# SciML/NeuralPDE.jl

Hardware: AMD Instinct MI355X
Metric: collocation-point residual+grad evals/sec, 2D Poisson 4x64 MLP (higher is better)
Workload: dtype f32, hidden-layer forward / dA / dW GEMMs as 3-piece bf16 split products (6 bf16 MFMAs per product block, fp32 accumulation; 24 mantissa bits rebuilt; the five small piece products on an accumulator of their own: zero-mean, a third of the rms error of an fp32-MFMA fmaf chain per GEMM output, tools/m

## Files before the change

### neuralpde.jl_amd/csrc/aux_kernels.hpp

```cpp
#pragma once
#include <cstdlib>
#include "aux_limits.hpp"
#include "int_limits.hpp"
#include "plat.hpp"
#include "rprog.hpp"
#include "update_rules.hpp"
#include "sample_rules.hpp"

namespace aux {

#ifdef PINN_EMU
#define AUX_DEV inline
#else
#define AUX_DEV __device__ __forceinline__
#endif

struct alignas(16) F4 { float x, y, z, w; };

struct Reduce1Args {
    double* tmp[MAX_GROUPS];
    const float* slabs[MAX_GROUPS];
    const double* losspart[MAX_GROUPS];
    int slab[MAX_GROUPS], nblocks[MAX_GROUPS], nsplit[MAX_GROUPS], nent[MAX_GROUPS], active[MAX_GROUPS];
    int nwpb[MAX_GROUPS];
    int K;
};
struct Reduce2Args {
    float* out;
    float* sums;
    double* lossraw;
    const int* row_ptr;
    const int* row_grp;
    const int* row_ent;
    const double* tmp[MAX_GROUPS];
    int stride[MAX_GROUPS], nsplit[MAX_GROUPS], nent[MAX_GROUPS], active[MAX_GROUPS];
    int ent_active[MAX_GROUPS];
    int ngroups, P, K;
    int skip_grad;
    const int* perm;
};
struct ReduceOneArgs {
    const float* slabs;
    int slab, nblocks, nent;
    const int* ent_theta;
    float* out;
    float* sums;
    double* lossraw;
    int P, K;
    int nloss;
    const double* losspart[MAX_GROUPS];
    int nrows[MAX_GROUPS];
};
constexpr int RONE_CHUNKS = 32, RONE_ENT = 32;

struct ExprArgs {
    const float* pts;
    int N, d, nparams, nparams_estim;
    const float* params;
    int nslots;
    const float* jets[EXPR_MAX_SLOTS];
    float* ubar[EXPR_MAX_SLOTS];
    int nzero;
    float* zero[EXPR_MAX_SLOTS];
    const rp::Instr* prog;
    int nops, out_row;
    float scale;
    double* losspart;
    float* pslab;
    int K, term_id;
    float* resid;
    int loss_only;
    const float* data;
    const float* pw;
};
AUX_DEV float expr_point(int p, const ExprArgs& a, float (&pb)[4]) {
    float v[EXPR_MAX_ROWS], g[EXPR_MAX_ROWS];
    const int R0 = a.d + a.nparams + a.nslots;
    for (int i = 0; i < a.d; ++i) v[i] = a.pts[(size_t)p * a.d + i];
    for (int j = 0; j < a.nparams; ++j) v[a.d + j] = a.params[j];
    for (int s = 0; s < a.nslots; ++s) v[a.d + a.nparams + s] = a.jets[s][p];
    for (int q = 0; q < a.nops; ++q) {
        const rp::Instr ins = a.prog[q];
        const float va = rp::is_nullary(ins.code) ? 0.f : v[ins.a];
        const float vb = rp::is_binary(ins.code) ? v[ins.b] : 0.f;
        v[R0 + q] = (ins.code == rp::OP_DATA) ? a.data[(size_t)(int)ins.imm * a.N + p] : rp::apply<float>(ins.code, va, vb, ins.imm);
    }
    const float r = v[a.out_row];
    for (int j = 0; j < 4; ++j) pb[j] = 0.f;
    if (a.resid) { a.resid[p] = r; return r; }
    if (a.loss_only) return r * (a.pw ? a.pw[p] : 1.0f);
    for (int q = 0; q < R0 + a.nops; ++q) g[q] = 0.f;
    g[a.out_row] = 1.0f;
    for (int q = a.nops - 1; q >= 0; --q) {
        const rp::Instr ins = a.prog[q];
        if (rp::is_nullary(ins.code)) continue;
        const float vb = rp::is_binary(ins.code) ? v[ins.b] : 0.f;
        float da, db;
        rp::adjoint<float>(ins.code, v[ins.a], vb, v[R0 + q], ins.imm, g[R0 + q], da, db);
        g[ins.a] += da;
        if (rp::is_binary(ins.code)) g[ins.b] += db;
    }
    const float sw = a.pw ? a.pw[p] : 1.0f;
    const float rs = r * sw;
    const float rbar = rs * a.scale * sw;
    for (int s = 0; s < a.nslots; ++s) a.ubar[s][p] = rbar * g[a.d + a.nparams + s];
    for (int z = 0; z < a.nzero; ++z) a.zero[z][p] = 0.f;
    for (int j = 0; j < a.nparams_estim; ++j) pb[j] = rbar * g[a.d + j];
    return rs;
}

struct IntNodeDev {
    int var, lo_row, hi_row;
    float lo, hi;
    double lo64, hi64;
    int slot0, nslots;
    int prog_off, nops, out_row;
};
struct IntSitesArgs {
    float* sites;
    int N, d, nnodes, Q;
    const double* xi;
    IntNodeDev node[INT_MAX_NODES];
};
AUX_DEV void int_site_body(int e, const IntSitesArgs& a) {
    const int per = a.nnodes * a.Q;
    if (e >= a.N * per) return;
    const int p = e % a.N, j = e / a.N;
    const int k = j / a.Q, q = j % a.Q;
    const IntNodeDev nd = a.node[k];
    const float* x = a.sites + (size_t)p * a.d;
    const double lo = nd.lo_row >= 0 ? (double)x[nd.lo_row] : nd.lo64;
    const double hi = nd.hi_row >= 0 ? (double)x[nd.hi_row] : nd.hi64;
    const float s = (float)(lo + (hi - lo) * (0.5 * (a.xi[q] + 1.0)));
    float* y = a.sites + ((size_t)(1 + j) * a.N + p) * a.d;
    for (int i = 0; i < a.d; ++i) y[i] = (i == nd.var) ? s : x[i];
}

// ... 142 lines not shown
    for (int q = a.inv_ptr[i]; q < a.inv_ptr[i + 1]; ++q) {
        const int pos = a.inv_pos[q];
        a.packed[pos >> 24][pos & 0xFFFFFF] = t;
    }
}
AUX_DEV void total_loss_body(double* hist, int step, const float* out, int P, int K, const float* w_over_n) {
    double s = 0.0;
    for (int k = 0; k < K; ++k) s += (double)out[P + k] * (double)w_over_n[k];
    hist[step] = s;
}
AUX_DEV void sums_from_double_body(int k, float* out_sums, const double* raw) { out_sums[k] = (float)raw[k]; }
constexpr int PACK_BF_MAX_LAYERS = 16;
struct PackBfArgs {
    const float* theta;
    unsigned* out_fwd;
    unsigned* out_tr;
    int nhh, hp;
    float* packed;
    const int* idx;
    int n_gather;
    int woff[PACK_BF_MAX_LAYERS], nout[PACK_BF_MAX_LAYERS], nin[PACK_BF_MAX_LAYERS];
};
AUX_DEV unsigned bf16_rne(float x) {
    unsigned u;
    __builtin_memcpy(&u, &x, 4);
    if ((u & 0x7FFFFFFFu) > 0x7F800000u) return (u >> 16) | 0x40u;
    u += 0x7FFFu + ((u >> 16) & 1u);
    return u >> 16;
}
AUX_DEV float bf16_val(unsigned h) { const unsigned u = h << 16; float x; __builtin_memcpy(&x, &u, 4); return x; }
AUX_DEV unsigned bf16_piece(float v, int piece) {
    const unsigned h = bf16_rne(v);
    if (piece == 0) return h;
    const float r = v - bf16_val(h);
    const unsigned m = bf16_rne(r);
    if (piece == 1) return m;
    return bf16_rne(r - bf16_val(m));
}
AUX_DEV void pack_bf16_body(int e, const PackBfArgs& a) {
    const int mt = a.hp / 16, kbn = a.hp / 32;
    const int total = a.nhh * mt * kbn * 3 * 256;
    if (e >= 2 * total) return;
    const bool tr = e >= total;
    int r = tr ? e - total : e;
    const int j2 = r & 3; r >>= 2;
    const int lane = r & 63; r >>= 6;
    const int piece = r % 3; r /= 3;
    const int kb = r % kbn; r /= kbn;
    const int ta = r % mt; r /= mt;
    const int hl = r;
    const int g = lane >> 4, c = lane & 15;
    unsigned word = 0;
    for (int half = 0; half < 2; ++half) {
        const int j = 2 * j2 + half;
        const int other = 16 * (2 * kb + (j >> 2)) + 4 * g + (j & 3), mine = 16 * ta + c;
        const int out = tr ? other : mine, in = tr ? mine : other;
        const float v = (out < a.nout[hl] && in < a.nin[hl]) ? a.theta[a.woff[hl] + out + in * a.nout[hl]] : 0.f;
        word |= bf16_piece(v, piece) << (16 * half);
    }
    (tr ? a.out_tr : a.out_fwd)[tr ? e - total : e] = word;
}
struct EmbedArgs {
    const float* upts;
    float* pts;
    int n, du, dx;
    int src[4], is_cos[4];
    double omega[4];
};
AUX_DEV void embed_body(int p, const EmbedArgs& a) {
    if (p >= a.n) return;
    for (int i = 0; i < a.du; ++i) a.pts[(size_t)p * a.dx + i] = a.upts[(size_t)p * a.du + i];
    for (int k = 0; k < a.dx - a.du; ++k) {
        const double ph = a.omega[k] * (double)a.upts[(size_t)p * a.du + a.src[k]];
        a.pts[(size_t)p * a.dx + a.du + k] = (float)(a.is_cos[k] ? cos(ph) : sin(ph));
    }
}
AUX_DEV void pack_body(int i, float* packed, const int* idx, const float* theta) {
    const int j = idx[i];
    packed[i] = (j >= 0) ? theta[j] : 0.f;
}
AUX_DEV void params_body(int j, float* params, const float* theta, const float* defaults, int ne, int p_off) {
    params[j] = (j < ne) ? theta[p_off + j] : defaults[j];
}
#ifdef PINN_EMU
#define AUX_UNROLL8
#else
#define AUX_UNROLL8 _Pragma("unroll 8")
#endif
AUX_DEV void reduce1_body(int e4, int chunk, int g, const Reduce1Args& a) {
    if (!a.active[g] || chunk >= a.nsplit[g]) return;
    const int nb = a.nblocks[g], ns = a.nsplit[g];
    const int per = (nb + ns - 1) / ns;
    const int b0 = chunk * per, b1 = (b0 + per < nb) ? b0 + per : nb;
    double* out = a.tmp[g] + chunk;
    const int nq = a.nent[g] / 4;
    if (e4 < nq) {
        double s0 = 0.0, s1 = 0.0, s2 = 0.0, s3 = 0.0;
        const float* p = a.slabs[g] + 4 * e4;
        AUX_UNROLL8
        for (int b = b0; b < b1; ++b) {
            const F4 q = *reinterpret_cast<const F4*>(p + (size_t)b * a.slab[g]);
            s0 += (double)q.x; s1 += (double)q.y; s2 += (double)q.z; s3 += (double)q.w;
        }
        out[(size_t)(4 * e4) * ns] = s0; out[(size_t)(4 * e4 + 1) * ns] = s1;
        out[(size_t)(4 * e4 + 2) * ns] = s2; out[(size_t)(4 * e4 + 3) * ns] = s3;
    } else if (e4 < nq + a.K) {
        const int k = e4 - nq;
        const double* p = a.losspart[g] + k;
        double s = 0.0;
        AUX_UNROLL8
        for (int wv = b0 * a.nwpb[g]; wv < b1 * a.nwpb[g]; ++wv) s += p[(size_t)wv * a.K];
        out[(size_t)(a.nent[g] + k) * ns] = s;
    }
}
AUX_DEV void reduce_one_chunk(int e4, int ch, const ReduceOneArgs& a, double (&s)[4]) {
    const int per = (a.nblocks + RONE_CHUNKS - 1) / RONE_CHUNKS;
    const int b0 = ch * per, b1 = (b0 + per < a.nblocks) ? b0 + per : a.nblocks;
    s[0] = s[1] = s[2] = s[3] = 0.0;
    const float* p = a.slabs + 4 * e4;
    AUX_UNROLL8
    for (int b = b0; b < b1; ++b) {
        const F4 q = *reinterpret_cast<const F4*>(p + (size_t)b * a.slab);
        s[0] += (double)q.x; s[1] += (double)q.y; s[2] += (double)q.z; s[3] += (double)q.w;
    }
}
AUX_DEV double reduce_one_loss_part(int k, int t, int nthreads, const ReduceOneArgs& a) {
    double s = 0.0;
    for (int i = 0; i < a.nloss; ++i)
        for (int r = t; r < a.nrows[i]; r += nthreads) s += a.losspart[i][(size_t)r * a.K + k];
    return s;
}
AUX_DEV void reduce2_body(int r, const Reduce2Args& a) {
    if (r < a.P) {
        if (a.skip_grad) return;
        double s = 0.0;
        const int i0 = a.row_ptr[r], i1 = a.row_ptr[r + 1];
        for (int i = i0; i < i1; i += 4) {
            const double* t[4];
            int ns[4];
            for (int j = 0; j < 4; ++j) {
                const int ii = (i + j < i1) ? i + j : i;
                const int g = a.row_grp[ii];
                ns[j] = (i + j < i1 && a.ent_active[g]) ? a.nsplit[g] : 0;
                t[j] = a.tmp[g] + (size_t)a.row_ent[ii] * a.nsplit[g];
            }
            for (int j = 0; j < 4; ++j) {
                AUX_UNROLL8
                for (int ch = 0; ch < ns[j]; ++ch) s += t[j][ch];
            }
        }
        a.out[r] = (float)s;
    } else if (r < a.P + a.K) {
        const int k = r - a.P;
        double s = 0.0;
        for (int g = 0; g < a.ngroups; ++g) {
            if (!a.active[g]) continue;
            const double* t = a.tmp[g] + (size_t)(a.nent[g] + k) * a.nsplit[g];
            AUX_UNROLL8
            for (int ch = 0; ch < a.nsplit[g]; ++ch) s += t[ch];
        }
        a.sums[k] = (float)s;
        if (a.lossraw) a.lossraw[k] = s;
    }
}

constexpr int REDUCE_DIRECT_MAX = 32;
AUX_DEV void reduce_direct_body(int t, const Reduce1Args& a1, const Reduce2Args& a) {
    if (t >= a.P + a.K) return;
    const int r = a.perm ? a.perm[t] : t;
    if (r < a.P) {
        if (a.skip_grad) return;
        double s = 0.0;
        for (int i = a.row_ptr[r]; i < a.row_ptr[r + 1]; ++i) {
            const int g = a.row_grp[i];
            if (!a.ent_active[g]) continue;
            const float* p = a1.slabs[g] + a.row_ent[i];
            const int nb = a1.nblocks[g], st = a1.slab[g];
            AUX_UNROLL8
            for (int b = 0; b < nb; ++b) s += (double)p[(size_t)b * st];
        }
        a.out[r] = (float)s;
    } else if (r < a.P + a.K) {
        const int k = r - a.P;
        double s = 0.0;
        for (int g = 0; g < a.ngroups; ++g) {
            if (!a.active[g]) continue;
            const double* p = a1.losspart[g] + k;
            const int nw = a1.nblocks[g] * a1.nwpb[g];
            AUX_UNROLL8
            for (int wv = 0; wv < nw; ++wv) s += p[(size_t)wv * a.K];
        }
        a.sums[k] = (float)s;
        if (a.lossraw) a.lossraw[k] = s;
    }
}

inline bool reduce_is_small(const Reduce1Args& a1, const Reduce2Args& a2) {
    const char* e = std::getenv("PINN_REDUCE_DIRECT_MAX");
    const int lim = e ? std::atoi(e) : REDUCE_DIRECT_MAX;
    for (int g = 0; g < a2.ngroups; ++g)
        if (a1.active[g] && a1.nblocks[g] > lim) return false;
    return true;
}
#ifdef PINN_EMU
inline void launch_pack(float* packed, const int* idx, const float* theta, int n, plat_stream) {
    for (int i = 0; i < n; ++i) pack_body(i, packed, idx, theta);
}
inline void launch_embed(const EmbedArgs& a, plat_stream) {
    for (int p = 0; p < a.n; ++p) embed_body(p, a);
}
inline void launch_params(float* params, const float* theta, const float* defaults, int np, int ne, int p_off, plat_stream) {
    for (int j = 0; j < np; ++j) params_body(j, params, theta, defaults, ne, p_off);
}
// ... 2 lines not shown
    for (int i = 0; i < a.n_gather; ++i) pack_body(i, a.packed, a.idx, a.theta);
    for (int e = 0; e < 2 * total; ++e) pack_bf16_body(e, a);
}
inline void launch_sums_from_double(float* out_sums, const double* raw, int K, plat_stream) {
    for (int k = 0; k < K; ++k) sums_from_double_body(k, out_sums, raw);
}
inline void launch_adam(float* theta, float* m, float* v, const float* grad, int P, float lr, float b1, float b2, float eps, float c1, float c2, plat_stream) {
    for (int i = 0; i < P; ++i) adam_body(i, theta, m, v, grad, lr, b1, b2, eps, c1, c2);
}
inline void launch_total_loss(double* hist, int step, const float* out, int P, int K, const float* w_over_n, plat_stream) {
    total_loss_body(hist, step, out, P, K, w_over_n);
}
inline void launch_sample(int kind, float* pts, int n_elems, int d, const float* lb, const float* ub, unsigned seed, unsigned draw, plat_stream) {
    for (int e = 0; e < n_elems; ++e) {
        if (kind == 3) sample_sobol_body(e, pts, d, lb, ub, seed, draw);
        else if (kind == 2) sample_lhs_body(e, pts, d, n_elems / d, lb, ub, seed, draw);
        else sample_body(e, pts, d, lb, ub, seed, draw);
    }
}
inline void launch_adam_fused(const AdamFusedArgs& a, plat_stream) {
    for (int i = 0; i < (a.P > 1 ? a.P : 1); ++i) adam_fused_body(i, a);
}
inline void launch_resample(const ResampleTerm* samp, int nsamp, int max_n, int step, plat_stream) {
    for (int p = 0; p < max_n; ++p) resample_point_sets(samp, nsamp, p, max_n, step);
}
inline void launch_adam_dev(float* theta, float* m, float* v, const float* grad, int P, float lr, float b1, float b2, float eps, const float* c12, const int* step, plat_stream st) {
    launch_adam(theta, m, v, grad, P, lr, b1, b2, eps, c12[2 * step[0]], c12[2 * step[0] + 1], st);
}
inline void launch_total_loss_dev(double* hist, const int* step, const float* out, int P, int K, const float* w_over_n, plat_stream st) {
    launch_total_loss(hist, step[0], out, P, K, w_over_n, st);
}
inline void launch_sample_dev(int kind, float* pts, int n_elems, int d, const float* lb, const float* ub, unsigned seed, const unsigned* draw, plat_stream st) {
    launch_sample(kind, pts, n_elems, d, lb, ub, seed, draw[0], st);
}
inline void launch_advance(int* step, unsigned* draws, const int* sampled, int K, plat_stream) {
    for (int t = 0; t < K; ++t) if (sampled[t]) ++draws[t];
    ++step[0];
}
inline void launch_src(const SrcArgs& a, plat_stream) {
    for (int p = 0; p < a.N; ++p) src_point(p, a);
}
inline void launch_expr(const ExprArgs& a, int nblocks, plat_stream) {
    for (int b = 0; b < nblocks; ++b)
        for (int w = 0; w < 4; ++w) {
            double ls = 0.0;
            double ps[4] = {0, 0, 0, 0};
            for (int l = 0; l < 64; ++l) {
                const int p = (b * 4 + w) * 64 + l;
                if (p >= a.N) continue;
                float pb[4];
                const float r = expr_point(p, a, pb);
                ls += (double)r * (double)r;
                for (int j = 0; j < 4; ++j) ps[j] += (double)pb[j];
            }
            if (!a.resid) {
                a.losspart[(size_t)(b * 4 + w) * a.K + a.term_id] = ls;
                for (int j = 0; j < 4; ++j) a.pslab[(size_t)(b * 4 + w) * 4 + j] = (float)ps[j];
            }
        }
}
inline void launch_int_sites(const IntSitesArgs& a, plat_stream) {
    for (int e = 0; e < a.N * a.nnodes * a.Q; ++e) int_site_body(e, a);
}
inline void launch_int_expr(const IntExprArgs& a, int nblocks, plat_stream) {
    for (int b = 0; b < nblocks; ++b)
        for (int w = 0; w < 4; ++w) {
            double ls = 0.0;
            double ps[4] = {0, 0, 0, 0};
            for (int l = 0; l < 64; ++l) {
                const int p = (b * 4 + w) * 64 + l;
                if (p >= a.N) continue;
                float pb[4];
                const float r = int_expr_point(p, a, pb);
                ls += (double)r * (double)r;
                for (int j = 0; j < 4; ++j) ps[j] += (double)pb[j];
            }
            if (!a.resid) {
                a.losspart[(size_t)(b * 4 + w) * a.K + a.term_id] = ls;
                for (int j = 0; j < 4; ++j) a.pslab[(size_t)(b * 4 + w) * 4 + j] = (float)ps[j];
            }
        }
}
inline void launch_reduce_one(const ReduceOneArgs& a, plat_stream) {
    for (int e4 = 0; e4 < a.nent / 4; ++e4) {
        double tot[4] = {0, 0, 0, 0}, s[4];
        for (int ch = 0; ch < RONE_CHUNKS; ++ch) {
            reduce_one_chunk(e4, ch, a, s);
            for (int e = 0; e < 4; ++e) tot[e] += s[e];
        }
        for (int e = 0; e < 4; ++e)
            if (a.ent_theta[4 * e4 + e] >= 0) a.out[a.ent_theta[4 * e4 + e]] = (float)tot[e];
    }
    for (int k = 0; k < a.K; ++k) {
        double part[256], s = 0.0;
        for (int t = 0; t < 256; ++t) part[t] = reduce_one_loss_part(k, t, 256, a);
        for (int st = 128; st >= 1; st >>= 1)
            for (int t = 0; t < st; ++t) part[t] += part[t + st];
        s = part[0];
        a.sums[k] = (float)s;
        if (a.lossraw) a.lossraw[k] = s;
    }
}
inline void launch_reduce(const Reduce1Args& a1, const Reduce2Args& a2, int max_n1, int max_split, plat_stream) {
    if (reduce_is_small(a1, a2)) {
        for (int r = 0; r < a2.P + a2.K; ++r) reduce_direct_body(r, a1, a2);
        return;
    }
    for (int g = 0; g < a2.ngroups; ++g)
        for (int ch = 0; ch < max_split; ++ch)
            for (int e = 0; e < max_n1; ++e) reduce1_body(e, ch, g, a1);
    for (int r = 0; r < a2.P + a2.K; ++r) reduce2_body(r, a2);
}
#else
__global__ void k_pack(float* packed, const int* idx, const float* theta, int n) {
    const int i = blockIdx.x * blockDim.x + threadIdx.x;
    if (i < n) pack_body(i, packed, idx, theta);
}
__global__ void k_params(float* params, const float* theta, const float* defaults, int np, int ne, int p_off) {
    const int j = threadIdx.x;
    if (j < np) params_body(j, params, theta, defaults, ne, p_off);
}
__global__ void k_adam(float* theta, float* m, float* v, const float* grad, int P, float lr, float b1, float b2, float eps, float c1, float c2) {
    const int i = blockIdx.x * blockDim.x + threadIdx.x;
    if (i < P) adam_body(i, theta, m, v, grad, lr, b1, b2, eps, c1, c2);
}
__global__ void k_total_loss(double* hist, int step, const float* out, int P, int K, const float* w_over_n) {
    if (threadIdx.x == 0 && blockIdx.x == 0) total_loss_body(hist, step, out, P, K, w_over_n);
}
__global__ void k_sample(float* pts, int n_elems, int d, const float* lb, const float* ub, unsigned seed, unsigned draw) {
    const int e = blockIdx.x * blockDim.x + threadIdx.x;
    if (e < n_elems) sample_body(e, pts, d, lb, ub, seed, draw);
}
__global__ void k_sample_lhs(float* pts, int n_elems, int d, const float* lb, const float* ub, unsigned seed, unsigned draw) {
    const int e = blockIdx.x * blockDim.x + threadIdx.x;
    if (e < n_elems) sample_lhs_body(e, pts, d, n_elems / d, lb, ub, seed, draw);
}
__global__ void k_sample_sobol(float* pts, int n_elems, int d, const float* lb, const float* ub, unsigned seed, unsigned draw) {
    const int e = blockIdx.x * blockDim.x + threadIdx.x;
    if (e < n_elems) sample_sobol_body(e, pts, d, lb, ub, seed, draw);
}
inline void launch_adam(float* theta, float* m, float* v, const float* grad, int P, float lr, float b1, float b2, float eps, float c1, float c2, plat_stream st) {
    hipLaunchKernelGGL(k_adam, dim3((P + 255) / 256), dim3(256), 0, st, theta, m, v, grad, P, lr, b1, b2, eps, c1, c2);
}
inline void launch_total_loss(double* hist, int step, const float* out, int P, int K, const float* w_over_n, plat_stream st) {
    hipLaunchKernelGGL(k_total_loss, dim3(1), dim3(64), 0, st, hist, step, out, P, K, w_over_n);
}
inline void launch_sample(int kind, float* pts, int n_elems, int d, const float* lb, const float* ub, unsigned seed, unsigned draw, plat_stream st) {
    if (kind == 3) hipLaunchKernelGGL(k_sample_sobol, dim3((n_elems + 255) / 256), dim3(256), 0, st, pts, n_elems, d, lb, ub, seed, draw);
    else if (kind == 2) hipLaunchKernelGGL(k_sample_lhs, dim3((n_elems + 255) / 256), dim3(256), 0, st, pts, n_elems, d, lb, ub, seed, draw);
    else hipLaunchKernelGGL(k_sample, dim3((n_elems + 255) / 256), dim3(256), 0, st, pts, n_elems, d, lb, ub, seed, draw);
}
__global__ void __launch_bounds__(256) k_resample(const ResampleTerm* samp, int nsamp, int step) {
    resample_point_sets(samp, nsamp, (int)(blockIdx.x * blockDim.x + threadIdx.x), (int)(gridDim.x * blockDim.x), step);
}
inline void launch_resample(const ResampleTerm* samp, int nsamp, int max_n, int step, plat_stream st) {
    hipLaunchKernelGGL(k_resample, dim3((max_n + 255) / 256), dim3(256), 0, st, samp, nsamp, step);
}
__global__ void k_adam_fused(const AdamFusedArgs a) { adam_fused_body((int)(blockIdx.x * blockDim.x + threadIdx.x), a); }
inline void launch_adam_fused(const AdamFusedArgs& a, plat_stream st) {
    hipLaunchKernelGGL(k_adam_fused, dim3((a.P + 255) / 256), dim3(256), 0, st, a);
}
__global__ void k_adam_dev(float* theta, float* m, float* v, const float* grad, int P, float lr, float b1, float b2, float eps, const float* c12, const int* step) {
    const int i = blockIdx.x * blockDim.x + threadIdx.x;
    const int s = step[0];
    if (i < P) adam_body(i, theta, m, v, grad, lr, b1, b2, eps, c12[2 * s], c12[2 * s + 1]);
}
__global__ void k_total_loss_dev(double* hist, const int* step, const float* out, int P, int K, const float* w_over_n) {
    if (threadIdx.x == 0 && blockIdx.x == 0) total_loss_body(hist, step[0], out, P, K, w_over_n);
}
__global__ void k_sample_dev(int kind, float* pts, int n_elems, int d, const float* lb, const float* ub, unsigned seed, const unsigned* draw) {
    const int e = blockIdx.x * blockDim.x + threadIdx.x;
    if (e >= n_elems) return;
    const unsigned dr = draw[0];
    if (kind == 3) sample_sobol_body(e, pts, d, lb, ub, seed, dr);
    else if (kind == 2) sample_lhs_body(e, pts, d, n_elems / d, lb, ub, seed, dr);
    else sample_body(e, pts, d, lb, ub, seed, dr);
}
__global__ void k_advance(int* step, unsigned* draws, const int* sampled, int K) {
    const int t = threadIdx.x;
    if (t < K && sampled[t]) ++draws[t];
    if (t == 0) ++step[0];
}
inline void launch_adam_dev(float* theta, float* m, float* v, const float* grad, int P, float lr, float b1, float b2, float eps, const float* c12, const int* step, plat_stream st) {
    hipLaunchKernelGGL(k_adam_dev, dim3((P + 255) / 256), dim3(256), 0, st, theta, m, v, grad, P, lr, b1, b2, eps, c12, step);
// ... 13 lines not shown
    float pb[4] = {0.f, 0.f, 0.f, 0.f};
    float r = 0.f;
    if (p < a.N) r = expr_point(p, a, pb);
    if (a.resid) return;
    sh[0][threadIdx.x] = (double)r * (double)r;
    for (int j = 0; j < 4; ++j) sh[1 + j][threadIdx.x] = (double)pb[j];
    __syncthreads();
    if (threadIdx.x < 20) {
        const int w = threadIdx.x & 3, q = threadIdx.x >> 2;
        double s = 0.0;
        for (int l = 0; l < 64; ++l) s += sh[q][w * 64 + l];
        if (q == 0) a.losspart[(size_t)(blockIdx.x * 4 + w) * a.K + a.term_id] = s;
        else a.pslab[(size_t)(blockIdx.x * 4 + w) * 4 + (q - 1)] = (float)s;
    }
}
__global__ void k_reduce1(const Reduce1Args a) {
    reduce1_body((int)(blockIdx.x * blockDim.x + threadIdx.x), (int)blockIdx.y, (int)blockIdx.z, a);
}
__global__ void k_reduce2(const Reduce2Args a) {
    reduce2_body((int)(blockIdx.x * blockDim.x + threadIdx.x), a);
}
inline void launch_pack(float* packed, const int* idx, const float* theta, int n, plat_stream st) {
    hipLaunchKernelGGL(k_pack, dim3((n + 255) / 256), dim3(256), 0, st, packed, idx, theta, n);
}
__global__ void k_embed(const EmbedArgs a) { embed_body((int)(blockIdx.x * blockDim.x + threadIdx.x), a); }
inline void launch_embed(const EmbedArgs& a, plat_stream st) {
    hipLaunchKernelGGL(k_embed, dim3((a.n + 255) / 256), dim3(256), 0, st, a);
}
inline void launch_params(float* params, const float* theta, const float* defaults, int np, int ne, int p_off, plat_stream st) {
    if (np > 0) hipLaunchKernelGGL(k_params, dim3(1), dim3(64), 0, st, params, theta, defaults, np, ne, p_off);
}
__global__ void k_pack_bf16(const PackBfArgs a) {
    const int e = (int)(blockIdx.x * blockDim.x + threadIdx.x);
    if (e < a.n_gather) pack_body(e, a.packed, a.idx, a.theta);
    else pack_bf16_body(e - a.n_gather, a);
}
inline void launch_pack_bf16(const PackBfArgs& a, plat_stream st) {
    const int total = a.nhh * (a.hp / 16) * (a.hp / 32) * 3 * 256;
    hipLaunchKernelGGL(k_pack_bf16, dim3((a.n_gather + 2 * total + 255) / 256), dim3(256), 0, st, a);
}
__global__ void k_sums_from_double(float* out_sums, const double* raw, int K) {
    const int k = (int)(blockIdx.x * blockDim.x + threadIdx.x);
    if (k < K) sums_from_double_body(k, out_sums, raw);
}
inline void launch_sums_from_double(float* out_sums, const double* raw, int K, plat_stream st) {
    hipLaunchKernelGGL(k_sums_from_double, dim3((K + 63) / 64), dim3(64), 0, st, out_sums, raw, K);
}
__global__ void __launch_bounds__(256) k_src(const SrcArgs a) {
    const int p = blockIdx.x * 256 + threadIdx.x;
    if (p < a.N) src_point(p, a);
}
inline void launch_src(const SrcArgs& a, plat_stream st) {
    hipLaunchKernelGGL(k_src, dim3((a.N + 255) / 256), dim3(256), 0, st, a);
}
inline void launch_expr(const ExprArgs& a, int nblocks, plat_stream st) {
    hipLaunchKernelGGL(k_expr, dim3(nblocks), dim3(256), 0, st, a);
}
__global__ void __launch_bounds__(256) k_int_sites(const IntSitesArgs a) { int_site_body((int)(blockIdx.x * 256 + threadIdx.x), a); }
inline void launch_int_sites(const IntSitesArgs& a, plat_stream st) {
    hipLaunchKernelGGL(k_int_sites, dim3((a.N * a.nnodes * a.Q + 255) / 256), dim3(256), 0, st, a);
}
__global__ void __launch_bounds__(256) k_int_expr(const IntExprArgs a) {
    __shared__ double sh[5][256];
    const int p = blockIdx.x * 256 + threadIdx.x;
    float pb[4] = {0.f, 0.f, 0.f, 0.f};
    float r = 0.f;
    if (p < a.N) r = int_expr_point(p, a, pb);
    if (a.resid) return;
    sh[0][threadIdx.x] = (double)r * (double)r;
    for (int j = 0; j < 4; ++j) sh[1 + j][threadIdx.x] = (double)pb[j];
    __syncthreads();
    if (threadIdx.x < 20) {
        const int w = threadIdx.x & 3, q = threadIdx.x >> 2;
        double s = 0.0;
        for (int l = 0; l < 64; ++l) s += sh[q][w * 64 + l];
        if (q == 0) a.losspart[(size_t)(blockIdx.x * 4 + w) * a.K + a.term_id] = s;
        else a.pslab[(size_t)(blockIdx.x * 4 + w) * 4 + (q - 1)] = (float)s;
    }
}
inline void launch_int_expr(const IntExprArgs& a, int nblocks, plat_stream st) {
    hipLaunchKernelGGL(k_int_expr, dim3(nblocks), dim3(256), 0, st, a);
}
__global__ void __launch_bounds__(256) k_reduce_one(const ReduceOneArgs a) {
    __shared__ double sh[RONE_CHUNKS][RONE_ENT + 1];
    const int tid = (int)threadIdx.x;
    const int nentblocks = (a.nent + RONE_ENT - 1) / RONE_ENT;
    if ((int)blockIdx.x < nentblocks) {
        const int j = tid & 7, ch = tid >> 3;
        const int e4 = (int)blockIdx.x * (RONE_ENT / 4) + j;
        double s[4] = {0.0, 0.0, 0.0, 0.0};
        if (4 * e4 < a.nent) reduce_one_chunk(e4, ch, a, s);
        for (int e = 0; e < 4; ++e) sh[ch][4 * j + e] = s[e];
        __syncthreads();
        if (tid < RONE_ENT) {
            const int ent = (int)blockIdx.x * RONE_ENT + tid;
            if (ent < a.nent) {
                double tot = 0.0;
                for (int c2 = 0; c2 < RONE_CHUNKS; ++c2) tot += sh[c2][tid];
                const int th = a.ent_theta[ent];
                if (th >= 0) a.out[th] = (float)tot;
            }
        }
    } else {
        const int k = (int)blockIdx.x - nentblocks;
        double* part = &sh[0][0];
        part[tid] = reduce_one_loss_part(k, tid, 256, a);
        __syncthreads();
        for (int st = 128; st >= 1; st >>= 1) {
            if (tid < st) part[tid] += part[tid + st];
            __syncthreads();
        }
        if (tid == 0) {
            a.sums[k] = (float)part[0];
            if (a.lossraw) a.lossraw[k] = part[0];
        }
    }
}
inline void launch_reduce_one(const ReduceOneArgs& a, plat_stream st) {
    hipLaunchKernelGGL(k_reduce_one, dim3((a.nent + RONE_ENT - 1) / RONE_ENT + a.K), dim3(256), 0, st, a);
}
__global__ void k_reduce_direct(const Reduce1Args a1, const Reduce2Args a2) {
    reduce_direct_body((int)(blockIdx.x * blockDim.x + threadIdx.x), a1, a2);
}
inline void launch_reduce(const Reduce1Args& a1, const Reduce2Args& a2, int max_n1, int max_split, plat_stream st) {
    if (reduce_is_small(a1, a2)) {
        hipLaunchKernelGGL(k_reduce_direct, dim3((a2.P + a2.K + 63) / 64), dim3(64), 0, st, a1, a2);
        return;
    }
    hipLaunchKernelGGL(k_reduce1, dim3((max_n1 + 255) / 256, max_split, a2.ngroups), dim3(256), 0, st, a1);
    hipLaunchKernelGGL(k_reduce2, dim3((a2.P + a2.K + 255) / 256), dim3(256), 0, st, a2);
}
#endif

}
```

### neuralpde.jl_amd/csrc/comm.cpp

```cpp
#include "engine_types.hpp"

using namespace pe;

#ifndef PINN_EMU
#include <dlfcn.h>
#include <rccl/rccl.h>

namespace {
struct Rccl {
    void* lib = nullptr;
    ncclResult_t (*GetUniqueId)(ncclUniqueId*) = nullptr;
    ncclResult_t (*CommInitRank)(ncclComm_t*, int, ncclUniqueId, int) = nullptr;
    ncclResult_t (*CommInitAll)(ncclComm_t*, int, const int*) = nullptr;
    ncclResult_t (*CommDestroy)(ncclComm_t) = nullptr;
    ncclResult_t (*AllReduce)(const void*, void*, size_t, ncclDataType_t, ncclRedOp_t, ncclComm_t, hipStream_t) = nullptr;
    ncclResult_t (*GroupStart)() = nullptr;
    ncclResult_t (*GroupEnd)() = nullptr;
    const char* (*GetErrorString)(ncclResult_t) = nullptr;
    std::string err;
};
Rccl& rccl() {
    static Rccl R = [] {
        Rccl r;
        for (const char* name : {"librccl.so.1", "librccl.so", "/opt/rocm/lib/librccl.so.1"}) {
// ... 216 lines not shown
    for (int i = 0; i < ndev; ++i) {
        pinn_engine& E = *es[i];
        DeviceScope scope(E.device);
        const ncclResult_t rc = rccl().AllReduce(vec[i], vec[i], (size_t)count, ncclDouble, ncclSum, (ncclComm_t)E.comm, E.stream);
        if (rc != ncclSuccess) { (void)rccl().GroupEnd(); return nccl_fail("ncclAllReduce", rc); }
    }
    NCCL_TRY(rccl().GroupEnd(), "ncclGroupEnd");
#else
    {
        std::vector<double> sum((size_t)count, 0.0);
        for (int i = 0; i < ndev; ++i)
            for (int64_t j = 0; j < count; ++j) sum[(size_t)j] += vec[i][j];
        for (int i = 0; i < ndev; ++i) std::memcpy(vec[i], sum.data(), sizeof(double) * (size_t)count);
    }
#endif
    return 0;
}

extern "C" {

int pinn_loss_grad_sharded_device_f64(pinn_handle h, const double* d_theta, const float* term_w, double* d_out, void* stream) {
    if (!h || !d_theta || !d_out) return fail("pinn_loss_grad_sharded_device_f64: null argument");
    pinn_engine& E = *h;
    if (!E.f64) return fail("pinn_loss_grad_sharded_device_f64: the handle is not in the float64 evaluation mode (pinn_set_option(h, \"precision\", \"f64\"))");
    if (!E.comm) return fail("pinn_loss_grad_sharded_device_f64: the handle has no communicator (pinn_comm_init_rank / pinn_comm_init_custom)");
    if (!E.comm_per_process && E.comm_size > 1)
        return fail("pinn_loss_grad_sharded_device_f64: the handle belongs to a single-process communicator (pinn_comm_init_all): use pinn_loss_grad_sharded_f64");
    DeviceScope scope(E.device);
    if (check_shards(E)) return 1;
    plat_stream saved = E.stream;
    E.stream = (plat_stream)stream;
    int rc = f64_eval_from_device_f64(E, d_theta, term_w, d_out);
    if (!rc) {
        pinn_engine* es[1] = {&E};
        double* vec[1] = {d_out};
        rc = comm_all_reduce_f64(es, 1, vec, E.ntheta + (int64_t)E.terms.size());
    }
    E.stream = saved;
    return rc;
}

int pinn_loss_grad_sharded_f64(pinn_handle* hs, int ndev, const double* theta, int64_t p, const double* term_w, double* term_losses, double* grad) {
    if (!hs || ndev < 1 || !theta) return fail("pinn_loss_grad_sharded_f64: null argument");
    for (int i = 0; i < ndev; ++i) {
        if (!hs[i] || !hs[i]->comm || hs[i]->comm_size != ndev || hs[i]->comm_rank != i)
            return fail("pinn_loss_grad_sharded_f64: pass the handles of one pinn_comm_init_all communicator, in rank order");
        if (!hs[i]->f64) return fail("pinn_loss_grad_sharded_f64: every handle must be in the float64 evaluation mode");
        if (p != hs[i]->ntheta) return fail("pinn_loss_grad_sharded_f64: theta length mismatch");
    }
    const int64_t P = hs[0]->ntheta;
    const int K = (int)hs[0]->terms.size();
    std::vector<double*> vec(ndev);
    for (int i = 0; i < ndev; ++i) {
        pinn_engine& E = *hs[i];
        DeviceScope scope(E.device);
        if (check_shards(E)) return 1;
        if (f64_eval_sharded_local(E, theta, term_w, &vec[i])) return 1;
    }
    if (comm_all_reduce_f64(hs, ndev, vec.data(), P + K)) return 1;
    std::vector<double> out((size_t)(P + K));
    {
        pinn_engine& E0 = *hs[0];
        DeviceScope scope(E0.device);
        if (plat_d2h(out.data(), vec[0], sizeof(double) * (size_t)(P + K), E0.stream)) return fail("D2H copy failed");
    }
    for (int i = 0; i < ndev; ++i) {
        DeviceScope scope(hs[i]->device);
        if (plat_sync(hs[i]->stream)) return fail(std::string("device error: ") + plat_last_error());
    }
    if (term_losses) for (int k = 0; k < K; ++k) term_losses[k] = out[(size_t)P + k] / (double)hs[0]->terms[k].n_norm;
    if (grad) std::memcpy(grad, out.data(), sizeof(double) * (size_t)P);
    return 0;
}

int pinn_loss_grad_sharded_device(pinn_handle h, const float* d_theta, const float* term_w, float* d_out, void* stream) {
    if (!h || !d_theta || !d_out) return fail("pinn_loss_grad_sharded_device: null argument");
    pinn_engine& E = *h;
    if (!E.comm) return fail("pinn_loss_grad_sharded_device: the handle has no communicator (pinn_comm_init_rank / pinn_comm_init_all)");
    DeviceScope scope(E.device);
    if (check_shards(E)) return 1;
    plat_stream st = (plat_stream)stream;
    plat_stream saved = E.stream;
    E.stream = st;
    int rc = run_loss_grad(E, d_theta, d_out, term_w, -1, true);
    E.stream = saved;
    if (rc) return rc;
    E.timing_valid = E.timing_level >= 2;
    if (!E.comm_per_process && E.comm_size > 1)
        return fail("pinn_loss_grad_sharded_device: the handle belongs to a single-process communicator (pinn_comm_init_all): use pinn_loss_grad_sharded");
    {
        pinn_engine* es[1] = {&E};
        float* vec[1] = {d_out};
        double* raw[1] = {E.d_lossraw};
        E.stream = st;
        rc = comm_all_reduce(es, 1, vec, raw);
        E.stream = saved;
        if (rc) return rc;
    }
    sums_from_double(d_out + E.ntheta, E.d_lossraw, (int)E.terms.size(), st);
    return 0;
}

int pinn_loss_grad_sharded(pinn_handle* hs, int ndev, const float* theta, int64_t p, const float* term_w, double* term_losses, float* grad) {
    if (!hs || ndev < 1 || !theta) return fail("pinn_loss_grad_sharded: null argument");
    for (int i = 0; i < ndev; ++i) {
        if (!hs[i] || !hs[i]->comm || hs[i]->comm_size != ndev || hs[i]->comm_rank != i)
            return fail("pinn_loss_grad_sharded: pass the handles of one pinn_comm_init_all communicator, in rank order");
        if (i > 0 && hs[i]->comm != hs[0]->comm
#ifndef PINN_EMU
            && false
#endif
        ) return fail("pinn_loss_grad_sharded: handles of different communicators");
    }
    const int64_t P = hs[0]->ntheta;
    const int K = (int)hs[0]->terms.size();
    for (int i = 0; i < ndev; ++i) {
        pinn_engine& E = *hs[i];
        DeviceScope scope(E.device);
        if (check_shards(E) || upload_theta(E, theta, p)) return 1;
        if (run_loss_grad(E, E.d_theta, E.d_out, term_w, -1, false)) return 1;
    }
    {
        std::vector<float*> vec(ndev);
        std::vector<double*> raw(ndev);
        for (int i = 0; i < ndev; ++i) { vec[i] = hs[i]->d_out; raw[i] = hs[i]->d_lossraw; }
        if (comm_all_reduce(hs, ndev, vec.data(), raw.data())) return 1;
    }
    pinn_engine& E0 = *hs[0];
    {
        DeviceScope scope(E0.device);
        if (plat_d2h(E0.hp_out, E0.d_out, sizeof(float) * (P + K), E0.stream)) return fail("D2H copy failed");
        if (plat_d2h(E0.hp_raw, E0.d_lossraw, sizeof(double) * K, E0.stream)) return fail("D2H copy failed");
    }
    for (int i = 0; i < ndev; ++i) {
        DeviceScope scope(hs[i]->device);
        if (plat_sync(hs[i]->stream)) return fail(std::string("device error: ") + plat_last_error());
    }
    if (term_losses)
        for (int k = 0; k < K; ++k) term_losses[k] = E0.hp_raw[k] / (double)E0.terms[k].n_norm;
    if (grad) std::memcpy(grad, E0.hp_out, sizeof(float) * P);
    return 0;
}

}
```

### neuralpde.jl_amd/csrc/engine.cpp

```cpp
#include "engine_types.hpp"
#include "aux_kernels.hpp"
#include "hmc_kernels.hpp"
#include "lbfgs_kernels.hpp"

#include <type_traits>

#ifdef PINN_EMU
namespace wv {
thread_local void (*emu_barrier_hook)(void*) = nullptr;
thread_local void* emu_barrier_ctx = nullptr;
thread_local void (*emu_grid_hook)(void*) = nullptr;
thread_local void* emu_grid_ctx = nullptr;
}
#endif

namespace pk {
std::deque<SpecInfo>& registry() {
    static std::deque<SpecInfo> r;
    return r;
}
std::deque<PairInfo>& pair_registry() {
    static std::deque<PairInfo> r;
    return r;
}
// ... 120 lines not shown
    std::memset(&a, 0, sizeof a);
    a.sites = T.d_pts; a.N = (int)T.n; a.d = T.d; a.nparams = E.np; a.nparams_estim = E.ne; a.params = E.d_params;
    a.jets = Cp.d_jets[0]; a.ubar = Cp.d_ubar[0]; a.C = E.groups[Cp.groups[0]].spec->C;
    a.n_outer = T.n_outer; a.nnodes = (int)T.inodes.size(); a.Q = T.int_q;
    for (size_t si = 0; si < T.slots.size(); ++si) a.chan[si] = T.chan_of_slot[si];
    for (int c = 0; c < aux::INT_MAX_C; ++c) {
        a.outer_slot_of_chan[c] = -1;
        for (int k = 0; k < aux::INT_MAX_NODES; ++k) a.node_slot_of_chan[k][c] = -1;
    }
    for (int si = 0; si < T.n_outer; ++si) a.outer_slot_of_chan[T.chan_of_slot[(size_t)si]] = si;
    int off = 0;
    for (int k = 0; k < a.nnodes; ++k) {
        a.node[k] = int_node_dev(T, k, off);
        off += (int)T.inodes[(size_t)k].ops.size();
        for (int si = a.node[k].slot0; si < a.node[k].slot0 + a.node[k].nslots; ++si) a.node_slot_of_chan[k][T.chan_of_slot[(size_t)si]] = si;
    }
    a.w = E.d_int_w;
    a.prog = Cp.d_prog; a.iprog = T.d_int_prog; a.nops = (int)T.ops.size(); a.out_row = T.out_row; a.scale = scale;
    a.losspart = Cp.d_losspart; a.pslab = Cp.d_pslab; a.K = (int)E.terms.size(); a.term_id = Cp.term; a.resid = resid;
    a.data = T.d_data;
    a.pw = (T.pw_n == T.n && T.pw_n > 0) ? T.d_pw : nullptr;
    return a;
}

int upload_int_rule(pinn_engine& E, int q) {
    std::vector<double> xi((size_t)q), w((size_t)q);
    const double PI = 3.14159265358979323846264338327950288;
    for (int i = 0; i < q; ++i) {
        double x = -std::cos(PI * (i + 0.75) / (q + 0.5)), dp = 1.0;
        for (int it = 0; it < 100; ++it) {
            double p0 = 1.0, p1 = x;
            for (int n = 2; n <= q; ++n) { const double p2 = ((2.0 * n - 1.0) * x * p1 - (n - 1.0) * p0) / n; p0 = p1; p1 = p2; }
            dp = q * (x * p1 - p0) / (x * x - 1.0);
            const double dx = p1 / dp;
            x -= dx;
            if (std::fabs(dx) < 1e-16) break;
        }
        {
            double p0 = 1.0, p1 = x;
            for (int n = 2; n <= q; ++n) { const double p2 = ((2.0 * n - 1.0) * x * p1 - (n - 1.0) * p0) / n; p0 = p1; p1 = p2; }
            dp = q * (x * p1 - p0) / (x * x - 1.0);
        }
        xi[(size_t)i] = x;
        w[(size_t)i] = 2.0 / ((1.0 - x * x) * dp * dp);
    }
    std::vector<float> wf(w.begin(), w.end());
    if (!E.d_int_xi) {
        E.d_int_xi = (double*)plat_malloc(sizeof(double) * aux::INT_MAX_Q);
        E.d_int_w = (float*)plat_malloc(sizeof(float) * aux::INT_MAX_Q);
        if (!E.d_int_xi || !E.d_int_w) return fail("device allocation failed (quadrature rule)");
    }
    plat_h2d(E.d_int_xi, xi.data(), sizeof(double) * q, E.stream);
    plat_h2d(E.d_int_w, wf.data(), sizeof(float) * q, E.stream);
    if (plat_sync(E.stream)) return fail(std::string("device error: ") + plat_last_error());
    return 0;
}

template <class V, class T> class As {
    static constexpr bool same = std::is_same_v<V, std::remove_const_t<T>>;
    T* x_;
    std::vector<V> copy_;
public:
    As(T* x, size_t n) : x_(x) {
        if constexpr (!same) {
            if (x && std::is_const_v<T>) copy_.assign(x, x + n);
            else if (x) copy_.resize(n);
        }
    }
    auto get() {
        if constexpr (same) return x_;
        else return x_ ? copy_.data() : nullptr;
    }
    int put() {
        if constexpr (!same) if (x_) std::copy(copy_.begin(), copy_.end(), x_);
        return 0;
    }
};
template <class V, class T> As<V, T> as(T* x, size_t n) { return As<V, T>(x, n); }

int check_theta(const pinn_engine& E, const char* who, int64_t p) {
    return p == E.ntheta ? 0 : fail(std::string(who) + ": theta length " + std::to_string(p) + " != ntheta " + std::to_string(E.ntheta));
}

}

int pe::run_loss_grad(pinn_engine& E, const float* d_theta, float* d_out, const float* term_w, int only_term , bool timing,
                  double* lossraw , bool packed_fresh, bool loss_only, float* d_sums) {
    if (!d_sums) d_sums = d_out + E.ntheta;
    if (ensure_points(E)) return 1;
    const int K = (int)E.terms.size();
    const bool phase_ev = timing && E.timing_level >= 2;
    auto group_ev = [&](size_t g) { return timing && E.timing_level >= 1 && (E.timing_group < 0 || E.timing_group == (int)g); };
    if (phase_ev) plat_event_record(E.ev0, E.stream);
    pack_all(E, d_theta, packed_fresh);
    if (phase_ev) plat_event_record(E.ev1, E.stream);
    aux::Reduce1Args a1;
    aux::Reduce2Args a2;
    std::memset(&a1, 0, sizeof a1);
    std::memset(&a2, 0, sizeof a2);
    int max_n1 = 1, max_split = 1;
    auto scale_of = [&](int ti) -> float {
        const float w = term_w ? term_w[ti] : 1.0f;
        const bool on = (only_term < 0 || only_term == ti);
        return on ? (float)(2.0 * (double)w / (double)E.terms[ti].n_norm) : 0.f;
    };
    int nfused_active = 0;
    bool all_small = true;
    for (auto& G : E.groups) {
        bool on = false;
        for (int ti : G.terms) on = on || (only_term < 0 || only_term == ti);
        if (G.kind == 0 && on) {
            ++nfused_active;
            const int per_round = G.max_blocks * (G.spec->family == 2 ? 1 : 4);
            if (2 * G.ga.ntiles > 3 * per_round) all_small = false;
        }
    }
    static const bool want_concurrent = std::getenv("PINN_CONCURRENT_GROUPS") != nullptr;
    const bool concurrent = want_concurrent && nfused_active >= 2 && all_small;
    static const bool no_chain = std::getenv("PINN_NO_CHAIN") != nullptr;
    const bool no_merge = std::getenv("PINN_NO_MERGE") != nullptr;
    const bool may_merge = !no_merge && !no_chain && !concurrent && only_term < 0;
    int nforked = 0;
    int nslabsets = 0, slabset_group = -1;
    if (concurrent) plat_event_record(E.ev_fork, E.stream);
    for (size_t g = 0; g < E.groups.size(); ++g) {
        Group& G = E.groups[g];
        bool any = false;
        for (size_t j = 0; j < G.terms.size(); ++j) {
            G.ga.terms[j].scale = scale_of(G.terms[j]);
            any = any || (only_term < 0 || only_term == G.terms[j]);
        }
        G.active = any;
        G.timed = false;
        const MergedUnit* mu = (may_merge && G.kind == 0 && G.merged >= 0) ? &E.merged[G.merged] : nullptr;
        a1.tmp[g] = G.d_tmp; a1.slabs[g] = G.d_slabs; a1.losspart[g] = G.d_losspart;
        a2.tmp[g] = G.d_tmp;
        if (mu && (int)g == mu->tail) {
            G.launched_by = mu->head;
            G.launched_blocks = E.groups[mu->head].launched_blocks;
            a1.active[g] = 0; a2.active[g] = 0; a2.ent_active[g] = 0;
            a1.slab[g] = G.slab_floats; a1.nblocks[g] = 0; a1.nsplit[g] = 1; a1.nent[g] = 0; a1.nwpb[g] = G.spec->NW;
            a2.stride[g] = K; a2.nsplit[g] = 1; a2.nent[g] = 0;
            continue;
        }
        const bool chained = any && !loss_only && !no_chain && !concurrent && G.kind == 0 && G.chain_to >= 0 && E.groups[G.chain_to].active &&
                             G.blocks <= E.groups[G.chain_to].launched_blocks;
        const int nent = (chained || loss_only) ? 0 : G.nent;
        G.ga.slabs = chained ? E.groups[G.chain_to].d_slabs : G.d_slabs;
        G.ga.chain = chained ? 1 : 0;
        pk::GroupArgs ga_one;
        const pk::GroupArgs* ga_launch = &G.ga;
        int blocks = G.blocks;
        if (any && only_term >= 0 && G.kind == 0 && G.terms.size() > 1) {
            ga_one = G.ga;
            for (size_t j = 0; j < G.terms.size(); ++j)
                if (G.terms[j] == only_term) ga_one.terms[0] = G.ga.terms[j];
            ga_one.nterms = 1;
            ga_one.terms[0].tile0 = 0;
            ga_one.ntiles = ga_one.terms[0].ntiles;
            blocks = std::max(1, std::min(G.max_blocks, G.spec->family == 1 ? (ga_one.ntiles + 3) / 4 : ga_one.ntiles));
            ga_launch = &ga_one;
        }
        const bool merged_head = mu && (int)g == mu->head;
        if (merged_head) {
            const Group& T2 = E.groups[mu->tail];
            ga_one = G.ga;
            for (size_t j = 0; j < T2.terms.size(); ++j) {
                pk::TermDev td = T2.ga.terms[j];
                td.tile0 += G.ga.ntiles;
                td.scale = scale_of(T2.terms[j]);
                ga_one.terms[G.terms.size() + j] = td;
            }
            ga_one.nterms = (int)(G.terms.size() + T2.terms.size());
            ga_one.sub_terms0 = (int)G.terms.size();
            ga_one.sub_tiles0 = G.ga.ntiles;
            ga_one.ntiles = G.ga.ntiles + T2.ga.ntiles;
            ga_one.scratch = mu->d_scratch;
            ga_one.scr_stride = mu->pair->SCR;
            ga_one.losspart = mu->d_losspart;
            a1.losspart[g] = mu->d_losspart;
            ga_one.chain = 0;
            blocks = std::max(1, std::min(loss_only ? E.ncu * mu->pair->WG_FWD : mu->max_blocks, ga_one.ntiles));
            ga_launch = &ga_one;
        }
        G.launched_blocks = blocks;
        G.launched_by = (int)g;
        const int epe = G.spec->family == 1 ? 4 : 1;
        const int nsplit_g = std::max(1, std::min(REDUCE_SPLIT, (int)std::ceil(std::sqrt((double)blocks / epe))));
        a1.slab[g] = G.slab_floats; a1.nblocks[g] = blocks; a1.nsplit[g] = nsplit_g; a1.nent[g] = nent; a1.active[g] = any; a1.nwpb[g] = G.spec->NW;
        a2.stride[g] = nent + K; a2.nsplit[g] = nsplit_g; a2.nent[g] = nent; a2.active[g] = any;
        a2.ent_active[g] = any && !chained && !loss_only;
        if (!any) continue;
        if (a2.ent_active[g]) { ++nslabsets; slabset_group = (int)g; }
        max_n1 = std::max(max_n1, nent / 4 + K);
        max_split = std::max(max_split, nsplit_g);
        if (G.kind == 1) {
            G.spec->launch(G.ga, (G.use_rec && !loss_only) ? pk::MODE_FWDREC : pk::MODE_FWD,
                           std::max(1, std::min(E.ncu * G.spec->WG_FWD, G.spec->family == 1 ? (G.ga.ntiles + 3) / 4 : G.ga.ntiles)), E.stream);
            continue;
        }
        if (G.kind == 2) continue;
        plat_stream st = E.stream;
        const bool forked = concurrent && nforked++ > 0;
        if (forked) {
            st = E.aux_stream[nforked % 2];
            plat_stream_wait_event(st, E.ev_fork);
        }
        if (group_ev(g)) plat_event_record(G.ev_a, st);
        if (merged_head) mu->pair->launch(*ga_launch, loss_only ? pk::MODE_LOSS : pk::MODE_FUSED, blocks, st);
        else if (loss_only) {
            const int tiles = ga_launch->ntiles;
            const int fb = std::max(1, std::min(E.ncu * G.spec->WG_FWD, G.spec->family == 1 ? (tiles + 3) / 4 : tiles));
            a1.nblocks[g] = fb;
            G.launched_blocks = fb;
            G.spec->launch(*ga_launch, pk::MODE_LOSS, fb, st);
        } else G.spec->launch(*ga_launch, pk::MODE_FUSED, blocks, st);
        if (group_ev(g)) plat_event_record(G.ev_b, st);
        G.timed = group_ev(g);
        if (forked) {
            plat_event_record(E.ev_join[g], st);
            plat_stream_wait_event(E.stream, E.ev_join[g]);
        }
    }
    bool coupled_active = false;
    for (size_t c = 0; c < E.coupled.size(); ++c) {
        Coupled& Cp = E.coupled[c];
        const int g = (int)(E.groups.size() + c);
        const bool on = (only_term < 0 || only_term == Cp.term);
        const int nsplit = std::min(REDUCE_SPLIT, Cp.blocks);
        const int nent = loss_only ? 0 : 16;
        a1.tmp[g] = Cp.d_tmp; a1.slabs[g] = Cp.d_pslab; a1.losspart[g] = Cp.d_losspart;
        a1.slab[g] = 16; a1.nblocks[g] = Cp.blocks; a1.nsplit[g] = nsplit; a1.nent[g] = nent; a1.active[g] = on; a1.nwpb[g] = 4;
        a2.tmp[g] = Cp.d_tmp; a2.stride[g] = nent + K; a2.nsplit[g] = nsplit; a2.nent[g] = nent; a2.active[g] = on; a2.ent_active[g] = on && !loss_only;
        bool groups_active = false;
        for (int gi : Cp.groups) groups_active = groups_active || E.groups[gi].active;
        if (!groups_active) continue;
        coupled_active = true;
        if (Cp.tail >= 0) {
            Group& G = E.groups[Cp.groups[Cp.tail]];
            a1.active[g] = 0; a2.active[g] = 0; a2.ent_active[g] = 0;
            if (group_ev((size_t)Cp.groups[Cp.tail])) plat_event_record(G.ev_a, E.stream);
            if (loss_only) {
                const int fb = std::max(1, std::min(E.ncu * G.spec->WG_FWD, G.ga.ntiles));
                a1.nblocks[Cp.groups[Cp.tail]] = fb;
                G.launched_blocks = fb;
                G.spec->launch(G.ga, pk::MODE_LOSS, fb, E.stream);
            } else G.spec->launch(G.ga, pk::MODE_FUSED, G.blocks, E.stream);
            if (group_ev((size_t)Cp.groups[Cp.tail])) plat_event_record(G.ev_b, E.stream);
            G.timed = group_ev((size_t)Cp.groups[Cp.tail]);
            continue;
        }
        max_n1 = std::max(max_n1, nent / 4 + K);
        max_split = std::max(max_split, nsplit);
        if (!E.terms[Cp.term].inodes.empty()) {
            aux::IntExprArgs ia = int_expr_args(E, Cp, scale_of(Cp.term), nullptr);
            ia.loss_only = loss_only ? 1 : 0;
            aux::launch_int_expr(ia, Cp.blocks, E.stream);
            continue;
        }
        aux::ExprArgs ea = expr_args(E, Cp, scale_of(Cp.term), nullptr);
        ea.loss_only = loss_only ? 1 : 0;
        aux::launch_expr(ea, Cp.blocks, E.stream);
    }
    for (size_t g = 0; g < E.groups.size() && !loss_only; ++g) {
        Group& G = E.groups[g];
        if (G.kind != 1 || !G.active) continue;
        if (group_ev(g)) plat_event_record(G.ev_a, E.stream);
        G.spec->launch(G.ga, G.use_rec ? pk::MODE_GRADREC : pk::MODE_GRADIN, G.blocks, E.stream);
        if (group_ev(g)) plat_event_record(G.ev_b, E.stream);
        G.timed = group_ev(g);
    }
    if (phase_ev) plat_event_record(E.ev2, E.stream);
    a1.K = K;
    a2.out = d_out; a2.sums = d_sums; a2.lossraw = lossraw ? lossraw : E.d_lossraw; a2.row_ptr = E.d_gr_ptr; a2.row_grp = E.d_gr_grp; a2.row_ent = E.d_gr_ent;
    a2.ngroups = (int)(E.groups.size() + E.coupled.size()); a2.P = (int)E.ntheta; a2.K = K;
    a2.skip_grad = loss_only ? 1 : 0;
    a2.perm = std::getenv("PINN_NO_REDUCE_PERM") ? nullptr : E.d_red_perm;
    const bool no_reduce_one = std::getenv("PINN_NO_REDUCE_ONE") != nullptr;
    const Group* RG = (nslabsets == 1 && !coupled_active && !loss_only && !no_reduce_one) ? &E.groups[slabset_group] : nullptr;
    const bool one_kernel = ((RG && RG->d_ent_theta && RG->ent_covers_theta) || (loss_only && !no_reduce_one)) && !aux::reduce_is_small(a1, a2);
    if (one_kernel) {
        aux::ReduceOneArgs ro;
        std::memset(&ro, 0, sizeof ro);
        if (RG) { ro.slabs = RG->d_slabs; ro.slab = RG->slab_floats; ro.nblocks = a1.nblocks[slabset_group]; ro.nent = RG->nent; ro.ent_theta = RG->d_ent_theta; }
        ro.out = d_out; ro.sums = d_sums; ro.lossraw = a2.lossraw; ro.P = (int)E.ntheta; ro.K = K;
        for (int g = 0; g < a2.ngroups; ++g)
            if (a1.active[g]) { ro.losspart[ro.nloss] = a1.losspart[g]; ro.nrows[ro.nloss] = a1.nblocks[g] * a1.nwpb[g]; ++ro.nloss; }
        aux::launch_reduce_one(ro, E.stream);
    } else {
        aux::launch_reduce(a1, a2, max_n1, max_split, E.stream);
    }
    if (phase_ev) plat_event_record(E.ev3, E.stream);
    { const std::string e = jit_take_launch_error(); if (!e.empty()) return fail(e); }
    return 0;
}

void pe::sums_from_double(float* d_out_sums, const double* d_raw, int K, plat_stream st) { aux::launch_sums_from_double(d_out_sums, d_raw, K, st); }

int pe::upload_theta(pinn_engine& E, const float* theta, int64_t p) {
    if (p != E.ntheta) return fail("theta length " + std::to_string(p) + " != ntheta " + std::to_string(E.ntheta));
    std::memcpy(E.hp_theta, theta, sizeof(float) * p);
    if (plat_h2d(E.d_theta, E.hp_theta, sizeof(float) * p, E.stream)) return fail(std::string("H2D copy of theta failed: ") + plat_last_error());
    return 0;
}

static void hmc_free(pinn_engine& E);
static void lbfgs_free(pinn_engine& E);

extern "C" {

const char* pinn_backend(void) { return plat_name(); }
int pinn_abi_version(void) { return 1; }
const char* pinn_last_error(void) { return g_err.c_str(); }

int pinn_create(const char* descriptor, pinn_handle* out) { return pinn_create_on(descriptor, -1, out); }

int pinn_create_on(const char* descriptor, int device, pinn_handle* out) {
    if (!descriptor || !out) return fail("pinn_create: null argument");
    *out = nullptr;
    std::string err;
    if (plat_init(err)) return fail(err);
    if (device >= plat_device_count()) return fail("pinn_create_on: device " + std::to_string(device) + " does not exist (" + std::to_string(plat_device_count()) + " visible)");
    const int dev = device < 0 ? plat_get_device() : device;
    DeviceScope scope(dev);
    std::unique_ptr<pinn_engine> E(new pinn_engine());
    E->device = dev;
    if (const char* gm = std::getenv("PINN_GEMM")) {
        if (std::string(gm) == "fp32") E->gemm = pk::GEMM_FP32;
        else if (std::string(gm) == "split") E->gemm = pk::GEMM_SPLIT;
        else return fail(std::string("PINN_GEMM must be \"split\" or \"fp32\", not \"") + gm + "\"");
    }
    if (parse_descriptor(descriptor, *E)) return 1;
    E->terms0 = E->terms;
    E->ncu = plat_num_cus();
    E->stream = plat_stream_create();
    const int K = (int)E->terms.size();
    E->d_theta = (float*)plat_malloc(sizeof(float) * E->ntheta);
    E->d_params = (float*)plat_malloc(sizeof(float) * pk::MAX_PARAMS);
    E->d_defaults = (float*)plat_malloc(sizeof(float) * pk::MAX_PARAMS);
    E->d_lossraw = (double*)plat_malloc(sizeof(double) * K);
    E->d_out = (float*)plat_malloc(sizeof(float) * (E->ntheta + K));
    plat_event_create(E->ev0); plat_event_create(E->ev1); plat_event_create(E->ev2); plat_event_create(E->ev3);
    plat_event_create(E->ev_fork);
    for (auto& e : E->ev_join) plat_event_create(e);
    for (auto& st : E->aux_stream) st = plat_stream_create();
    if (!E->d_theta || !E->d_params || !E->d_defaults || !E->d_lossraw || !E->d_out) {
        pinn_destroy(E.release());
        return fail("device allocation failed");
    }
    plat_h2d(E->d_defaults, E->p_defaults.data(), sizeof(float) * pk::MAX_PARAMS, E->stream);
    E->hp_theta = (float*)plat_host_alloc(sizeof(float) * (2 * E->ntheta + K + 2) + sizeof(double) * K);
    if (!E->hp_theta) {
        pinn_destroy(E.release());
        return fail("pinned host allocation failed");
    }
    E->hp_out = E->hp_theta + E->ntheta;
    E->hp_raw = (double*)(E->hp_theta + ((2 * E->ntheta + K + 1) / 2) * 2);
    bool any_int = false;
    for (auto& T : E->terms) any_int = any_int || !T.inodes.empty();
    if ((any_int && upload_int_rule(*E, E->int_q)) || build_plan(*E)) {
        const std::string msg = g_err;
        pinn_destroy(E.release());
        g_err = msg;
        return 1;
    }
    *out = E.release();
    return 0;
}

int pinn_destroy(pinn_handle h) {
    if (!h) return 0;
    pinn_engine& E = *h;
    DeviceScope scope(E.device);
    pinn_comm_destroy(h);
    plat_sync(E.stream);
    hmc_free(E);
    lbfgs_free(E);
    f64_destroy(E);
    free_plan(E);
    for (auto& T : E.terms) { plat_free(T.d_pts); plat_free(T.d_upts); plat_free(T.d_resid); plat_free(T.d_lb); plat_free(T.d_ub); plat_free(T.d_data); plat_free(T.d_pw); }
    plat_free(E.d_opt_theta); plat_free(E.d_opt_m); plat_free(E.d_opt_v); plat_free(E.d_opt_out); plat_free(E.d_w_over_n); plat_free(E.d_hist); plat_free(E.d_step); plat_free(E.d_draws); plat_free(E.d_sampled); plat_free(E.d_c12); plat_free(E.d_bar); plat_free(E.d_sums2); plat_free(E.d_own_r); plat_free(E.d_train_samp); plat_free(E.d_opt_bak); plat_host_free(E.h_flag);
    plat_free(E.d_theta); plat_free(E.d_params); plat_free(E.d_defaults); plat_free(E.d_lossraw);
    plat_free(E.d_int_xi); plat_free(E.d_int_w);
    plat_free(E.d_out); plat_free(E.d_phi_pts); plat_free(E.d_phi_out); plat_free(E.d_phi_scr);
    plat_host_free(E.hp_theta);
    plat_event_destroy(E.ev0); plat_event_destroy(E.ev1); plat_event_destroy(E.ev2); plat_event_destroy(E.ev3);
    plat_event_destroy(E.ev_fork);
    for (auto& e : E.ev_join) plat_event_destroy(e);
    for (auto& st : E.aux_stream) plat_stream_destroy(st);
    if (E.own_stream) plat_stream_destroy(E.stream);
    delete h;
    return 0;
}

int pinn_num_terms(pinn_handle h) { return h ? (int)h->terms.size() : -1; }
int64_t pinn_num_theta(pinn_handle h) { return h ? h->ntheta : -1; }

static int term_installed(pinn_engine& E, int term);
static int set_points_impl(pinn_handle h, int term, const float* pts, int64_t n, int64_t n_norm, bool device) {
    if (!h) return fail("null handle");
    pinn_engine& E = *h;
    DeviceScope scope(E.device);
    if (term < 0 || term >= (int)E.terms.size()) return fail("pinn_set_points: term index out of range");
    if (!pts || n <= 0) return fail("pinn_set_points: empty point set (the reference's mean(abs2, .) over an empty set is NaN; refusing)");
    Term& T = E.terms[term];
    if (n * T.d >= (int64_t)1 << 31) return fail("pinn_set_points: point set too large for 32-bit indexing; shard it");
    const int64_t S = T.sites();
    if (S > 1 && n * S * std::max(T.d, aux::INT_MAX_C) >= (int64_t)1 << 31)
        return fail("pinn_set_points: the site set of integral term " + std::to_string(term) + " (" + std::to_string(n) + " points x (1 + " +
                    std::to_string(T.inodes.size()) + " integral node(s) x " + std::to_string(T.int_q) + " quadrature nodes) = " + std::to_string(n * S) +
                    " sites) exceeds what one launch group takes (32-bit indexing of its jet channels); shard the point set or lower integral_nodes");
    if (n > T.pts_cap || !T.d_pts) {
        plat_sync(E.stream);
        plat_free(T.d_pts);
        plat_free(T.d_upts);
        T.d_upts = nullptr;
        T.pts_cap = 0;
        T.d_pts = (float*)plat_malloc(sizeof(float) * n * S * T.d);
        if (!T.emb_cols.empty()) T.d_upts = (float*)plat_malloc(sizeof(float) * n * T.d_user);
        if (!T.d_pts || (!T.emb_cols.empty() && !T.d_upts)) return fail("device allocation failed (points)");
        T.pts_cap = n;
    }
    int rc = device ? plat_d2d(user_pts(T), pts, sizeof(float) * n * T.d_user, E.stream) : plat_h2d(user_pts(T), pts, sizeof(float) * n * T.d_user, E.stream);
    if (rc) return fail(std::string("copy of points failed: ") + plat_last_error());
    T.n = n;
    embed_points(E, T);
    plat_sync(E.stream);
    T.n_norm = n_norm > 0 ? n_norm : n;
    T.data_n = 0;
    T.pw_n = 0;
    if (term_installed(E, term)) return 1;
    return f64_points_changed(E, term);
}

static int term_installed(pinn_engine& E, int term) {
    Term& T = E.terms[term];
    int64_t n = T.n;
    if (T.coupled < 0) {
        if (!T.src_root.empty()) {
            if (T.src_cap < n) {
                plat_free(T.d_src);
                T.d_src = (float*)plat_malloc(sizeof(float) * T.src_root.size() * (size_t)n);
                if (!T.d_src) return fail("device allocation failed (source channels)");
                T.src_cap = n;
            }
            eval_sources(E, T);
            plat_sync(E.stream);
        }
        retile(E, T.group);
        return 0;
    }
    Coupled& Cp = E.coupled[T.coupled];
    const int K = (int)E.terms.size();
    const int64_t npts = n;
    n *= T.sites();
    if (Cp.cap < n) {
        for (size_t i = 0; i < Cp.d_jets.size(); ++i)
            if (Cp.tail < 0 || (int)i == Cp.tail) { plat_free(Cp.d_jets[i]); plat_free(Cp.d_ubar[i]); }
        plat_free(Cp.d_jets_all); plat_free(Cp.d_ubar_all);
        Cp.d_jets_all = Cp.d_ubar_all = nullptr;
        Cp.d_jets.assign(Cp.nets.size(), nullptr);
        Cp.d_ubar.assign(Cp.nets.size(), nullptr);
        Cp.cap = 0;
        if (Cp.tail >= 0 && Cp.nsrc > 0) {
            Cp.d_jets_all = (float*)plat_malloc(sizeof(float) * (size_t)Cp.nsrc * n);
            Cp.d_ubar_all = (float*)plat_malloc(sizeof(float) * (size_t)Cp.nsrc * n);
            if (!Cp.d_jets_all || !Cp.d_ubar_all) return fail("device allocation failed (coupled jets)");
        }
        for (size_t i = 0; i < Cp.nets.size(); ++i) {
            if (Cp.tail >= 0 && (int)i != Cp.tail) continue;
            const int C = E.groups[Cp.groups[i]].spec->C;
            Cp.d_jets[i] = (float*)plat_malloc(sizeof(float) * (size_t)C * n);
            Cp.d_ubar[i] = (float*)plat_malloc(sizeof(float) * (size_t)C * n);
            if (!Cp.d_jets[i] || !Cp.d_ubar[i]) return fail("device allocation failed (coupled jets)");
        }
        Cp.cap = n;
    }
    if (Cp.tail >= 0)
        for (size_t i = 0; i < Cp.nets.size(); ++i)
            if ((int)i != Cp.tail) { Cp.d_jets[i] = Cp.d_jets_all + (size_t)Cp.src_off[i] * n; Cp.d_ubar[i] = Cp.d_ubar_all + (size_t)Cp.src_off[i] * n; }
    Cp.blocks = (int)((npts + 255) / 256);
    if (Cp.cap_blocks < Cp.blocks) {
        plat_free(Cp.d_losspart); plat_free(Cp.d_pslab);
        Cp.d_losspart = (double*)plat_malloc(sizeof(double) * (size_t)Cp.blocks * 4 * K);
        Cp.d_pslab = (float*)plat_malloc(sizeof(float) * (size_t)Cp.blocks * 16);
        if (!Cp.d_losspart || !Cp.d_pslab) return fail("device allocation failed (coupled partials)");
        plat_memset(Cp.d_losspart, 0, sizeof(double) * (size_t)Cp.blocks * 4 * K, E.stream);
        plat_memset(Cp.d_pslab, 0, sizeof(float) * (size_t)Cp.blocks * 16, E.stream);
        plat_sync(E.stream);
        Cp.cap_blocks = Cp.blocks;
    }
    for (int gi : Cp.groups) retile(E, gi);
    return 0;
}
int pinn_set_points(pinn_handle h, int term, const float* pts, int64_t n, int64_t n_norm) { return set_points_impl(h, term, pts, n, n_norm, false); }
int pinn_set_points_device(pinn_handle h, int term, const float* d_pts, int64_t n, int64_t n_norm) { return set_points_impl(h, term, d_pts, n, n_norm, true); }
int pinn_set_points_f64(pinn_handle h, int term, const double* pts, int64_t n, int64_t n_norm) {
    if (!h || !pts || n <= 0) return fail("pinn_set_points_f64: null argument / empty point set");
    if (term < 0 || term >= (int)h->terms.size()) return fail("pinn_set_points_f64: term index out of range");
    auto p32 = as<float>(pts, (size_t)n * h->terms[term].d_user);
    if (set_points_impl(h, term, p32.get(), n, n_norm, false)) return 1;
    if (!h->f64) return 0;
    DeviceScope scope(h->device);
    return f64_set_points(*h, term, pts, n);
}

static void measure_grad_health(pinn_engine& E, const float* grad_and_sums, const float* term_w);
static int gemm_auto_check(pinn_engine& E, const float* d_theta, const float* term_w, long long now);
static bool eval_eligible(pinn_engine& E);
static int eval_fused(pinn_engine& E, const float* d_theta, float* d_out, const float* term_w, double* lossraw);
static bool train_timed_out(pinn_engine& E);
static int eval_and_sync(pinn_engine& E, float* d_out, const float* term_w, double* lossraw, bool timing) {
    E.eval_path = 1;
    if (ensure_points(E)) return 1;
    if (eval_eligible(E)) {
        if (eval_fused(E, E.d_theta, d_out, term_w, lossraw)) return 1;
        if (plat_sync(E.stream)) return fail(std::string("device error: ") + plat_last_error());
        if (!train_timed_out(E)) { E.eval_path = 2; return 0; }
    }
    if (run_loss_grad(E, E.d_theta, d_out, term_w, -1, timing, lossraw, false, false)) return 1;
    if (plat_sync(E.stream)) return fail(std::string("device error: ") + plat_last_error());
    return 0;
}

static int loss_grad_f32(pinn_engine& E, const float* theta, const float* term_w, double* term_losses, float* grad) {
    const int K = (int)E.terms.size();
    if (upload_theta(E, theta, E.ntheta)) return 1;
    if (grad) {
        if (eval_and_sync(E, E.hp_out, term_w, E.hp_raw, true)) return 1;
    } else {
        if (run_loss_grad(E, E.d_theta, E.hp_out, term_w, -1, true, E.hp_raw, false, true)) return 1;
        if (plat_sync(E.stream)) return fail(std::string("device error: ") + plat_last_error());
    }
    E.timing_valid = E.timing_level >= 2;
    if (term_losses)
        for (int k = 0; k < K; ++k) term_losses[k] = E.hp_raw[k] / (double)E.terms[k].n_norm;
    if (grad) std::memcpy(grad, E.hp_out, sizeof(float) * E.ntheta);
    if (grad && E.gemm_auto) {
        std::vector<float> gs((size_t)E.ntheta + K);
        std::memcpy(gs.data(), E.hp_out, sizeof(float) * E.ntheta);
        for (int k = 0; k < K; ++k) gs[(size_t)E.ntheta + k] = (float)E.hp_raw[k];
        measure_grad_health(E, gs.data(), term_w);
        if (gemm_auto_check(E, E.d_theta, term_w, ++E.eval_count)) return 1;
    }
    return 0;
}

static void loglik_from_sse(const pinn_engine& E, const double* stds, const double* sse, double* loglik, double* grad_std) {
    const int K = (int)E.terms.size();
    double ll = 0.0;
    for (int k = 0; k < K; ++k) {
        const double N = (double)E.terms[k].n, sd = stds[k];
        ll += -0.5 * N * std::log(2.0 * 3.14159265358979323846) - N * std::log(sd) - sse[k] / (2.0 * sd * sd);
        if (grad_std) grad_std[k] = -N / sd + sse[k] / (sd * sd * sd);
    }
    *loglik = ll;
}
static int loglik_f64(pinn_engine& E, const double* theta, const double* stds, double* loglik, double* grad_theta, double* grad_std) {
    const int K = (int)E.terms.size();
    std::vector<double> w(K), L(K), g(grad_theta ? (size_t)E.ntheta : 0);
    for (int k = 0; k < K; ++k) w[k] = (double)E.terms[k].n_norm / (2.0 * stds[k] * stds[k]);
    if (f64_eval(E, theta, w.data(), L.data(), grad_theta ? g.data() : nullptr)) return 1;
    for (int k = 0; k < K; ++k) L[k] *= (double)E.terms[k].n_norm;
    loglik_from_sse(E, stds, L.data(), loglik, grad_std);
    if (grad_theta) for (int64_t i = 0; i < E.ntheta; ++i) grad_theta[i] = -g[(size_t)i];
    return 0;
}

static int loglik_f32(pinn_engine& E, const float* theta, const double* stds, double* loglik, float* grad_theta, double* grad_std) {
    const int K = (int)E.terms.size();
    std::vector<float> w(K);
    for (int k = 0; k < K; ++k) w[k] = (float)((double)E.terms[k].n_norm / (2.0 * stds[k] * stds[k]));
    if (upload_theta(E, theta, E.ntheta)) return 1;
    if (run_loss_grad(E, E.d_theta, E.hp_out, w.data(), -1, false, E.hp_raw)) return 1;
    if (plat_sync(E.stream)) return fail(std::string("device error: ") + plat_last_error());
    loglik_from_sse(E, stds, E.hp_raw, loglik, grad_std);
    if (grad_theta)
        for (int64_t i = 0; i < E.ntheta; ++i) grad_theta[i] = -E.hp_out[i];
    return 0;
}

static int term_grads_f64(pinn_engine& E, const double* theta, double* term_losses, double* term_grads) {
    const int K = (int)E.terms.size();
    const int64_t p = E.ntheta;
    std::vector<double> w(K), L(K);
    for (int k = 0; k < K; ++k) {
        for (int j = 0; j < K; ++j) w[j] = (j == k) ? 1.0 : 0.0;
        if (f64_eval(E, theta, w.data(), L.data(), term_grads + (size_t)k * p)) return 1;
        if (term_losses) term_losses[k] = L[k];
    }
    return 0;
}

static int term_grads_f32(pinn_engine& E, const float* theta, double* term_losses, float* term_grads) {
    const int K = (int)E.terms.size();
    const int64_t p = E.ntheta;
    if (upload_theta(E, theta, p)) return 1;
    for (int k = 0; k < K; ++k) {
        if (run_loss_grad(E, E.d_theta, E.hp_out, nullptr, k, false, E.hp_raw)) return 1;
        if (plat_sync(E.stream)) return fail(std::string("device error: ") + plat_last_error());
        std::memcpy(term_grads + (size_t)k * p, E.hp_out, sizeof(float) * p);
        if (term_losses) term_losses[k] = E.hp_raw[k] / (double)E.terms[k].n_norm;
    }
    return 0;
}

int pinn_loss_grad_device(pinn_handle h, const float* d_theta, const float* term_w, float* d_out, void* stream) {
    if (!h || !d_theta || !d_out) return fail("pinn_loss_grad_device: null argument");
    pinn_engine& E = *h;
    DeviceScope scope(E.device);
    const int K = (int)E.terms.size();
    plat_stream user = (plat_stream)stream;
    plat_stream saved = E.stream;
    E.stream = user;
    int rc = E.f64 ? f64_eval_from_device_f32(E, d_theta, term_w, d_out, true) : run_loss_grad(E, d_theta, d_out, term_w, -1, true);
    E.stream = saved;
    if (rc && g_err.empty()) return fail("pinn_loss_grad_device failed");
    E.timing_valid = (rc == 0) && E.timing_level >= 2;
    return rc;
}

int pinn_loss_grad_device_f64(pinn_handle h, const double* d_theta, const float* term_w, double* d_out, void* stream) {
    if (!h || !d_theta || !d_out) return fail("pinn_loss_grad_device_f64: null argument");
    pinn_engine& E = *h;
    if (!E.f64) return fail("pinn_loss_grad_device_f64: the handle is not in the float64 evaluation mode (pinn_set_option(h, \"precision\", \"f64\"))");
    DeviceScope scope(E.device);
    plat_stream saved = E.stream;
    E.stream = (plat_stream)stream;
    const int rc = f64_eval_from_device_f64(E, d_theta, term_w, d_out);
    E.stream = saved;
    if (rc && g_err.empty()) return fail("pinn_loss_grad_device_f64 failed");
    return rc;
}

int pinn_loss_device(pinn_handle h, const float* d_theta, float* d_sums, void* stream) {
    if (!h || !d_theta || !d_sums) return fail("pinn_loss_device: null argument");
    pinn_engine& E = *h;
    DeviceScope scope(E.device);
    plat_stream saved = E.stream;
    E.stream = (plat_stream)stream;
    int rc = E.f64 ? f64_eval_from_device_f32(E, d_theta, nullptr, d_sums, false)
                   : run_loss_grad(E, d_theta, nullptr, nullptr, -1, false, nullptr, false, true, d_sums);
    E.stream = saved;
    if (rc && g_err.empty()) return fail("pinn_loss_device failed");
    return rc;
}

int pinn_group_launched_by(pinn_handle h, int group) {
    if (!h || group < 0 || group >= (int)h->groups.size()) return -1;
    return h->groups[group].launched_by;
}

static int residual_f32(pinn_engine& E, int term, const float* theta, float* r) {
    Term& T = E.terms[term];
    if (!T.d_pts) return fail("pinn_residual: term has no points");
    if (upload_theta(E, theta, E.ntheta)) return 1;
    pack_all(E);
    jit_take_launch_error();
    if (T.resid_cap < T.n) {
        plat_free(T.d_resid);
        T.d_resid = (float*)plat_malloc(sizeof(float) * T.n);
        T.resid_cap = T.n;
        if (!T.d_resid) return fail("device allocation failed (residual)");
    }
    if (T.coupled >= 0) {
        Coupled& Cp = E.coupled[T.coupled];
        for (int gi : Cp.groups) {
            Group& G = E.groups[gi];
            pk::GroupArgs ga = G.ga;
            int j = 0;
            for (size_t q = 0; q < G.terms.size(); ++q) if (G.terms[q] == term) j = (int)q;
            ga.nterms = 1;
            ga.terms[0] = G.ga.terms[j];
            ga.terms[0].tile0 = 0;
            ga.ntiles = ga.terms[0].ntiles;
            G.spec->launch(ga, pk::MODE_FWD, std::max(1, std::min(E.ncu * G.spec->WG_FWD, G.spec->family == 1 ? (ga.ntiles + 3) / 4 : ga.ntiles)), E.stream);
        }
        if (!T.inodes.empty()) aux::launch_int_expr(int_expr_args(E, Cp, 0.f, T.d_resid), Cp.blocks, E.stream);
        else aux::launch_expr(expr_args(E, Cp, 0.f, T.d_resid), Cp.blocks, E.stream);
        if (plat_d2h(r, T.d_resid, sizeof(float) * T.n, E.stream)) return fail("D2H copy failed");
        if (plat_sync(E.stream)) return fail(std::string("device error: ") + plat_last_error());
        { const std::string le = jit_take_launch_error(); if (!le.empty()) return fail("pinn_residual: " + le); }
        return 0;
    }
    Group& G = E.groups[T.group];
    pk::GroupArgs ga = G.ga;
    ga.nterms = 1;
    ga.terms[0] = G.ga.terms[T.slot_in_group];
    ga.terms[0].tile0 = 0;
    ga.terms[0].out = T.d_resid;
    ga.ntiles = ga.terms[0].ntiles;
    const int blocks = std::max(1, std::min(E.ncu * G.spec->WG_FWD, G.spec->family == 1 ? (ga.ntiles + 3) / 4 : ga.ntiles));
    G.spec->launch(ga, pk::MODE_RESID, blocks, E.stream);
    if (plat_d2h(r, T.d_resid, sizeof(float) * T.n, E.stream)) return fail("D2H copy failed");
    if (plat_sync(E.stream)) return fail(std::string("device error: ") + plat_last_error());
    { const std::string le = jit_take_launch_error(); if (!le.empty()) return fail("pinn_residual: " + le); }
    return 0;
}
// ... 997 lines not shown
    if (plat_sync(E.stream)) return fail(std::string("device error: ") + plat_last_error());
    return 0;
}

int pinn_set_timing(pinn_handle h, int level, int group) {
    if (!h) return fail("pinn_set_timing: null handle");
    if (level < 0 || level > 2) return fail("pinn_set_timing: level must be 0, 1 or 2");
    if (group < -1 || group >= (int)h->groups.size()) return fail("pinn_set_timing: group index out of range");
    h->timing_level = level; h->timing_group = group;
    h->timing_valid = false;
    for (auto& G : h->groups) G.timed = false;
    return 0;
}

int pinn_last_timing(pinn_handle h, float* kernel_ms, float* total_ms) {
    if (!h) return fail("null handle");
    if (!h->timing_valid) return fail("no timing available: switch the phase events on (pinn_set_timing(h, 2, -1)), then call pinn_loss_grad");
    plat_event_sync(h->ev3);
    if (kernel_ms) *kernel_ms = plat_event_ms(h->ev1, h->ev2);
    if (total_ms) *total_ms = plat_event_ms(h->ev0, h->ev3);
    return 0;
}

int pinn_num_groups(pinn_handle h) { return h ? (int)h->groups.size() : -1; }

#ifdef PINN_STAMP
int pinn_debug_train_stamps(pinn_handle h, unsigned long long* out4) {
    if (!h || !h->d_bar || !out4) return -1;
    plat_sync(h->stream);
    plat_d2h(out4, h->d_bar + 4, sizeof(unsigned long long) * 4, h->stream);
    plat_sync(h->stream);
    return 0;
}
int pinn_debug_slab(pinn_handle h, int group, int blk, float* dst, int64_t n) {
    if (!h || group < 0 || group >= (int)h->groups.size()) return -1;
    Group& G = h->groups[group];
    if (blk < 0) return G.blocks;
    if (blk == (1 << 30)) return G.spec->SLAB;
    if (blk >= G.blocks || n > G.spec->SLAB) return -1;
    plat_sync(h->stream);
    plat_d2h(dst, G.d_slabs + (size_t)blk * G.spec->SLAB + (G.spec->SLAB - n), sizeof(float) * n, h->stream);
    plat_sync(h->stream);
    return 0;
}
#endif

int pinn_group_timing(pinn_handle h, int group, float* ms, int64_t* points, int* channels, int* tiles) {
    if (!h) return fail("null handle");
    if (group < 0 || group >= (int)h->groups.size()) return fail("pinn_group_timing: group index out of range");
    Group& G = h->groups[group];
    if (ms) *ms = -1.f;
    if (G.timed) {
        plat_event_sync(G.ev_b);
        if (ms) *ms = plat_event_ms(G.ev_a, G.ev_b);
    }
    int64_t n = 0;
    for (int t : G.terms) n += h->terms[t].n;
    if (points) *points = n;
    if (channels) *channels = G.spec->C;
    if (tiles) *tiles = G.ga.ntiles;
    return 0;
}

int pinn_describe(pinn_handle h, char* buf, int64_t buflen) {
    if (!h || !buf || buflen <= 0) return fail("pinn_describe: bad argument");
    std::ostringstream os;
    os << "backend=" << plat_name() << " cus=" << h->ncu << " ntheta=" << h->ntheta << " terms=" << h->terms.size()
       << (h->f64 ? " precision=f64 (pinn_loss_grad*, pinn_lbfgs evaluate in double — matrix-pipe tile kernels where instantiated, one lane per point elsewhere; the plan below serves the fp32 entry points)" + pe::f64_describe(*h) : std::string())
       << (h->lbfgs ? " lbfgs=resident(history=" + std::to_string(h->lbfgs_history) + ",chunk=" + std::to_string(h->lbfgs_chunk) + ")" : std::string()) << "\n";
    for (size_t n = 0; n < h->netplans.size(); ++n)
        if (h->netplans[n].spec && h->netplans[n].spec->family != 3)
            os << "net " << n << " weights=packed image (k_pack per evaluation)"
               << " gemm=" << (h->netplans[n].spec->BFX ? (h->netplans[n].spec->BFX_DW ? "split-bf16(fwd,dA,dW)" : "split-bf16(fwd,dA)") : "fp32") << "\n";
    for (size_t g = 0; g < h->groups.size(); ++g) {
        const Group& G = h->groups[g];
        os << "group " << g << (G.kind == 1 ? (G.use_rec ? " [coupled fwd/gradin, records in HBM]" : " [coupled fwd/gradin]") :
                                (G.kind == 2 ? " [coupled tail: forward + tape + reverse in one launch]" : "")) << " net=" << G.net << " kernel=" << spec_name(*G.spec) << (G.ga.act == pk::ACT_SWISH ? "+swish" : "") << " tiles=" << G.ga.ntiles << " blocks=" << G.blocks << " terms=";
        for (int t : G.terms) {
            os << t;
            if (!h->terms[t].inodes.empty()) os << "+integral(" << h->terms[t].int_q << ")";
            os << ",";
        }
        if (G.chain_to >= 0) os << " slabs=" << (G.blocks <= h->groups[G.chain_to].blocks ? "chained onto group " : "own (more workgroups than group ") << G.chain_to << (G.blocks <= h->groups[G.chain_to].blocks ? "" : ")");
        if (G.merged >= 0 && h->merged[G.merged].tail == (int)g) os << " launch=merged into group " << h->merged[G.merged].head << "'s (one persistent kernel walks both tile lists)";
        os << "\n";
    }
    for (size_t t = 0; t < h->terms.size(); ++t) {
        const Term& T = h->terms[t];
        if (T.coupled >= 0) continue;
        os << "term " << t << ": tape ops=" << T.tape_ops.size() << " of " << T.ops.size() << ", sources=" << T.src_root.size()
           << " (" << T.src_prog.size() << " coordinate-only ops evaluated per point set)" << (T.linear ? ", affine residual: no tape interpreter" : "") << "\n";
    }
    std::string s = os.str();
    std::snprintf(buf, (size_t)buflen, "%s", s.c_str());
    return 0;
}

}

namespace {

template <class T> int loss_grad_twin(const char* who, pinn_handle h, const T* theta, int64_t p, const T* term_w, double* term_losses, T* grad) {
    if (!h || !theta) return fail(std::string(who) + ": null argument");
    pinn_engine& E = *h;
    if (check_theta(E, who, p)) return 1;
    DeviceScope scope(E.device);
    const size_t P = (size_t)p, K = E.terms.size();
    if (E.f64) {
        auto th = as<double>(theta, P); auto w = as<double>(term_w, K); auto g = as<double>(grad, P);
        return f64_eval(E, th.get(), w.get(), term_losses, g.get()) ? 1 : g.put();
    }
    auto th = as<float>(theta, P); auto w = as<float>(term_w, K); auto g = as<float>(grad, P);
    return loss_grad_f32(E, th.get(), w.get(), term_losses, g.get()) ? 1 : g.put();
}

template <class T> int loglik_twin(const char* who, pinn_handle h, const T* theta, int64_t p, const double* stds, double* loglik, T* grad_theta, double* grad_std) {
    if (!h || !theta || !stds || !loglik) return fail(std::string(who) + ": null argument");
    pinn_engine& E = *h;
    if (check_theta(E, who, p)) return 1;
    for (size_t k = 0; k < E.terms.size(); ++k)
        if (!(stds[k] > 0.0)) return fail(std::string(who) + ": standard deviations must be positive");
    DeviceScope scope(E.device);
    if (E.f64) {
        auto th = as<double>(theta, (size_t)p); auto g = as<double>(grad_theta, (size_t)p);
        return loglik_f64(E, th.get(), stds, loglik, g.get(), grad_std) ? 1 : g.put();
    }
    auto th = as<float>(theta, (size_t)p); auto g = as<float>(grad_theta, (size_t)p);
    return loglik_f32(E, th.get(), stds, loglik, g.get(), grad_std) ? 1 : g.put();
}

template <class T> int term_grads_twin(const char* who, pinn_handle h, const T* theta, int64_t p, double* term_losses, T* term_grads) {
    if (!h || !theta || !term_grads) return fail(std::string(who) + ": null argument");
    pinn_engine& E = *h;
    if (check_theta(E, who, p)) return 1;
    DeviceScope scope(E.device);
    const size_t P = (size_t)p, KP = E.terms.size() * P;
    if (E.f64) {
        auto th = as<double>(theta, P); auto g = as<double>(term_grads, KP);
        return term_grads_f64(E, th.get(), term_losses, g.get()) ? 1 : g.put();
    }
    auto th = as<float>(theta, P); auto g = as<float>(term_grads, KP);
    return term_grads_f32(E, th.get(), term_losses, g.get()) ? 1 : g.put();
}

template <class T> int residual_twin(const char* who, pinn_handle h, int term, const T* theta, int64_t p, T* r) {
    if (!h || !theta || !r) return fail(std::string(who) + ": null argument");
    pinn_engine& E = *h;
    if (term < 0 || term >= (int)E.terms.size()) return fail(std::string(who) + ": term index out of range");
    if (check_theta(E, who, p)) return 1;
    DeviceScope scope(E.device);
    const size_t P = (size_t)p, n = (size_t)E.terms[term].n;
    if (E.f64) {
        auto th = as<double>(theta, P); auto o = as<double>(r, n);
        return f64_residual(E, term, th.get(), o.get()) ? 1 : o.put();
    }
    auto th = as<float>(theta, P); auto o = as<float>(r, n);
    return residual_f32(E, term, th.get(), o.get()) ? 1 : o.put();
}

template <class T> int net_eval_twin(const char* who, pinn_handle h, int net, const T* theta, int64_t p, const T* pts, int64_t n, int order, const int* axes, T* out) {
    if (!h || !theta || !pts || !out) return fail(std::string(who) + ": null argument");
    pinn_engine& E = *h;
    if (net < 0 || net >= (int)E.nets.size()) return fail(std::string(who) + ": net index out of range");
    if (n <= 0) return fail(std::string(who) + ": n must be positive");
    if (order < 0 || order > MAX_DERIV_ORDER || (order > 0 && !axes)) return fail(std::string(who) + ": order must be 0..6 (with `order` axes)");
    const Net& N = E.nets[net];
// ... 495 lines not shown
```

### neuralpde.jl_amd/csrc/engine_types.hpp

```cpp
#pragma once
#include <algorithm>
#include <cmath>
#include <cstdio>
#include <cstdlib>
#include <map>
#include <memory>
#include <sstream>
#include <string>
#include <vector>

#include "../../include/pinn_hip.h"
#include "aux_limits.hpp"
#include "int_limits.hpp"
#include "plat.hpp"
#include "spec_registry.hpp"

namespace pe {

constexpr int REDUCE_SPLIT = 32;

extern thread_local std::string g_err;
int fail(const std::string& m);

constexpr int MAX_DERIV_ORDER = 6;
// ... 155 lines not shown
    const pk::PairInfo* pair = nullptr;
    float* d_scratch = nullptr;
    double* d_losspart = nullptr;
    int max_blocks = 0;
};
struct NetPlan {
    const pk::SpecInfo* spec = nullptr;
    float* d_packed = nullptr;
    int* d_pack_idx = nullptr;
    const float* cur = nullptr;
    std::vector<int> h_pack_idx;
    int npacked = 0;
};

}

using pe::Coupled; using pe::Group; using pe::MergedUnit; using pe::Net; using pe::NetPlan; using pe::Slot; using pe::Term;

struct pinn_engine {
    int64_t ntheta = 0;
    int np = 0, ne = 0, p_theta_off = 0;
    std::vector<float> p_defaults;
    std::vector<Net> nets;
    std::vector<Term> terms;
    std::vector<Term> terms0;
    void* f64 = nullptr;
    std::vector<Group> groups;
    std::vector<Coupled> coupled;
    std::vector<MergedUnit> merged;
    std::vector<NetPlan> netplans;
    int ncu = 0;
    int gemm = pk::GEMM_SPLIT;
    bool gemm_auto = false;
    double grad_health = -1.0;
    double gemm_delta = -1.0;
    long long gemm_check_t = -1;
    long long eval_count = 0;
    int device = 0;
    void* comm = nullptr;
    int comm_size = 1, comm_rank = 0;
    bool comm_per_process = false;
    pinn_allreduce_fn comm_fn = nullptr;
    void* comm_ctx = nullptr;
    plat_stream stream = nullptr;
    bool own_stream = true;
    float* d_theta = nullptr;
    float* d_params = nullptr;
    float* d_defaults = nullptr;
    double* d_lossraw = nullptr;
    int* d_gr_ptr = nullptr;
    int* d_gr_grp = nullptr;
    int* d_gr_ent = nullptr;
    int* d_red_perm = nullptr;
    float* d_out = nullptr;
    float* hp_theta = nullptr;
    float* hp_out = nullptr;
    double* hp_raw = nullptr;
    plat_event ev0, ev1, ev2, ev3;
    plat_stream aux_stream[2] = {nullptr, nullptr};
    plat_event ev_fork, ev_join[aux::MAX_GROUPS];
    float last_kernel_ms = 0.f, last_total_ms = 0.f;
    bool timing_valid = false;
    int timing_level = 0;
    int timing_group = -1;
    float* d_opt_theta = nullptr;
    float* d_opt_m = nullptr;
    float* d_opt_v = nullptr;
    float* d_opt_out = nullptr;
    float* d_w_over_n = nullptr;
    double* d_hist = nullptr;
    int hist_cap = 0;
    long long opt_t = 0;
    int* d_inv_ptr = nullptr;
    int* d_inv_pos = nullptr;
    bool inv_ok = false;
    int* d_step = nullptr;
    unsigned* d_draws = nullptr;
    int* d_sampled = nullptr;
    float* d_c12 = nullptr;
    int c12_cap = 0;
    unsigned* d_bar = nullptr;
    unsigned* h_flag = nullptr;
    unsigned bar_arrivals = 0;
    float* d_sums2 = nullptr;
    int* d_own_r = nullptr;
    int own_blocks = 0, hist_gid = 0;
    void* d_train_samp = nullptr;
    int train_samp_cap = 0;
    float* d_opt_bak = nullptr;
    int max_contrib = 0, max_inv_pos = 0;
    bool persistent = true;
    int eval_path = 0;
    int int_q = 16;
    double* d_int_xi = nullptr;
    float* d_int_w = nullptr;
    int adam_path = 0;
    float* d_phi_pts = nullptr;
    float* d_phi_out = nullptr;
    float* d_phi_scr = nullptr;
    size_t phi_scr_cap = 0;
    int64_t phi_cap = 0;
    int phi_chan = 0;
    void* hmc = nullptr;
    void* lbfgs = nullptr;
    int lbfgs_history = 0;
    int lbfgs_chunk = 8;
};

namespace pe {
int parse_descriptor(const char* text, pinn_engine& E);
int apply_embeddings(pinn_engine& E);
struct SexprContext {
    std::vector<std::string> params;
    std::vector<std::string> depvars;
    std::vector<std::vector<std::string>> depvar_inputs;
};
int lower_sexpr_term(const SexprContext& C, const std::vector<std::string>& indvars, const std::string& lhs, const std::string& rhs,
                     int np, Term& T);
void analyse_static(Term& T, int np);
bool fuse_laplacian(Term& T, int np);
int run_loss_grad(pinn_engine& E, const float* d_theta, float* d_out, const float* term_w, int only_term, bool timing, double* lossraw = nullptr,
                  bool packed_fresh = false, bool loss_only = false, float* d_sums = nullptr);
int upload_theta(pinn_engine& E, const float* theta, int64_t p);
void sums_from_double(float* d_out_sums, const double* d_raw, int K, plat_stream st);
int comm_all_reduce(pinn_engine** es, int ndev, float** vec, double** raw);
int comm_all_reduce_f64(pinn_engine** es, int ndev, double** vec, int64_t count);
struct DeviceScope {
    int prev;
    explicit DeviceScope(int dev) : prev(plat_get_device()) { if (prev != dev) plat_set_device(dev); else prev = -1; }
    ~DeviceScope() { if (prev >= 0) plat_set_device(prev); }
};
int f64_enable(pinn_engine& E);
void f64_destroy(pinn_engine& E);
std::string f64_describe(const pinn_engine& E);
int f64_affine_terms(const pinn_engine& E);
int f64_chunks(const pinn_engine& E);
int f64_merged(const pinn_engine& E);
const char* f64_path(const pinn_engine& E);
int f64_points_changed(pinn_engine& E, int term);
int f64_set_points(pinn_engine& E, int term, const double* pts, int64_t n);
int f64_set_point_data(pinn_engine& E, int term, const double* data);
int f64_eval(pinn_engine& E, const double* theta, const double* term_w, double* term_losses, double* grad);
int f64_residual(pinn_engine& E, int term, const double* theta, double* r);
int f64_net_eval(pinn_engine& E, int net, const double* theta, const double* pts, int64_t n, int order, const int* axes, double* out);
int f64_adam_apply(pinn_engine& E, const double* grad_and_sums, double lr, double beta1, double beta2, double eps, const float* term_w, double* loss);
int f64_stencil_enable(pinn_engine& E, bool on);
bool f64_stencil_on(const pinn_engine& E);
int f64_adam_init(pinn_engine& E, const double* theta);
int f64_adam_get(pinn_engine& E, double* theta);
int f64_adam_steps(pinn_engine& E, int nsteps, double lr, double beta1, double beta2, double eps, const float* term_w, double* loss_history,
                   void (*redraw)(pinn_engine&, pe::Term&));
int f64_points_from_device(pinn_engine& E, int term);
int f64_eval_from_device_f32(pinn_engine& E, const float* d_theta, const float* term_w, float* d_out, bool want_grad);
int f64_eval_from_device_f64(pinn_engine& E, const double* d_theta, const float* term_w, double* d_out);
double* f64_theta_buffer(pinn_engine& E);
int f64_eval_resident(pinn_engine& E, const double* term_w, double* d_out);
int f64_eval_sharded_local(pinn_engine& E, const double* theta, const double* term_w, double** d_out);
int f64_adam_steps_comm(pinn_engine** es, int ndev, int nsteps, double lr, double beta1, double beta2, double eps, const float* term_w, double* loss_history,
                        void (*redraw)(pinn_engine&, pe::Term&));
int current_gemm();
int current_act_hint();
struct GemmScope {
    int prev;
    explicit GemmScope(int mode);
    ~GemmScope();
};
int round_hp(int h);
const pk::SpecInfo* find_spec(int HP, int NHH, int D, unsigned need_first, const std::vector<std::pair<int, int>>& need_pairs,
                              unsigned need_hi, std::vector<int>* pair_index, int need_variant = 0, int need_family = 0);
int chan_of(const pk::SpecInfo& s, const Slot& sl);
const pk::SpecInfo* ensure_spec(const Net& N, unsigned need_first, const std::vector<std::pair<int, int>>& need_pairs, unsigned need_hi,
                                int need_family = 0);
int jit_round_hp(int h);
int jit_spec(int HP, int NHH, int D, unsigned D1MASK, unsigned long long PAIRS, int NPAIR, unsigned HI, int variant);
std::string jit_take_launch_error();
std::vector<unsigned> gen_close(const std::vector<unsigned>& want);
int jit_spec_gen(int HP, int NHH, int D, const std::vector<unsigned>& channels, int variant);
int jit_spec_dgm(int MP, int L, int D, unsigned D1MASK, unsigned long long PAIRS, int NPAIR, unsigned HI, const std::vector<unsigned>* gen_channels, int act1, int act2);
constexpr unsigned GEN_FLAG = 0x80000000u;
int gen_set_id(const std::vector<unsigned>& want);
const std::vector<unsigned>& gen_set(int id);
unsigned slot_mi(const Slot& s);
bool slot_is_general(const Slot& s);
inline int variant_of(int act) { return act == pk::ACT_SIN ? pk::VARIANT_SIN : (act == pk::ACT_MIXED ? pk::VARIANT_MIXED : (act == pk::ACT_SWISH ? pk::VARIANT_SWISH : 0)); }
std::string spec_name(const pk::SpecInfo& s);
int build_plan(pinn_engine& E);
void free_plan(pinn_engine& E);
void retile(pinn_engine& E, int gi);
}
```

### neuralpde.jl_amd/csrc/kernel_entry.hpp

```cpp
#pragma once
#include "pinn_kernels.hpp"
#include "pinn_kernels2.hpp"
#include "pinn_kernels3.hpp"
#include "pinn_train.hpp"
#ifdef __HIPCC_RTC__
typedef struct ihipStream_t* plat_stream;
#else
#include "plat.hpp"
#endif

namespace pk {

constexpr int MAX_GEN_CHANNELS = 24;

struct SpecInfo {
    int family;
    int WG_PER_CU;
    int WG_FWD;
    int NW;
    int HP, NHH, D;
    unsigned D1MASK;
    unsigned long long PAIRS;
    unsigned HI;
    unsigned LAP;
    int NPAIR, PG, C, NG, TP, MT, LH, NFIRST;
    int PACKED, SLAB, SCR, LDS_WG, COOP, SH, PW;
    int has_sin;
    int REC;
    int jit;
    int act1, act2, dgm_rows;
    int r_s, r_rec1, r_sr, r_dp1, r_dp, r_dpo, first_ch[8];
    int ngen;
    unsigned gen[MAX_GEN_CHANNELS];
    int OFF_W1, OFF_B, OFF_WL, OFF_BL, OFF_WPK, OFF_WTPK;
    int BFX_DW;
    int BFX, OFF_WB, OFF_WTB;
    int gemm;
    int twin;
    int O_WBAR, O_BFRH, O_BFR0, O_W1, O_WL, O_BL, O_P;
    void (*launch)(const GroupArgs&, int mode, int blocks, plat_stream);
    void (*train)(const GroupArgs&, const TrainArgs&, int blocks, plat_stream);
};

template <class S>
HD SpecInfo make_info(void (*launch)(const GroupArgs&, int, int, plat_stream), int has_sin = 0,
                      void (*train)(const GroupArgs&, const TrainArgs&, int, plat_stream) = nullptr) {
    SpecInfo s = {};
    s.train = train;
    s.has_sin = has_sin;
    s.jit = 0;
    s.act1 = s.act2 = s.dgm_rows = 0;
    s.ngen = S::J::GEN ? S::C : 0;
    for (int i = 0; i < MAX_GEN_CHANNELS; ++i) s.gen[i] = (S::J::GEN && i < S::C) ? S::J::gen_channel(i) : 0u;
    s.family = 1; s.WG_PER_CU = 1; s.WG_FWD = 1; s.NW = 4; s.gemm = GEMM_FP32; s.twin = 0; s.BFX = 0; s.BFX_DW = 0; s.OFF_WB = s.OFF_WTB = 0;
    s.HP = S::HP; s.NHH = S::NHH; s.D = S::D; s.D1MASK = S::D1MASK; s.PAIRS = S::PAIRS; s.NPAIR = S::NPAIR; s.HI = S::HI & 0xFFFFFFu; s.LAP = S::J::LAP;
    s.PG = S::PG; s.C = S::C; s.NG = S::NG; s.TP = S::TP; s.MT = S::MT; s.LH = S::LH; s.NFIRST = S::NFIRST;
    s.PACKED = S::PACKED; s.SLAB = S::SLAB; s.SCR = S::SCR; s.LDS_WG = S::LDS_WG; s.COOP = S::COOP ? 1 : 0; s.SH = S::SH; s.PW = S::PW;
    s.REC = 0;
    s.OFF_W1 = S::OFF_W1; s.OFF_B = S::OFF_B; s.OFF_WL = S::OFF_WL; s.OFF_BL = S::OFF_BL;
    s.OFF_WPK = S::OFF_WPK; s.OFF_WTPK = S::OFF_WTPK;
    s.O_WBAR = S::O_WBAR; s.O_BFRH = S::O_BFRH; s.O_BFR0 = S::O_BFR0; s.O_W1 = S::O_W1; s.O_WL = S::O_WL; s.O_BL = S::O_BL; s.O_P = S::O_P;
    s.launch = launch;
    return s;
}

template <class S>
HD SpecInfo make_info2(void (*launch)(const GroupArgs&, int, int, plat_stream), int has_sin = 0) {
    SpecInfo s = {};
    s.has_sin = has_sin;
    s.jit = 0;
    s.act1 = s.act2 = s.dgm_rows = 0;
    s.ngen = S::J::GEN ? S::C : 0;
    for (int i = 0; i < MAX_GEN_CHANNELS; ++i) s.gen[i] = (S::J::GEN && i < S::C) ? S::J::gen_channel(i) : 0u;
    s.family = 2; s.WG_PER_CU = S::WG_PER_CU; s.WG_FWD = S::WG_FWD; s.NW = S::NW; s.gemm = S::BFIMG ? GEMM_SPLIT : GEMM_FP32; s.twin = S::HAS_SPLIT ? 1 : 0;
    s.BFX = S::BFIMG ? 1 : 0; s.OFF_WB = S::OFF_WB; s.OFF_WTB = S::OFF_WTB; s.BFX_DW = S::DW_NATURAL ? 1 : 0;
    s.HP = S::HP; s.NHH = S::NHH; s.D = S::D; s.D1MASK = S::D1MASK; s.PAIRS = S::PAIRS; s.NPAIR = S::NPAIR; s.HI = S::HI & 0xFFFFFFu; s.LAP = S::J::LAP;
    s.PG = S::PG; s.C = S::C; s.NG = S::NG; s.TP = S::TP; s.MT = S::MT; s.LH = S::LH; s.NFIRST = S::NFIRST;
    s.PACKED = S::PACKED; s.SLAB = S::SLAB; s.SCR = S::SCR; s.LDS_WG = S::LDS_WG; s.COOP = 1; s.SH = S::SLAB; s.PW = 0;
    s.REC = S::REC;
    s.OFF_W1 = S::OFF_W1; s.OFF_B = S::OFF_B; s.OFF_WL = S::OFF_WL; s.OFF_BL = S::OFF_BL;
    s.OFF_WPK = S::OFF_WPK; s.OFF_WTPK = S::OFF_WTPK;
    s.O_WBAR = S::O_WBAR; s.O_BFRH = S::O_BH; s.O_BFR0 = S::O_BH; s.O_W1 = S::O_W1; s.O_WL = S::O_WL; s.O_BL = S::O_BL; s.O_P = S::O_P;
    s.launch = launch;
    return s;
}

template <class S>
HD SpecInfo make_info3(void (*launch)(const GroupArgs&, int, int, plat_stream)) {
    SpecInfo s = {};
    s.family = 3; s.WG_PER_CU = 8; s.WG_FWD = 8; s.NW = 1;
    s.HP = S::MP; s.NHH = S::L; s.D = S::D; s.D1MASK = S::D1MASK; s.PAIRS = S::PAIRS; s.NPAIR = S::NPAIR; s.HI = S::HI & 0xFFFFFFu; s.LAP = 0;
    s.PG = 4; s.C = S::C; s.NG = S::C; s.TP = 64; s.MT = 0; s.LH = S::L; s.NFIRST = S::NFIRST;
    s.COOP = 1;
    s.act1 = S::ACT1; s.act2 = S::ACT2; s.dgm_rows = S::ROWS;
    s.r_s = S::R_S; s.r_rec1 = S::R_REC1; s.r_sr = S::R_SR; s.r_dp1 = S::R_DP1; s.r_dp = S::R_DP; s.r_dpo = S::R_DPO;
    for (int i = 0; i < 8; ++i) {
        s.first_ch[i] = -1;
        for (int k = 0; k < S::NFIRST; ++k) if (S::J::first_axis(k) == i) s.first_ch[i] = S::J::CH_FIRST + k;
    }
    s.ngen = S::J::GEN ? S::C : 0;
    for (int i = 0; i < MAX_GEN_CHANNELS; ++i) s.gen[i] = (S::J::GEN && i < S::C) ? S::J::gen_channel(i) : 0u;
    s.launch = launch;
    return s;
}
#ifndef PINN_EMU
template <class S, int MODE, int ACTK>
__global__ void __launch_bounds__(256, 1) k_wave(const GroupArgs ga) {
    __shared__ __attribute__((aligned(16))) float lds_all[S::LDS_WG];
    const int w = __builtin_amdgcn_readfirstlane((int)(threadIdx.x >> 6));
    wave_main<S, MODE, ACTK>(ga, (int)blockIdx.x, (int)gridDim.x, w, lds_all);
}
template <class S, int ACTK>
__global__ void __launch_bounds__(256, 1) k_train(const GroupArgs ga, const TrainArgs ta) {
    __shared__ __attribute__((aligned(16))) float lds_all[S::LDS_WG];
    const int w = __builtin_amdgcn_readfirstlane((int)(threadIdx.x >> 6));
    wave_train<S, ACTK>(ga, ta, (int)blockIdx.x, (int)gridDim.x, w, lds_all);
}
template <class S, int MODE, int ACTK>
__global__ void __launch_bounds__(64 * S::NW, (mode_is_forward_only(MODE) ? S::OCC_FWD : S::OCC)) k_wave2(const GroupArgs ga) {
    __shared__ __attribute__((aligned(16))) float lds_all[mode_is_forward_only(MODE) ? S::LDS_FWD : S::LDS_WG];
    const int w = __builtin_amdgcn_readfirstlane((int)(threadIdx.x >> 6));
    wave_main2<S, MODE, ACTK>(ga, (int)blockIdx.x, (int)gridDim.x, w, lds_all);
}
template <class S0, class S1> struct Pair2 {
    static constexpr int WG_PER_CU = S0::WG_PER_CU < S1::WG_PER_CU ? S0::WG_PER_CU : S1::WG_PER_CU;
    static constexpr int LDS_WG = S0::LDS_WG > S1::LDS_WG ? S0::LDS_WG : S1::LDS_WG;
    static constexpr int SCR = S0::SCR > S1::SCR ? S0::SCR : S1::SCR;
    static constexpr int OCC = WG_PER_CU * S0::NW / 4;
    static constexpr int WG_FWD = S0::WG_FWD < S1::WG_FWD ? S0::WG_FWD : S1::WG_FWD;
    static constexpr int LDS_FWD = S0::LDS_FWD > S1::LDS_FWD ? S0::LDS_FWD : S1::LDS_FWD;
    static constexpr int OCC_FWD = WG_FWD * S0::NW / 4;
};
template <class S0, class S1, int ACTK, int MODE>
__global__ void __launch_bounds__(64 * S0::NW, (mode_is_forward_only(MODE) ? Pair2<S0, S1>::OCC_FWD : Pair2<S0, S1>::OCC)) k_wave2m(const GroupArgs ga) {
    __shared__ __attribute__((aligned(16))) float lds_all[mode_is_forward_only(MODE) ? Pair2<S0, S1>::LDS_FWD : Pair2<S0, S1>::LDS_WG];
    const int w = __builtin_amdgcn_readfirstlane((int)(threadIdx.x >> 6));
    wave_main2m<S0, S1, ACTK, MODE>(ga, (int)blockIdx.x, (int)gridDim.x, w, lds_all);
}
template <class S, int MODE>
__global__ void __launch_bounds__(64) k_dgm(const GroupArgs ga) { wave_dgm<S, MODE>(ga, (int)blockIdx.x, (int)gridDim.x); }
#endif

}
```

### neuralpde.jl_amd/csrc/pinn_kernels.hpp

```cpp
#pragma once
#include "rprog.hpp"
#include "vec.hpp"

#ifndef PINN_F1_PREFETCH
#define PINN_F1_PREFETCH 1
#endif
#ifndef PINN_F1_RESIDENT
#define PINN_F1_RESIDENT 3
#endif

namespace pk {
using namespace wv;

enum Act : int { ACT_TANH = 0, ACT_SIGMOID = 1, ACT_SIN = 2,
                 ACT_MIXED = 3 ,
                 ACT_SWISH = 4  };
constexpr int NUM_ACTS = 5;
enum ActClass : int { ACLS_A = 0 ,
                      ACLS_Z_SIN = 1 , ACLS_Z_SWISH = 2  };
constexpr int act_class(int actk) { return actk == ACT_SIN ? ACLS_Z_SIN : (actk == ACT_SWISH ? ACLS_Z_SWISH : ACLS_A); }
constexpr bool act_records_z(int acls) { return acls != ACLS_A; }
enum Variant : int { VARIANT_SIN = 1, VARIANT_MIXED = 2, VARIANT_SWISH = 4 };
enum Mode : int { MODE_FUSED = 0, MODE_RESID = 1, MODE_FWD = 2, MODE_GRADIN = 3, MODE_FWDREC = 4, MODE_GRADREC = 5, MODE_LOSS = 6 };
constexpr bool mode_is_forward_only(int mode) { return mode == MODE_RESID || mode == MODE_FWD || mode == MODE_FWDREC || mode == MODE_LOSS; }
// ... 62 lines not shown
        return 4u | (ax << 4) | (ax << 8) | (ax << 12) | (ax << 16);
    }
};

template <int HP_, int NHH_, int D_, unsigned D1MASK_, unsigned long long PAIRS_, int NPAIR_, int PG_, unsigned HI_ = 0>
struct Spec {
    using J = JetSet<D1MASK_, PAIRS_, NPAIR_, HI_>;
    static constexpr unsigned HI = HI_;
    static constexpr int HP = HP_;
    static constexpr int MT = HP_ / 16;
    static constexpr int NHH = NHH_;
    static constexpr int LH = NHH_ + 1;
    static constexpr int D = D_;
    static constexpr unsigned D1MASK = D1MASK_;
    static constexpr unsigned long long PAIRS = PAIRS_;
    static constexpr int NPAIR = NPAIR_;
    static constexpr int PG = PG_;
    static constexpr int NFIRST = J::NFIRST;
    static constexpr int C = J::C;
    static constexpr int NG = C * PG_;
    static constexpr int TP = 16 * PG_;
    static constexpr int first_axis(int k) { return J::first_axis(k); }
    static constexpr int first_rank(int axis) { return J::first_rank(axis); }
    static constexpr int pair_a(int p) { return J::pair_a(p); }
    static constexpr int pair_b(int p) { return J::pair_b(p); }
    static constexpr int OFF_W1 = 0;
    static constexpr int OFF_B = OFF_W1 + D_ * HP_;
    static constexpr int OFF_WL = OFF_B + LH * HP_;
    static constexpr int OFF_BL = OFF_WL + HP_;
    static constexpr int OFF_WPK = OFF_BL + 4;
    static constexpr int OFF_WTPK = OFF_WPK + NHH_ * HP_ * HP_;
    static constexpr int PACKED = OFF_WTPK + NHH_ * HP_ * HP_;
    static constexpr bool COOP = (MT == 4);
    static constexpr int WT = COOP ? 1 : MT;
    static constexpr int O_WBAR = 0;
    static constexpr int O_BFRH = NHH_ * HP_ * HP_;
    static constexpr int SH = COOP ? (NHH_ * HP_ * HP_ + NHH_ * HP_) : 0;
    static constexpr int PB = COOP ? 0 : (NHH_ * HP_ * HP_ + NHH_ * HP_);
    static constexpr int O_BFR0 = PB;
    static constexpr int O_W1 = O_BFR0 + HP_;
    static constexpr int O_WL = O_W1 + D_ * HP_;
    static constexpr int O_BL = O_WL + HP_;
    static constexpr int O_P = O_BL + 1;
    static constexpr int PW = ((O_P + MAX_PARAMS + 63) / 64) * 64;
    static constexpr int SLAB = SH + 4 * PW;
    static constexpr int SCR = LH * NG * MT * 256;
    static constexpr int LDS_T = (16 * HP_ > 1024) ? 16 * HP_ : 1024;
    static constexpr int LDS_X = ((16 * PG_ * D_ + 63) / 64) * 64;
    static constexpr int LDS_PRIV = 4 * LDS_T + LDS_X;
    static constexpr int LDS_SHARED = COOP ? 2 * 4 * 2 * LDS_T : 0;
    static constexpr int LDS_WG = LDS_SHARED + 4 * LDS_PRIV;
    static constexpr int WREGS = 2 * NHH_ * 4 * MT * MT;
    static constexpr int RREGS = NHH_ * NG * MT * 4;
    static constexpr int LIVE = 7 * NG * MT * 4 + NHH_ * WT * MT * 4 + (LH + D_ + 1) * MT * 4;
    static constexpr bool W_RESIDENT = (PINN_F1_RESIDENT & 1) && NHH_ > 0 && MT < 4 && LIVE + WREGS <= 400;
    static constexpr bool R_RESIDENT = (PINN_F1_RESIDENT & 2) && NHH_ > 0 && LIVE + (W_RESIDENT ? WREGS : 0) + RREGS <= 400;
};

struct TermDev {
    const float* pts;
    int N;
    int tile0;
    int ntiles;
    int prog_off;
    int nops;
    int out_row;
    int term_id;
    float scale;
    float* out;
    const float* in;
    const float* src;
    int nsrc;
    float* src_bar;
    int dt;
    int hetero;
    int imap[4];
    const float* pw;
    int linear;
    float lin_k;
    float lin_a[LIN_MAX_C];
    float lin_b[LIN_MAX_SRC];
};

struct GroupArgs {
    const float* packed;
    const float* params;
    const rp::Instr* prog;
    float* slabs;
    double* losspart;
    float* scratch;
    float* rec;
    int nterms_total;
    int nterms;
    int ntiles;
    int nparams;
    int nparams_estim;
    int act;
    int act_layers;
    int dgm_modes;
    int dgm_npad;
    int dgm_slab;
    int dgm_nparams;
    int chain;
    int sub_terms0, sub_tiles0;
    int scr_stride;
    TermDev terms[MAX_GROUP_TERMS];
};

template <class V> DEV V sig_poly6(V s) {
    return vfma(vfma(vfma(vfma(vfma(V(-720.0f), s, V(1800.0f)), s, V(-1560.0f)), s, V(540.0f)), s, V(-62.0f)), s, V(1.0f));
}
template <class V> DEV V sig_poly7(V s) {
    return vfma(vfma(vfma(vfma(vfma(vfma(V(5040.0f), s, V(-15120.0f)), s, V(16800.0f)), s, V(-8400.0f)), s, V(1806.0f)), s, V(-126.0f)), s, V(1.0f));
}
template <int NORD, int ACLS, bool MIXED = false, class V = vfloat>
DEV void act_derivs_n(int act, V a, V (&d)[ND]) {
    if (MIXED) {
        const float m = 2.0f - (float)act, im = 0.5f + 0.5f * (float)act, m2 = m * m;
        const V s = (a + V(m - 1.0f)) * V(im);
        const V s1 = s * (V(1.0f) - s);
        const V s2 = s1 * vfma(V(-2.0f), s, V(1.0f));
        const V s3 = s1 * vfma(V(-6.0f), s1, V(1.0f));
        d[1] = V(m2) * s1;
        d[2] = V(m2 * m) * s2;
        d[3] = V(m2 * m2) * s3;
        if (NORD >= 4) d[4] = V(m2 * m2 * m) * (s2 * vfma(V(-12.0f), s1, V(1.0f)));
        if (NORD >= 5) d[5] = V(m2 * m2 * m2) * vfma(s3, vfma(V(-12.0f), s1, V(1.0f)), V(-12.0f) * s2 * s2);
        if (NORD >= 6) d[6] = V(m2 * m2 * m2 * m) * s1 * sig_poly6(s);
        if (NORD >= 7) d[7] = V(m2 * m2 * m2 * m2) * s1 * sig_poly7(s);
        return;
    }
    if (ACLS == ACLS_Z_SWISH) {
        const V z = a, s = vsigmoid_fast(z);
        const V s1 = s * (V(1.0f) - s);
        const V s2 = s1 * vfma(V(-2.0f), s, V(1.0f));
        const V s3 = s1 * vfma(V(-6.0f), s1, V(1.0f));
        d[1] = vfma(z, s1, s);
        d[2] = vfma(z, s2, V(2.0f) * s1);
        d[3] = vfma(z, s3, V(3.0f) * s2);
        if (NORD >= 4) {
            const V q = vfma(V(-12.0f), s1, V(1.0f));
            const V s4 = s2 * q;
            d[4] = vfma(z, s4, V(4.0f) * s3);
            if (NORD >= 5) {
                const V s5 = vfma(s3, q, V(-12.0f) * s2 * s2);
                d[5] = vfma(z, s5, V(5.0f) * s4);
                if (NORD >= 6) {
                    const V s6 = s1 * sig_poly6(s);
                    d[6] = vfma(z, s6, V(6.0f) * s5);
                    if (NORD >= 7) d[7] = vfma(z, s1 * sig_poly7(s), V(7.0f) * s6);
                }
            }
        }
    } else if (ACLS == ACLS_Z_SIN) {
        V sn, cs;
        vsincos(a, sn, cs);
        d[1] = cs;
        d[2] = V(0.f) - sn;
        d[3] = V(0.f) - cs;
        if (NORD >= 4) d[4] = sn;
        if (NORD >= 5) d[5] = cs;
        if (NORD >= 6) d[6] = V(0.f) - sn;
        if (NORD >= 7) d[7] = V(0.f) - cs;
    } else if (act == ACT_TANH) {
        const V a2 = a * a;
        d[1] = vfma(-a, a, V(1.0f));
        d[2] = V(-2.0f) * a * d[1];
        d[3] = d[1] * vfma(V(6.0f), a2, V(-2.0f));
        if (NORD >= 4) d[4] = d[1] * a * vfma(V(-24.0f), a2, V(16.0f));
        if (NORD >= 5) d[5] = d[1] * (vfma(vfma(V(120.0f), a2, V(-120.0f)), a2, V(16.0f)));
        if (NORD >= 6) d[6] = d[1] * a * vfma(vfma(V(-720.0f), a2, V(960.0f)), a2, V(-272.0f));
        if (NORD >= 7) d[7] = d[1] * vfma(vfma(vfma(V(5040.0f), a2, V(-8400.0f)), a2, V(3696.0f)), a2, V(-272.0f));
    } else {
        d[1] = a * (V(1.0f) - a);
        d[2] = d[1] * vfma(V(-2.0f), a, V(1.0f));
        d[3] = d[1] * vfma(V(-6.0f), d[1], V(1.0f));
        if (NORD >= 4) d[4] = d[2] * vfma(V(-12.0f), d[1], V(1.0f));
        if (NORD >= 5) d[5] = vfma(d[3], vfma(V(-12.0f), d[1], V(1.0f)), V(-12.0f) * d[2] * d[2]);
        if (NORD >= 6) d[6] = d[1] * sig_poly6(a);
        if (NORD >= 7) d[7] = d[1] * sig_poly7(a);
    }
}
template <class J, class V>
DEV void jet_forward(V (&z)[J::C], const V (&d)[ND]) {
    PINN_UNROLL for (int k = 0; k < J::N4; ++k) {
        const int ax = J::hi_axis(4, k);
        const V z1 = z[J::CH_FIRST + J::first_rank(ax)], z2 = z[J::CH_PAIR + J::pair_index(ax, ax)], z3 = z[J::CH_3 + J::hi_rank(3, ax)];
        const V z11 = z1 * z1;
// ... 670 lines not shown
```

### neuralpde.jl_amd/csrc/pinn_kernels2.hpp

```cpp
#pragma once
#include "pinn_kernels.hpp"

#if defined(PINN_STAMP) && !defined(PINN_EMU)
#define STAMP_MEMBERS unsigned st_acc[24]; unsigned long long st_last;
#define STAMP_INIT(ac) { for (int i_ = 0; i_ < 24; ++i_) (ac).st_acc[i_] = 0; (ac).st_last = __builtin_amdgcn_s_memtime(); }
#define STAMP(i) { const unsigned long long st_now = __builtin_amdgcn_s_memtime(); ac.st_acc[i] += (unsigned)(st_now - ac.st_last); ac.st_last = st_now; }
#define STAMP_EXTRA 128
#else
#define STAMP_MEMBERS
#define STAMP_INIT(ac)
#define STAMP(i)
#define STAMP_EXTRA 0
#endif

#ifndef PINN_F2_REC_LDS
#define PINN_F2_REC_LDS 1
#endif
#ifndef PINN_F2_SWP
#define PINN_F2_SWP 7
#endif
#ifndef PINN_PROBE
#define PINN_PROBE 0
#endif
#ifndef PINN_F2_ADJ_IL
#define PINN_F2_ADJ_IL 1
#endif
#ifndef PINN_F2_TR_FWDIMG
#define PINN_F2_TR_FWDIMG 1
#endif
#ifndef PINN_F2_SPLIT_ACC2
#define PINN_F2_SPLIT_ACC2 1
#endif
#ifndef PINN_F2_WACC_PRELOAD
#define PINN_F2_WACC_PRELOAD 2
#endif
#ifndef PINN_F2_MODES
#define PINN_F2_MODES 3
#endif

namespace pk {

constexpr int GEMM_FP32 = 0, GEMM_SPLIT = 1;
constexpr int F2_WAVES128 = 8;
constexpr int F2_NW8_MAXNG = 6;
constexpr int F2_GEMM_AHEAD = 2;
constexpr int F2_SPRE_MAX = 24;


template <class A, class B> struct same_type { static constexpr bool value = false; };
template <class A> struct same_type<A, A> { static constexpr bool value = true; };
template <int HP_, int NHH_, int D_, int NW_, bool WBAR_REG_>
struct Shape2 {
    static constexpr int HP = HP_, MT = HP_ / 16, NHH = NHH_, LH = NHH_ + 1, D = D_, NW = NW_, MTW = MT / NW_;
    static constexpr bool WBAR_REG = WBAR_REG_;
};
template <class SH>
struct Acc2 {
    vfloat4 wbar[(SH::WBAR_REG && SH::NHH > 0) ? SH::NHH : 1][SH::MTW][SH::MT];
    vfloat4 bbar[SH::LH][SH::MTW];
    vfloat4 w1bar[SH::D][SH::MTW];
    vfloat4 wLbar[SH::MTW];
    vfloat bLbar;
    vfloat pbar[MAX_PARAMS];
    vdacc lsum;
    int cur_term;
    STAMP_MEMBERS
};

template <int HP_, int NHH_, int D_, unsigned D1MASK_, unsigned long long PAIRS_, int NPAIR_, int PG_, unsigned HI_ = 0, int GEMM_ = GEMM_SPLIT>
struct Spec2 {
    using J = JetSet<D1MASK_, PAIRS_, NPAIR_, HI_>;
    static constexpr unsigned HI = HI_;
    static constexpr int FAMILY = 2;
    static constexpr int GEMM = GEMM_;
    static constexpr int HP = HP_, MT = HP_ / 16, NHH = NHH_, LH = NHH_ + 1, D = D_, NPAIR = NPAIR_, PG = PG_;
    static constexpr unsigned D1MASK = D1MASK_;
    static constexpr unsigned long long PAIRS = PAIRS_;
    static constexpr int NW = (HP_ >= 128 && J::C * PG_ <= F2_NW8_MAXNG) ? F2_WAVES128 : 4;
    static constexpr int MTW = MT / NW;
    static_assert(MT % NW == 0 && MT % 4 == 0, "family 2 needs a hidden width that is a multiple of 64 (16 x waves per workgroup)");
    static constexpr int NFIRST = J::NFIRST;
    static constexpr int C = J::C;
    static constexpr int NG = C * PG_;
    static constexpr int TP = 16 * PG_;
// ... 1045 lines not shown
DEV void acc2_store(Acc2<typename S::Shape>& ac, const GroupArgs& ga, int blk, int w, float* lds) {
    constexpr int HP = S::HP, MT = S::MT, MTW = S::MTW, NHH = S::NHH, LH = S::LH, D = S::D, NG = S::NG;
    const vint lane = lane_id();
    const vint g = lane >> 4;
    const vint c = lane & vint(15);
    float* slab = ga.slabs + (size_t)blk * S::SLAB;
    float* UP = lds + S::OFF_UP;
    if (S::WBAR_REG)
        PINN_UNROLL for (int hl = 0; hl < NHH; ++hl)
            PINN_UNROLL for (int t = 0; t < MTW; ++t)
                PINN_UNROLL for (int ti = 0; ti < MT; ++ti)
                    gstore4(slab + S::O_WBAR, vint((((hl * MT + w * MTW + t) * MT + ti) * 64) * 4) + (lane << 2), ac.wbar[hl][t][ti]);
    const vbool c0 = veq(c, 0);
    auto reduce_cols = [&](vfloat v) -> vfloat {
        v = row_allsum16(v);
        return v;
    };
    PINN_UNROLL for (int t = 0; t < MTW; ++t)
        PINN_UNROLL for (int r = 0; r < 4; ++r) {
            const vint n = vint(16 * (w * MTW + t) + r) + (g << 2);
            PINN_UNROLL for (int l = 0; l < LH; ++l) gstore_masked(slab + S::O_BH + l * HP, n, reduce_cols(ac.bbar[l][t][r]), c0);
            PINN_UNROLL for (int i = 0; i < D; ++i) gstore_masked(slab + S::O_W1 + i * HP, n, reduce_cols(ac.w1bar[i][t][r]), c0);
            gstore_masked(slab + S::O_WL, n, reduce_cols(ac.wLbar[t][r]), c0);
        }
    static_assert(4 * MAX_PARAMS <= 16, "UB holds the per-wave parameter partials");
    const vbool all = vlt(lane, 64);
    float* UBp = UP + S::NW * NG * 16;
    if (w > 0 && w < PG)
        PINN_UNROLL for (int j = 0; j < MAX_PARAMS; ++j)
            lds_store(UBp, vint(w * MAX_PARAMS + j) + (lane & vint(0)), vfloat((float)wave_sum_d(ac.pbar[j], all)));
    if (PG > 1) wg_barrier();
    if (w == 0) {
        float s = (float)wave_sum_d(ac.bLbar, all);
        gstore_masked(slab + S::O_BL, vint(0), vfloat(s), veq(lane, 0));
        PINN_UNROLL for (int j = 0; j < MAX_PARAMS; ++j) {
            vfloat sp = vfloat((float)wave_sum_d(ac.pbar[j], all));
            PINN_UNROLL for (int ws = 1; ws < PG; ++ws) sp = sp + lds_load(UBp, vint(ws * MAX_PARAMS + j) + (lane & vint(0)));
            gstore_masked(slab + S::O_P, vint(j), sp, veq(lane, 0));
        }
    }
#if defined(PINN_STAMP) && !defined(PINN_EMU)
    STAMP(14)
    if ((threadIdx.x & 63) == 0)
        for (int i = 0; i < 24; ++i) reinterpret_cast<unsigned*>(slab + S::SLAB - 128)[w * 24 + i] = ac.st_acc[i];
#endif
}

template <class S, int MODE, int ACTK>
DEV void wave_main2(const GroupArgs& ga, int blk, int nblocks, int w, float* lds) {
    constexpr bool BWD = (MODE == MODE_FUSED || MODE == MODE_GRADIN || MODE == MODE_GRADREC);
    constexpr bool SUMS = (MODE == MODE_FUSED || MODE == MODE_LOSS);
    const int wave = blk * S::NW + w;
    Acc2<typename S::Shape> ac;
    acc2_init<S>(ac, ga, blk, w, BWD);
    if (SUMS)
        for (int j = 0; j < ga.nterms; ++j) ga.losspart[(size_t)wave * ga.nterms_total + ga.terms[j].term_id] = 0.0;
    wave_tiles2<S, MODE, ACTK>(ga, blk, nblocks, w, lds, ac, 0, ga.nterms, 0, ga.ntiles);
    if (SUMS && ac.cur_term >= 0)
        ga.losspart[(size_t)wave * ga.nterms_total + ga.terms[ac.cur_term].term_id] = wave_sum_dd(ac.lsum, veq(lane_id() >> 4, 0));
    if (!BWD) return;
    acc2_store<S>(ac, ga, blk, w, lds);
}

template <class S0, class S1, int ACTK, int MODE = MODE_FUSED>
DEV void wave_main2m(const GroupArgs& ga, int blk, int nblocks, int w, float* lds) {
    static_assert(same_type<typename S0::Shape, typename S1::Shape>::value, "merged launches need members of one network shape and neuron split");
    static_assert(S0::SLAB == S1::SLAB && S0::PACKED == S1::PACKED, "merged launches share the slab and the packed weight image");
    static_assert(S0::DW_NATURAL == S1::DW_NATURAL && S0::BFX_TR == S1::BFX_TR, "merged launches: one order of the dW tiles in the slab, one exchange-image layout");
    static_assert(MODE == MODE_FUSED || MODE == MODE_LOSS, "merged launches: the fused evaluation and the loss-only evaluation");
    const int wave = blk * S0::NW + w;
    Acc2<typename S0::Shape> ac;
    acc2_init<S0>(ac, ga, blk, w, MODE == MODE_FUSED);
    for (int j = 0; j < ga.nterms; ++j) ga.losspart[(size_t)wave * ga.nterms_total + ga.terms[j].term_id] = 0.0;
    wave_tiles2<S0, MODE, ACTK>(ga, blk, nblocks, w, lds, ac, 0, ga.sub_terms0, 0, ga.sub_tiles0);
    wg_barrier();
    wave_tiles2<S1, MODE, ACTK>(ga, blk, nblocks, w, lds, ac, ga.sub_terms0, ga.nterms, ga.sub_tiles0, ga.ntiles);
    if (ac.cur_term >= 0)
        ga.losspart[(size_t)wave * ga.nterms_total + ga.terms[ac.cur_term].term_id] = wave_sum_dd(ac.lsum, veq(lane_id() >> 4, 0));
    if (MODE != MODE_FUSED) return;
    wg_barrier();
    acc2_store<S0, (S0::PG > S1::PG ? S0::PG : S1::PG)>(ac, ga, blk, w, lds);
}

}
```

### neuralpde.jl_amd/csrc/spec_registry.hpp

```cpp
#pragma once
#include <condition_variable>
#include <cstring>
#include <deque>
#include <mutex>
#include <thread>
#include <vector>

#include "plat.hpp"
#include "kernel_entry.hpp"

namespace pk {

std::deque<SpecInfo>& registry();

struct PairInfo {
    SpecInfo a, b;
    int WG_PER_CU, NW, LDS_WG, SCR;
    int WG_FWD;
    void (*launch)(const GroupArgs&, int mode , int blocks, plat_stream);
};
std::deque<PairInfo>& pair_registry();

#ifdef PINN_EMU
struct EmuBarrier {
    std::mutex m;
    std::condition_variable cv;
    int count = 0, gen = 0, nwaves = 4;
    static void wait(void* p) {
        EmuBarrier* b = (EmuBarrier*)p;
        std::unique_lock<std::mutex> lk(b->m);
        const int g = b->gen;
        if (++b->count == b->nwaves) { b->count = 0; ++b->gen; b->cv.notify_all(); }
        else b->cv.wait(lk, [&] { return b->gen != g; });
    }
};
template <class S, int MODE, int ACTK>
void run_emu(const GroupArgs& ga, int blocks) {
    std::vector<float> lds((size_t)S::LDS_WG);
    for (int b = 0; b < blocks; ++b) {
        std::fill(lds.begin(), lds.end(), 0.f);
        EmuBarrier bar;
        std::thread th[4];
        for (int w = 0; w < 4; ++w)
            th[w] = std::thread([&, w] {
                wv::emu_barrier_hook = &EmuBarrier::wait;
                wv::emu_barrier_ctx = &bar;
                wave_main<S, MODE, ACTK>(ga, b, blocks, w, lds.data());
            });
        for (int w = 0; w < 4; ++w) th[w].join();
    }
}
template <class S, int ACTK>
void run_emu_train(const GroupArgs& ga, const TrainArgs& ta, int blocks) {
    std::vector<std::vector<float>> lds((size_t)blocks, std::vector<float>((size_t)S::LDS_WG, 0.f));
    std::vector<EmuBarrier> bars((size_t)blocks);
    EmuBarrier grid;
    grid.nwaves = 4 * blocks;
    std::vector<std::thread> th;
    for (int b = 0; b < blocks; ++b)
        for (int w = 0; w < 4; ++w)
            th.emplace_back([&, b, w] {
                wv::emu_barrier_hook = &EmuBarrier::wait;
                wv::emu_barrier_ctx = &bars[(size_t)b];
                wv::emu_grid_hook = &EmuBarrier::wait;
                wv::emu_grid_ctx = &grid;
                wave_train<S, ACTK>(ga, ta, b, blocks, w, lds[(size_t)b].data());
            });
    for (auto& t : th) t.join();
}
template <class S, int MODE, int ACTK>
void run_emu2(const GroupArgs& ga, int blocks) {
    std::vector<float> lds((size_t)S::LDS_WG);
    for (int b = 0; b < blocks; ++b) {
        for (auto& v : lds) v = std::nanf("");
        EmuBarrier bar;
        bar.nwaves = S::NW;
        std::thread th[S::NW];
        for (int w = 0; w < S::NW; ++w)
            th[w] = std::thread([&, w] {
                wv::emu_barrier_hook = &EmuBarrier::wait;
                wv::emu_barrier_ctx = &bar;
                wave_main2<S, MODE, ACTK>(ga, b, blocks, w, lds.data());
            });
        for (int w = 0; w < S::NW; ++w) th[w].join();
    }
}
template <class S0, class S1, int ACTK, int MODE>
void run_emu2m(const GroupArgs& ga, int blocks) {
    std::vector<float> lds((size_t)(S0::LDS_WG > S1::LDS_WG ? S0::LDS_WG : S1::LDS_WG));
    for (int b = 0; b < blocks; ++b) {
        for (auto& v : lds) v = std::nanf("");
        EmuBarrier bar;
        bar.nwaves = S0::NW;
        std::thread th[S0::NW];
        for (int w = 0; w < S0::NW; ++w)
            th[w] = std::thread([&, w] {
                wv::emu_barrier_hook = &EmuBarrier::wait;
                wv::emu_barrier_ctx = &bar;
                wave_main2m<S0, S1, ACTK, MODE>(ga, b, blocks, w, lds.data());
            });
        for (int w = 0; w < S0::NW; ++w) th[w].join();
    }
}
#define PINN_LAUNCH2(S, MODE, ACTK, ga, blocks, st) run_emu2<S, MODE, ACTK>(ga, blocks)
#define PINN_LAUNCH2M(S0, S1, ACTK, MODE, ga, blocks, st) run_emu2m<S0, S1, ACTK, MODE>(ga, blocks)
#define PINN_LAUNCH1(S, MODE, ACTK, ga, blocks, st) run_emu<S, MODE, ACTK>(ga, blocks)
#define PINN_LAUNCH_TRAIN(S, ACTK, ga, ta, blocks, st) run_emu_train<S, ACTK>(ga, ta, blocks)
#else
#define PINN_LAUNCH2(S, MODE, ACTK, ga, blocks, st) hipLaunchKernelGGL((k_wave2<S, MODE, ACTK>), dim3(blocks), dim3(64 * S::NW), 0, st, ga)
#define PINN_LAUNCH2M(S0, S1, ACTK, MODE, ga, blocks, st) hipLaunchKernelGGL((k_wave2m<S0, S1, ACTK, MODE>), dim3(blocks), dim3(64 * S0::NW), 0, st, ga)
#define PINN_LAUNCH1(S, MODE, ACTK, ga, blocks, st) hipLaunchKernelGGL((k_wave<S, MODE, ACTK>), dim3(blocks), dim3(256), 0, st, ga)
#define PINN_LAUNCH_TRAIN(S, ACTK, ga, ta, blocks, st) hipLaunchKernelGGL((k_train<S, ACTK>), dim3(blocks), dim3(256), 0, st, ga, ta)
#endif

template <class S, int ACTK>
void launch_modes2(const GroupArgs& ga, int mode, int blocks, plat_stream st) {
    (void)st;
    if (mode == MODE_FUSED) PINN_LAUNCH2(S, MODE_FUSED, ACTK, ga, blocks, st);
    else if (mode == MODE_RESID) PINN_LAUNCH2(S, MODE_RESID, ACTK, ga, blocks, st);
    else if (mode == MODE_GRADIN) PINN_LAUNCH2(S, MODE_GRADIN, ACTK, ga, blocks, st);
    else if (mode == MODE_FWDREC) PINN_LAUNCH2(S, MODE_FWDREC, ACTK, ga, blocks, st);
    else if (mode == MODE_GRADREC) PINN_LAUNCH2(S, MODE_GRADREC, ACTK, ga, blocks, st);
    else if (mode == MODE_LOSS) PINN_LAUNCH2(S, MODE_LOSS, ACTK, ga, blocks, st);
    else PINN_LAUNCH2(S, MODE_FWD, ACTK, ga, blocks, st);
}
template <class S, int ACTK>
void launch_modes1(const GroupArgs& ga, int mode, int blocks, plat_stream st) {
    (void)st;
    if (mode == MODE_FUSED) PINN_LAUNCH1(S, MODE_FUSED, ACTK, ga, blocks, st);
    else if (mode == MODE_RESID) PINN_LAUNCH1(S, MODE_RESID, ACTK, ga, blocks, st);
    else if (mode == MODE_GRADIN) PINN_LAUNCH1(S, MODE_GRADIN, ACTK, ga, blocks, st);
    else if (mode == MODE_LOSS) PINN_LAUNCH1(S, MODE_LOSS, ACTK, ga, blocks, st);
    else PINN_LAUNCH1(S, MODE_FWD, ACTK, ga, blocks, st);
}
template <class S> void launch_spec2(const GroupArgs& ga, int mode, int blocks, plat_stream st) {
    if (ga.act == ACT_TANH) launch_modes2<S, ACT_TANH>(ga, mode, blocks, st); else launch_modes2<S, ACT_SIGMOID>(ga, mode, blocks, st);
}
template <class S> void launch_spec(const GroupArgs& ga, int mode, int blocks, plat_stream st) {
    if (ga.act == ACT_TANH) launch_modes1<S, ACT_TANH>(ga, mode, blocks, st); else launch_modes1<S, ACT_SIGMOID>(ga, mode, blocks, st);
}
template <class S> void launch_train(const GroupArgs& ga, const TrainArgs& ta, int blocks, plat_stream st) {
    (void)st;
    static_assert(sizeof(GroupArgs) + sizeof(TrainArgs) <= 4096, "kernel arguments of k_train");
    if (ga.act == ACT_TANH) PINN_LAUNCH_TRAIN(S, ACT_TANH, ga, ta, blocks, st); else PINN_LAUNCH_TRAIN(S, ACT_SIGMOID, ga, ta, blocks, st);
}
template <class S0, class S1> void launch_pair2(const GroupArgs& ga, int mode, int blocks, plat_stream st) {
    (void)st;
    if (mode == MODE_LOSS) {
        if (ga.act == ACT_TANH) PINN_LAUNCH2M(S0, S1, ACT_TANH, MODE_LOSS, ga, blocks, st); else PINN_LAUNCH2M(S0, S1, ACT_SIGMOID, MODE_LOSS, ga, blocks, st);
    } else {
        if (ga.act == ACT_TANH) PINN_LAUNCH2M(S0, S1, ACT_TANH, MODE_FUSED, ga, blocks, st); else PINN_LAUNCH2M(S0, S1, ACT_SIGMOID, MODE_FUSED, ga, blocks, st);
    }
}
template <class S, int VARIANTS> void launch_spec2_var(const GroupArgs& ga, int mode, int blocks, plat_stream st) {
    if constexpr ((VARIANTS & VARIANT_SIN) != 0) if (ga.act == ACT_SIN) return launch_modes2<S, ACT_SIN>(ga, mode, blocks, st);
    if constexpr ((VARIANTS & VARIANT_SWISH) != 0) if (ga.act == ACT_SWISH) return launch_modes2<S, ACT_SWISH>(ga, mode, blocks, st);
    launch_spec2<S>(ga, mode, blocks, st);
}
template <class S, int VARIANTS> void launch_spec_var(const GroupArgs& ga, int mode, int blocks, plat_stream st) {
    if constexpr ((VARIANTS & VARIANT_SIN) != 0) if (ga.act == ACT_SIN) return launch_modes1<S, ACT_SIN>(ga, mode, blocks, st);
    if constexpr ((VARIANTS & VARIANT_MIXED) != 0) if (ga.act == ACT_MIXED) return launch_modes1<S, ACT_MIXED>(ga, mode, blocks, st);
    if constexpr ((VARIANTS & VARIANT_SWISH) != 0) if (ga.act == ACT_SWISH) return launch_modes1<S, ACT_SWISH>(ga, mode, blocks, st);
    launch_spec<S>(ga, mode, blocks, st);
}


inline DgmDwArgs dgm_dw_args(const GroupArgs& ga, const SpecInfo& s, int blocks) {
    DgmDwArgs a;
    std::memset(&a, 0, sizeof a);
    a.scratch = ga.scratch; a.slabs = ga.slabs; a.npad = ga.dgm_npad; a.slab = ga.dgm_slab; a.nblocks = blocks; a.ntiles = ga.ntiles;
    a.M = ga.dgm_modes; a.MPad = s.HP; a.d = s.D; a.L = s.NHH; a.C = s.C; a.nparams = ga.dgm_nparams;
    a.r_s = s.r_s; a.r_rec1 = s.r_rec1; a.r_sr = s.r_sr; a.r_dp1 = s.r_dp1; a.r_dp = s.r_dp; a.r_dpo = s.r_dpo;
    for (int i = 0; i < 8; ++i) a.first_ch[i] = s.first_ch[i];
    a.nterms = ga.nterms;
    for (int j = 0; j < MAX_GROUP_TERMS; ++j) a.terms[j] = ga.terms[j];
    return a;
}
#ifdef PINN_EMU
template <class S, int MODE> void run_emu3(const GroupArgs& ga, int blocks) {
    for (int b = 0; b < blocks; ++b) wave_dgm<S, MODE>(ga, b, blocks);
}
inline void run_dgm_dw(const DgmDwArgs& a, plat_stream) {
    for (int b = 0; b < a.nblocks; ++b)
        for (int e = 0; e < a.nparams; ++e) dgm_dw_entry(e, b, a);
}
#define PINN_LAUNCH3(S, MODE, ga, blocks, st) run_emu3<S, MODE>(ga, blocks)
#else
template <int UNUSED>
__global__ void __launch_bounds__(256) k_dgm_dw(const DgmDwArgs a) {
    const int e = (int)(blockIdx.x * 256 + threadIdx.x);
    if (e < a.nparams) dgm_dw_entry(e, (int)blockIdx.y, a);
}
inline void run_dgm_dw(const DgmDwArgs& a, plat_stream st) {
    hipLaunchKernelGGL((k_dgm_dw<0>), dim3((a.nparams + 255) / 256, a.nblocks), dim3(256), 0, st, a);
}
#define PINN_LAUNCH3(S, MODE, ga, blocks, st) hipLaunchKernelGGL((k_dgm<S, MODE>), dim3(blocks), dim3(64), 0, st, ga)
#endif
template <class S> SpecInfo& info3_of();
template <class S> void launch_spec3(const GroupArgs& ga, int mode, int blocks, plat_stream st) {
    (void)st;
    if (mode == MODE_FUSED) {
        PINN_LAUNCH3(S, MODE_FUSED, ga, blocks, st);
        run_dgm_dw(dgm_dw_args(ga, info3_of<S>(), blocks), st);
    } else if (mode == MODE_RESID) PINN_LAUNCH3(S, MODE_RESID, ga, blocks, st);
    else if (mode == MODE_LOSS) PINN_LAUNCH3(S, MODE_LOSS, ga, blocks, st);
    else PINN_LAUNCH3(S, MODE_FWD, ga, blocks, st);
}

struct Registrar {
    explicit Registrar(const SpecInfo& s) { registry().push_back(s); }
};
template <class S0, class S1>
PairInfo make_pair_info() {
    PairInfo p;
    p.a = make_info2<S0>(nullptr);
    p.b = make_info2<S1>(nullptr);
    p.WG_PER_CU = S0::WG_PER_CU < S1::WG_PER_CU ? S0::WG_PER_CU : S1::WG_PER_CU;
    p.NW = S0::NW;
    p.LDS_WG = S0::LDS_WG > S1::LDS_WG ? S0::LDS_WG : S1::LDS_WG;
    p.SCR = S0::SCR > S1::SCR ? S0::SCR : S1::SCR;
    p.WG_FWD = S0::WG_FWD < S1::WG_FWD ? S0::WG_FWD : S1::WG_FWD;
    p.launch = &launch_pair2<S0, S1>;
    return p;
}

#define PINN_PAIR(p, a, b) (((unsigned long long)((a) | ((b) << 4))) << (8 * (p)))

#define PINN_HI(axis, order) ((unsigned)(order) << (4 * (axis)))
#define PINN_LAP(mask) ((unsigned)(mask) << 24)
#if PINN_F2_MODES & 1
#define PINN_F2_IF_SPLIT(...) __VA_ARGS__
#else
#define PINN_F2_IF_SPLIT(...)
#endif
#if PINN_F2_MODES & 2
#define PINN_F2_IF_FP32(...) __VA_ARGS__
#else
#define PINN_F2_IF_FP32(...)
#endif
#ifndef PINN_F1_TRAIN
#define PINN_F1_TRAIN 1
#endif
#if PINN_F1_TRAIN
#define PINN_TRAIN_OF(S) (&pk::launch_train<S>)
#else
#define PINN_TRAIN_OF(S) nullptr
#endif
template <class S> struct Launch2Plain { static void fn(const GroupArgs& ga, int mode, int blocks, plat_stream st) { launch_spec2<S>(ga, mode, blocks, st); } };
template <class S> struct Launch2Sin { static void fn(const GroupArgs& ga, int mode, int blocks, plat_stream st) { launch_spec2_var<S, VARIANT_SIN>(ga, mode, blocks, st); } };
template <class S> struct Launch2Swish { static void fn(const GroupArgs& ga, int mode, int blocks, plat_stream st) { launch_spec2_var<S, VARIANT_SWISH>(ga, mode, blocks, st); } };
template <class S> struct Launch2SinSwish { static void fn(const GroupArgs& ga, int mode, int blocks, plat_stream st) { launch_spec2_var<S, VARIANT_SIN | VARIANT_SWISH>(ga, mode, blocks, st); } };
template <class S, template <class> class L, bool ENABLE> struct Registrar2 {
    explicit Registrar2(int has_sin) { registry().push_back(make_info2<S>(&L<S>::fn, has_sin)); }
};
template <class S, template <class> class L> struct Registrar2<S, L, false> { explicit Registrar2(int) {} };
template <class S0, class S1, bool ENABLE> struct PairRegistrar2 { PairRegistrar2() { pair_registry().push_back(make_pair_info<S0, S1>()); } };
template <class S0, class S1> struct PairRegistrar2<S0, S1, false> { PairRegistrar2() {} };
#define PINN_F2_FP32_ENABLED(S) (S::HAS_SPLIT || !(PINN_F2_MODES & 1))
#define PINN_INSTANTIATE2_ANY(NAME, LAUNCH, VARIANT, HP, NHH, D, D1MASK, PAIRS, NPAIR, PG, HI)                                   \
    namespace {                                                                                                                  \
    PINN_F2_IF_SPLIT(using NAME##_spec2 = pk::Spec2<HP, NHH, D, D1MASK, PAIRS, NPAIR, PG, HI, pk::GEMM_SPLIT>;                    \
                     pk::Registrar2<NAME##_spec2, pk::LAUNCH, true> NAME##_reg2(VARIANT);)                                       \
    PINN_F2_IF_FP32(using NAME##_spec2f = pk::Spec2<HP, NHH, D, D1MASK, PAIRS, NPAIR, PG, HI, pk::GEMM_FP32>;                     \
                    pk::Registrar2<NAME##_spec2f, pk::LAUNCH, PINN_F2_FP32_ENABLED(NAME##_spec2f)> NAME##_reg2f(VARIANT);)       \
    }
#define PINN_INSTANTIATE2_HI(NAME, HP, NHH, D, D1MASK, PAIRS, NPAIR, PG, HI) PINN_INSTANTIATE2_ANY(NAME, Launch2Plain, 0, HP, NHH, D, D1MASK, PAIRS, NPAIR, PG, HI)
#define PINN_INSTANTIATE_HI(NAME, HP, NHH, D, D1MASK, PAIRS, NPAIR, PG, HI)                  \
    namespace {                                                                              \
    using NAME##_spec = pk::Spec<HP, NHH, D, D1MASK, PAIRS, NPAIR, PG, HI>;                  \
    pk::Registrar NAME##_reg(pk::make_info<NAME##_spec>(&pk::launch_spec<NAME##_spec>, 0, PINN_TRAIN_OF(NAME##_spec))); \
    }
#define PINN_INSTANTIATE_HI_VAR(NAME, VARIANTS, HP, NHH, D, D1MASK, PAIRS, NPAIR, PG, HI)    \
    namespace {                                                                              \
    using NAME##_spec = pk::Spec<HP, NHH, D, D1MASK, PAIRS, NPAIR, PG, HI>;                  \
    pk::Registrar NAME##_reg(pk::make_info<NAME##_spec>(&pk::launch_spec_var<NAME##_spec, (VARIANTS)>, (VARIANTS), PINN_TRAIN_OF(NAME##_spec))); \
    }
#define PINN_INSTANTIATE2_HI_SIN(NAME, HP, NHH, D, D1MASK, PAIRS, NPAIR, PG, HI) PINN_INSTANTIATE2_ANY(NAME, Launch2Sin, pk::VARIANT_SIN, HP, NHH, D, D1MASK, PAIRS, NPAIR, PG, HI)
#define PINN_INSTANTIATE2_HI_SWISH(NAME, HP, NHH, D, D1MASK, PAIRS, NPAIR, PG, HI) PINN_INSTANTIATE2_ANY(NAME, Launch2Swish, pk::VARIANT_SWISH, HP, NHH, D, D1MASK, PAIRS, NPAIR, PG, HI)
#define PINN_INSTANTIATE2_HI_SIN_SWISH(NAME, HP, NHH, D, D1MASK, PAIRS, NPAIR, PG, HI) PINN_INSTANTIATE2_ANY(NAME, Launch2SinSwish, pk::VARIANT_SIN | pk::VARIANT_SWISH, HP, NHH, D, D1MASK, PAIRS, NPAIR, PG, HI)
#define PINN_INSTANTIATE_HI_SIN(NAME, HP, NHH, D, D1MASK, PAIRS, NPAIR, PG, HI) PINN_INSTANTIATE_HI_VAR(NAME, pk::VARIANT_SIN, HP, NHH, D, D1MASK, PAIRS, NPAIR, PG, HI)
#define PINN_INSTANTIATE_HI_SWISH(NAME, HP, NHH, D, D1MASK, PAIRS, NPAIR, PG, HI) PINN_INSTANTIATE_HI_VAR(NAME, pk::VARIANT_SWISH, HP, NHH, D, D1MASK, PAIRS, NPAIR, PG, HI)
#define PINN_INSTANTIATE_HI_SIN_SWISH(NAME, HP, NHH, D, D1MASK, PAIRS, NPAIR, PG, HI) PINN_INSTANTIATE_HI_VAR(NAME, pk::VARIANT_SIN | pk::VARIANT_SWISH, HP, NHH, D, D1MASK, PAIRS, NPAIR, PG, HI)
#define PINN_INSTANTIATE_HI_MIX(NAME, HP, NHH, D, D1MASK, PAIRS, NPAIR, PG, HI) PINN_INSTANTIATE_HI_VAR(NAME, pk::VARIANT_MIXED, HP, NHH, D, D1MASK, PAIRS, NPAIR, PG, HI)
#define PINN_INSTANTIATE_DGM(NAME, MP, L, D, D1MASK, PAIRS, NPAIR, HI, ACT1, ACT2)           \
    namespace pk {                                                                           \
    using NAME##_spec3 = Spec3<MP, L, D, D1MASK, PAIRS, NPAIR, HI, ACT1, ACT2>;              \
    template <> SpecInfo& info3_of<NAME##_spec3>() { static SpecInfo s = make_info3<NAME##_spec3>(&launch_spec3<NAME##_spec3>); return s; } \
    }                                                                                        \
    namespace {                                                                              \
    pk::Registrar NAME##_reg3(pk::info3_of<pk::NAME##_spec3>());                             \
    }
#define PINN_INSTANTIATE2_PAIR(NAME, HP, NHH, D, D1MASK_A, PAIRS_A, NPAIR_A, PG_A, HI_A, D1MASK_B, PAIRS_B, NPAIR_B, PG_B, HI_B) \
    namespace {                                                                              \
    PINN_F2_IF_SPLIT(using NAME##_pa = pk::Spec2<HP, NHH, D, D1MASK_A, PAIRS_A, NPAIR_A, PG_A, HI_A, pk::GEMM_SPLIT>;  \
                     using NAME##_pb = pk::Spec2<HP, NHH, D, D1MASK_B, PAIRS_B, NPAIR_B, PG_B, HI_B, pk::GEMM_SPLIT>;  \
                     pk::PairRegistrar2<NAME##_pa, NAME##_pb, true> NAME##_regp;)            \
    PINN_F2_IF_FP32(using NAME##_paf = pk::Spec2<HP, NHH, D, D1MASK_A, PAIRS_A, NPAIR_A, PG_A, HI_A, pk::GEMM_FP32>;   \
                    using NAME##_pbf = pk::Spec2<HP, NHH, D, D1MASK_B, PAIRS_B, NPAIR_B, PG_B, HI_B, pk::GEMM_FP32>;   \
                    pk::PairRegistrar2<NAME##_paf, NAME##_pbf, PINN_F2_FP32_ENABLED(NAME##_paf)> NAME##_regpf;)        \
    }
#define PINN_INSTANTIATE2(NAME, HP, NHH, D, D1MASK, PAIRS, NPAIR, PG) PINN_INSTANTIATE2_HI(NAME, HP, NHH, D, D1MASK, PAIRS, NPAIR, PG, 0u)
#define PINN_INSTANTIATE(NAME, HP, NHH, D, D1MASK, PAIRS, NPAIR, PG) PINN_INSTANTIATE_HI(NAME, HP, NHH, D, D1MASK, PAIRS, NPAIR, PG, 0u)

}
```

### neuralpde.jl_amd/csrc/vec.hpp

```cpp
#pragma once
#ifndef __HIPCC_RTC__
#include <cmath>
#include <cstdint>
#include <cstring>
#include <type_traits>
#endif

#ifdef PINN_EMU
#define DEV inline
#define HD inline
#define PINN_UNROLL
namespace wv {
constexpr int W = 64;
struct vbool { bool v[W]; };
struct vint {
    int v[W];
    vint() {}
    vint(int s) { for (int l = 0; l < W; ++l) v[l] = s; }
};
struct vfloat {
    float v[W];
    vfloat() {}
    vfloat(float s) { for (int l = 0; l < W; ++l) v[l] = s; }
};
// ... 358 lines not shown
}
DEV void keep_alive(const vfloat4& x) {
    if (PINN_STORE_PAD > 0) asm volatile("" ::"v"(x[0]), "v"(x[1]), "v"(x[2]), "v"(x[3]));
}
template <int NGROUPS, int MFMA_PER, int AHEAD, int DS_PER = 1> DEV void sched_gemm_prefetch() {
    __builtin_amdgcn_sched_group_barrier(0x100, AHEAD * DS_PER, 0);
    PINN_UNROLL for (int i = 0; i < NGROUPS - AHEAD; ++i) {
        __builtin_amdgcn_sched_group_barrier(0x008, MFMA_PER, 0);
        __builtin_amdgcn_sched_group_barrier(0x100, DS_PER, 0);
    }
    __builtin_amdgcn_sched_group_barrier(0x008, MFMA_PER * AHEAD, 0);
}
template <int P> DEV void wave_prio_t() { __builtin_amdgcn_s_setprio(P); }
#define wave_prio(P) wave_prio_t<P>()
struct urec16 { int x, y, z, w; };
DEV urec16 uload16(const void* p) {
    typedef int i4 __attribute__((ext_vector_type(4)));
    const unsigned long long a = (unsigned long long)p;
    const unsigned lo = (unsigned)__builtin_amdgcn_readfirstlane((int)(unsigned)a);
    const unsigned hi = (unsigned)__builtin_amdgcn_readfirstlane((int)(unsigned)(a >> 32));
    const unsigned long long u = (unsigned long long)lo | ((unsigned long long)hi << 32);
    const i4 v = *(const __attribute__((address_space(4))) i4*)u;
    return {v.x, v.y, v.z, v.w};
}
struct urec32 { int v[8]; };
DEV urec32 uload32(const void* p) {
    typedef int i8 __attribute__((ext_vector_type(8)));
    const unsigned long long a = (unsigned long long)p;
    const unsigned lo = (unsigned)__builtin_amdgcn_readfirstlane((int)(unsigned)a);
    const unsigned hi = (unsigned)__builtin_amdgcn_readfirstlane((int)(unsigned)(a >> 32));
    const unsigned long long u = (unsigned long long)lo | ((unsigned long long)hi << 32);
    const i8 v = *(const __attribute__((address_space(4))) i8*)u;
    return {{v[0], v[1], v[2], v[3], v[4], v[5], v[6], v[7]}};
}
struct ubuf { __amdgpu_buffer_rsrc_t r; };
typedef unsigned vuint4 __attribute__((ext_vector_type(4)));
DEV ubuf ub_make(const float* p, size_t nfloats) {
    return ubuf{__builtin_amdgcn_make_buffer_rsrc(const_cast<float*>(p), 0, (int)(nfloats * 4), 0x00020000)};
}
DEV vfloat4 ub_load4(ubuf b, int soff, vint voff) {
    return __builtin_bit_cast(vfloat4, __builtin_amdgcn_raw_buffer_load_b128(b.r, voff * 4, soff * 4, 0));
}
DEV vfloat4 ub_load4_sc1(ubuf b, int soff, vint voff) {
    return __builtin_bit_cast(vfloat4, __builtin_amdgcn_raw_buffer_load_b128(b.r, voff * 4, soff * 4, 16));
}
DEV void ub_store4(ubuf b, int soff, vint voff, vfloat4 x) {
    __builtin_amdgcn_raw_buffer_store_b128(__builtin_bit_cast(vuint4, x), b.r, voff * 4, soff * 4, 0);
}
DEV vfloat ub_load(ubuf b, int soff, vint voff) {
    return __builtin_bit_cast(float, __builtin_amdgcn_raw_buffer_load_b32(b.r, voff * 4, soff * 4, 0));
}
template <int AUX> DEV double ub_loadd(ubuf b, int soff, vint voff) {
    return __builtin_bit_cast(double, __builtin_amdgcn_raw_buffer_load_b64(b.r, voff * 8, soff * 8, AUX));
}
template <int AUX> DEV float ub_loadf(ubuf b, int soff, vint voff) {
    return __builtin_bit_cast(float, __builtin_amdgcn_raw_buffer_load_b32(b.r, voff * 4, soff * 4, AUX));
}
DEV void opaque_v(int& x) { asm volatile("" : "+v"(x)); }
DEV void opaque_s(int& x) { asm volatile("" : "+s"(x)); }
DEV vfloat ub_load_sc1(ubuf b, int soff, vint voff) {
    return __builtin_bit_cast(float, __builtin_amdgcn_raw_buffer_load_b32(b.r, voff * 4, soff * 4, 16));
}
DEV void ub_store4_wt(ubuf b, vint voff, vfloat4 x) {
    __builtin_amdgcn_raw_buffer_store_b128(__builtin_bit_cast(vuint4, x), b.r, voff * 4, 0, 16);
}
DEV void gstore_masked_wt(float* p, vint i, vfloat x, vbool m) { if (m) __hip_atomic_store(p + i, x, __ATOMIC_RELAXED, __HIP_MEMORY_SCOPE_AGENT); }
DEV void ustore_wt(double* p, double x) { __hip_atomic_store(p, x, __ATOMIC_RELAXED, __HIP_MEMORY_SCOPE_AGENT); }
DEV void ustore_wt(float* p, float x) { __hip_atomic_store(p, x, __ATOMIC_RELAXED, __HIP_MEMORY_SCOPE_AGENT); }
DEV float uload_wt(const float* p) { return __hip_atomic_load(p, __ATOMIC_RELAXED, __HIP_MEMORY_SCOPE_AGENT); }
DEV double uload_wt(const double* p) { return __hip_atomic_load(p, __ATOMIC_RELAXED, __HIP_MEMORY_SCOPE_AGENT); }
DEV vfloat lds_load(const float* p, vint i) { return p[i]; }
DEV void lds_store(float* p, vint i, vfloat x) { p[i] = x; }
DEV vfloat4 lds_load4(const float* p, vint i) { return *reinterpret_cast<const vfloat4*>(p + i); }
DEV void lds_store4(float* p, vint i, vfloat4 x) { *reinterpret_cast<vfloat4*>(p + i) = x; }
DEV void wave_fence() {
    __builtin_amdgcn_fence(__ATOMIC_RELEASE, "wavefront");
    __builtin_amdgcn_wave_barrier();
    __builtin_amdgcn_fence(__ATOMIC_ACQUIRE, "wavefront");
}
#ifndef PINN_PROBE
#define PINN_PROBE 0
#endif
DEV void wg_barrier() { if (!(PINN_PROBE & 4)) __syncthreads(); }
DEV void grid_barrier(unsigned* bar, unsigned target) {
    asm volatile("s_waitcnt vmcnt(0)" ::: "memory");
    __syncthreads();
    if (threadIdx.x == 0) {
        if (__hip_atomic_load(bar + 1, __ATOMIC_RELAXED, __HIP_MEMORY_SCOPE_AGENT) == 0u) {
            __builtin_amdgcn_fence(__ATOMIC_RELEASE, "agent");
            asm volatile("s_waitcnt vmcnt(0)" ::: "memory");
            __hip_atomic_fetch_add(bar, 1u, __ATOMIC_RELAXED, __HIP_MEMORY_SCOPE_AGENT);
            unsigned spins = 0;
            while ((int)(__hip_atomic_load(bar, __ATOMIC_RELAXED, __HIP_MEMORY_SCOPE_AGENT) - target) < 0) {
                __builtin_amdgcn_s_sleep(1);
                if (++spins > (1u << 21)) { __hip_atomic_store(bar + 1, 1u, __ATOMIC_RELAXED, __HIP_MEMORY_SCOPE_AGENT); break; }
            }
            __builtin_amdgcn_fence(__ATOMIC_ACQUIRE, "agent");
        }
    }
    __syncthreads();
}
DEV void grid_barrier_wt(unsigned* bar, unsigned target) {
    asm volatile("s_waitcnt vmcnt(0)" ::: "memory");
    __syncthreads();
    if (threadIdx.x == 0) {
        if (__hip_atomic_load(bar + 1, __ATOMIC_RELAXED, __HIP_MEMORY_SCOPE_AGENT) == 0u) {
            __hip_atomic_fetch_add(bar, 1u, __ATOMIC_RELAXED, __HIP_MEMORY_SCOPE_AGENT);
            unsigned spins = 0;
            while ((int)(__hip_atomic_load(bar, __ATOMIC_RELAXED, __HIP_MEMORY_SCOPE_AGENT) - target) < 0) {
                __builtin_amdgcn_s_sleep(1);
                if (++spins > (1u << 21)) { __hip_atomic_store(bar + 1, 1u, __ATOMIC_RELAXED, __HIP_MEMORY_SCOPE_AGENT); break; }
            }
        }
    }
    __syncthreads();
}
DEV vfloat shfl_xor(vfloat a, int m) { return __shfl_xor(a, m, 64); }
template <int CTRL> DEV float dpp_mov(float v) {
    return __builtin_bit_cast(float, __builtin_amdgcn_update_dpp(0, __builtin_bit_cast(int, v), CTRL, 0xF, 0xF, false));
}
DEV vfloat row_allsum16(vfloat v) {
    v += dpp_mov<0x128>(v); v += dpp_mov<0x124>(v); v += dpp_mov<0x122>(v); v += dpp_mov<0x121>(v);
    return v;
}
DEV vfloat xrow_allsum(vfloat v) {
    float a = v, b = v;
    asm volatile("s_nop 1\n\tv_permlane16_swap_b32 %0, %1\n\ts_nop 1" : "+v"(a), "+v"(b));
    float s = a + b, t = s;
    asm volatile("s_nop 1\n\tv_permlane32_swap_b32 %0, %1\n\ts_nop 1" : "+v"(s), "+v"(t));
    return s + t;
}
DEV float lane0(vfloat a) { return __builtin_bit_cast(float, __builtin_amdgcn_readfirstlane(__builtin_bit_cast(int, a))); }
DEV double wave_sum_d(vfloat a, vbool m) {
    double s = m ? (double)a : 0.0;
    PINN_UNROLL for (int o = 32; o >= 1; o >>= 1) s += __shfl_xor(s, o, 64);
    return s;
}
using vdacc = double;
DEV vdacc vdacc_zero() { return 0.0; }
DEV vdacc vdacc_fma(vfloat a, vfloat b, vdacc c) { return __builtin_fma((double)a, (double)b, c); }
DEV double wave_sum_dd(vdacc a, vbool m) {
    double s = m ? a : 0.0;
    PINN_UNROLL for (int o = 32; o >= 1; o >>= 1) s += __shfl_xor(s, o, 64);
    return s;
}
DEV vfloat4 mfma16(vfloat a, vfloat b, vfloat4 c) { return __builtin_amdgcn_mfma_f32_16x16x4f32(a, b, c, 0, 0, 0); }
DEV vfloat4 vzero4() { return vfloat4{0.f, 0.f, 0.f, 0.f}; }
typedef __bf16 vbf4 __attribute__((ext_vector_type(4)));
typedef __bf16 vbf8 __attribute__((ext_vector_type(8)));
#ifndef PINN_SPLIT_PK
#define PINN_SPLIT_PK 1
#endif
typedef __bf16 vbf2_ __attribute__((ext_vector_type(2)));
DEV void split3_bf16(vfloat4 x, vbf4& h, vbf4& m, vbf4& l) {
#if PINN_SPLIT_PK
    PINN_UNROLL for (int q = 0; q < 2; ++q) {
        const vfloat2_ xx = {x[2 * q], x[2 * q + 1]};
        const vbf2_ hb = __builtin_convertvector(xx, vbf2_);
        const vfloat2_ r = xx - __builtin_convertvector(hb, vfloat2_);
        const vbf2_ mb = __builtin_convertvector(r, vbf2_);
        const vfloat2_ r2 = r - __builtin_convertvector(mb, vfloat2_);
        const vbf2_ lb = __builtin_convertvector(r2, vbf2_);
        h[2 * q] = hb[0]; h[2 * q + 1] = hb[1];
        m[2 * q] = mb[0]; m[2 * q + 1] = mb[1];
        l[2 * q] = lb[0]; l[2 * q + 1] = lb[1];
    }
#else
    PINN_UNROLL for (int k = 0; k < 4; ++k) {
        const __bf16 hb = (__bf16)x[k];
        const float r = x[k] - (float)hb;
        const __bf16 mb = (__bf16)r;
        const float r2 = r - (float)mb;
        h[k] = hb; m[k] = mb; l[k] = (__bf16)r2;
    }
#endif
}
DEV void split1_bf16(vfloat4 x, vbf4& h) { PINN_UNROLL for (int k = 0; k < 4; ++k) h[k] = (__bf16)x[k]; }
DEV void lds_store_bf4(float* p, vint i, vbf4 x) { *reinterpret_cast<vbf4*>(p + i) = x; }
DEV vbf8 lds_load_bf8(const float* p, vint i) { return *reinterpret_cast<const vbf8*>(p + i); }
#ifndef PINN_F2_LDS_NOMERGE
#define PINN_F2_LDS_NOMERGE 1
#endif
DEV vbf4 lds_load_bf4(const float* p, vint i) {
#if PINN_F2_LDS_NOMERGE
// ... 95 lines not shown
```

Before: 239.9 million.

## Fuse final gradient/loss reduction into persistent fused kernel via grid barrier

Adds a tail to the fused forward/backward kernel. After a grid-wide barrier, the resident workgroups perform the slab and loss-part reduction themselves, so the separate k_reduce_one launch is no longer needed. The tail is gated on a single network, one or two groups, and occupancy confirming that all workgroups are co-resident. A host-visible timeout flag falls back to the stand-alone reduction kernel and reruns the evaluation. This removes one kernel launch and its dependency gap, at the cost of a grid barrier spin and some extra complexity.

```diff
diff --git a/neuralpde.jl_amd/csrc/aux_kernels.hpp b/neuralpde.jl_amd/csrc/aux_kernels.hpp
--- a/neuralpde.jl_amd/csrc/aux_kernels.hpp
+++ b/neuralpde.jl_amd/csrc/aux_kernels.hpp
@@ -1,6 +1,7 @@
 #pragma once
 #include <cstdlib>
 #include "aux_limits.hpp"
+#include "reduce_one.hpp"
 #include "int_limits.hpp"
 #include "plat.hpp"
 #include "rprog.hpp"
@@ -8,14 +9,6 @@
 #include "sample_rules.hpp"
 
 namespace aux {
-
-#ifdef PINN_EMU
-#define AUX_DEV inline
-#else
-#define AUX_DEV __device__ __forceinline__
-#endif
-
-struct alignas(16) F4 { float x, y, z, w; };
 
 struct Reduce1Args {
     double* tmp[MAX_GROUPS];
@@ -39,20 +32,6 @@
     int skip_grad;
     const int* perm;
 };
-struct ReduceOneArgs {
-    const float* slabs;
-    int slab, nblocks, nent;
-    const int* ent_theta;
-    float* out;
-    float* sums;
-    double* lossraw;
-    int P, K;
-    int nloss;
-    const double* losspart[MAX_GROUPS];
-    int nrows[MAX_GROUPS];
-};
-constexpr int RONE_CHUNKS = 32, RONE_ENT = 32;
-
 struct ExprArgs {
     const float* pts;
     int N, d, nparams, nparams_estim;
@@ -361,11 +340,6 @@
 AUX_DEV void params_body(int j, float* params, const float* theta, const float* defaults, int ne, int p_off) {
     params[j] = (j < ne) ? theta[p_off + j] : defaults[j];
 }
-#ifdef PINN_EMU
-#define AUX_UNROLL8
-#else
-#define AUX_UNROLL8 _Pragma("unroll 8")
-#endif
 AUX_DEV void reduce1_body(int e4, int chunk, int g, const Reduce1Args& a) {
     if (!a.active[g] || chunk >= a.nsplit[g]) return;
     const int nb = a.nblocks[g], ns = a.nsplit[g];
@@ -391,23 +365,6 @@
         for (int wv = b0 * a.nwpb[g]; wv < b1 * a.nwpb[g]; ++wv) s += p[(size_t)wv * a.K];
         out[(size_t)(a.nent[g] + k) * ns] = s;
     }
-}
-AUX_DEV void reduce_one_chunk(int e4, int ch, const ReduceOneArgs& a, double (&s)[4]) {
-    const int per = (a.nblocks + RONE_CHUNKS - 1) / RONE_CHUNKS;
-    const int b0 = ch * per, b1 = (b0 + per < a.nblocks) ? b0 + per : a.nblocks;
-    s[0] = s[1] = s[2] = s[3] = 0.0;
-    const float* p = a.slabs + 4 * e4;
-    AUX_UNROLL8
-    for (int b = b0; b < b1; ++b) {
-        const F4 q = *reinterpret_cast<const F4*>(p + (size_t)b * a.slab);
-        s[0] += (double)q.x; s[1] += (double)q.y; s[2] += (double)q.z; s[3] += (double)q.w;
-    }
-}
-AUX_DEV double reduce_one_loss_part(int k, int t, int nthreads, const ReduceOneArgs& a) {
-    double s = 0.0;
-    for (int i = 0; i < a.nloss; ++i)
-        for (int r = t; r < a.nrows[i]; r += nthreads) s += a.losspart[i][(size_t)r * a.K + k];
-    return s;
 }
 AUX_DEV void reduce2_body(int r, const Reduce2Args& a) {
     if (r < a.P) {
@@ -576,24 +533,8 @@
         }
 }
 inline void launch_reduce_one(const ReduceOneArgs& a, plat_stream) {
-    for (int e4 = 0; e4 < a.nent / 4; ++e4) {
-        double tot[4] = {0, 0, 0, 0}, s[4];
-        for (int ch = 0; ch < RONE_CHUNKS; ++ch) {
-            reduce_one_chunk(e4, ch, a, s);
-            for (int e = 0; e < 4; ++e) tot[e] += s[e];
-        }
-        for (int e = 0; e < 4; ++e)
-            if (a.ent_theta[4 * e4 + e] >= 0) a.out[a.ent_theta[4 * e4 + e]] = (float)tot[e];
-    }
-    for (int k = 0; k < a.K; ++k) {
-        double part[256], s = 0.0;
-        for (int t = 0; t < 256; ++t) part[t] = reduce_one_loss_part(k, t, 256, a);
-        for (int st = 128; st >= 1; st >>= 1)
-            for (int t = 0; t < st; ++t) part[t] += part[t + st];
-        s = part[0];
-        a.sums[k] = (float)s;
-        if (a.lossraw) a.lossraw[k] = s;
-    }
+    double sh[RONE_SH];
+    for (int u = 0; u < reduce_one_units(a); ++u) reduce_one_unit_host(u, a, sh, false);
 }
 inline void launch_reduce(const Reduce1Args& a1, const Reduce2Args& a2, int max_n1, int max_split, plat_stream) {
     if (reduce_is_small(a1, a2)) {
@@ -773,38 +714,21 @@
     hipLaunchKernelGGL(k_int_expr, dim3(nblocks), dim3(256), 0, st, a);
 }
 __global__ void __launch_bounds__(256) k_reduce_one(const ReduceOneArgs a) {
-    __shared__ double sh[RONE_CHUNKS][RONE_ENT + 1];
-    const int tid = (int)threadIdx.x;
-    const int nentblocks = (a.nent + RONE_ENT - 1) / RONE_ENT;
-    if ((int)blockIdx.x < nentblocks) {
-        const int j = tid & 7, ch = tid >> 3;
-        const int e4 = (int)blockIdx.x * (RONE_ENT / 4) + j;
-        double s[4] = {0.0, 0.0, 0.0, 0.0};
-        if (4 * e4 < a.nent) reduce_one_chunk(e4, ch, a, s);
-        for (int e = 0; e < 4; ++e) sh[ch][4 * j + e] = s[e];
+    __shared__ double sh[RONE_SH];
+    const int tid = (int)threadIdx.x, u = (int)blockIdx.x;
+    const int nentblocks = reduce_one_nentblocks(a);
+    if (u < nentblocks) {
+        reduce_one_ent_chunks(u, tid, a, sh);
         __syncthreads();
-        if (tid < RONE_ENT) {
-            const int ent = (int)blockIdx.x * RONE_ENT + tid;
-            if (ent < a.nent) {
-                double tot = 0.0;
-                for (int c2 = 0; c2 < RONE_CHUNKS; ++c2) tot += sh[c2][tid];
-                const int th = a.ent_theta[ent];
-                if (th >= 0) a.out[th] = (float)tot;
-            }
-        }
+        reduce_one_ent_total(u, tid, a, sh, false);
     } else {
-        const int k = (int)blockIdx.x - nentblocks;
-        double* part = &sh[0][0];
-        part[tid] = reduce_one_loss_part(k, tid, 256, a);
+        reduce_one_loss_parts(u - nentblocks, tid, a, sh);
         __syncthreads();
         for (int st = 128; st >= 1; st >>= 1) {
-            if (tid < st) part[tid] += part[tid + st];
+            reduce_one_loss_tree(st, tid, sh);
             __syncthreads();
         }
-        if (tid == 0) {
-            a.sums[k] = (float)part[0];
-            if (a.lossraw) a.lossraw[k] = part[0];
-        }
+        reduce_one_loss_out(u - nentblocks, tid, a, sh, false);
     }
 }
 inline void launch_reduce_one(const ReduceOneArgs& a, plat_stream st) {
diff --git a/neuralpde.jl_amd/csrc/comm.cpp b/neuralpde.jl_amd/csrc/comm.cpp
--- a/neuralpde.jl_amd/csrc/comm.cpp
+++ b/neuralpde.jl_amd/csrc/comm.cpp
@@ -322,7 +322,11 @@
     plat_stream st = (plat_stream)stream;
     plat_stream saved = E.stream;
     E.stream = st;
-    int rc = run_loss_grad(E, d_theta, d_out, term_w, -1, true);
+    int rc;
+    {
+        SingleScope single(E);
+        rc = run_loss_grad(E, d_theta, d_out, term_w, -1, true);
+    }
     E.stream = saved;
     if (rc) return rc;
     E.timing_valid = E.timing_level >= 2;
diff --git a/neuralpde.jl_amd/csrc/engine.cpp b/neuralpde.jl_amd/csrc/engine.cpp
--- a/neuralpde.jl_amd/csrc/engine.cpp
+++ b/neuralpde.jl_amd/csrc/engine.cpp
@@ -226,6 +226,51 @@
     return p == E.ntheta ? 0 : fail(std::string(who) + ": theta length " + std::to_string(p) + " != ntheta " + std::to_string(E.ntheta));
 }
 
+}
+
+static void single_timed_out(pinn_engine& E) {
+    E.h_sl_flag[0] = 0;
+    E.single_off = true;
+    std::fprintf(stderr, "[pinn] the fused kernel's grid barrier timed out (its workgroups were not all resident: is the device shared?); "
+                         "this handle continues with the stand-alone reduction kernel\n");
+}
+bool pe::single_check_timeout(pinn_engine& E) {
+    if (!E.single_last || E.single_off) return false;
+    if (!(E.h_sl_flag && E.h_sl_flag[0]) && std::getenv("PINN_SINGLE_FORCE_TIMEOUT") == nullptr) return false;
+    single_timed_out(E);
+    return true;
+}
+static int single_tail_group(pinn_engine& E, bool loss_only, int only_term, bool concurrent, bool may_merge) {
+    E.single_last = 0;
+    if (E.h_sl_flag && E.h_sl_flag[0]) single_timed_out(E);
+    if (!E.single_allow || E.single_off || loss_only || only_term >= 0 || concurrent || !E.coupled.empty() || E.nets.size() != 1 || E.np != 0) return -1;
+    if (std::getenv("PINN_NO_SINGLE_LAUNCH") || std::getenv("PINN_NO_REDUCE_ONE")) return -1;
+    const size_t ng = E.groups.size();
+    if (ng != 1 && ng != 2) return -1;
+    for (auto& G : E.groups) if (G.kind != 0 || !G.spec) return -1;
+    int head = 0;
+    const pk::PairInfo* pair = nullptr;
+    if (ng == 2) {
+        if (!may_merge || E.groups[0].merged < 0 || E.groups[1].merged != E.groups[0].merged) return -1;
+        head = E.merged[E.groups[0].merged].head;
+        pair = E.merged[E.groups[0].merged].pair;
+    }
+    const Group& H = E.groups[(size_t)head];
+    if (H.spec->family != 2 || !H.spec->BFX || !H.d_ent_theta || !H.ent_covers_theta) return -1;
+    if (E.single_resident < 0) {
+        auto q = pair ? pair->resident_fused : H.spec->resident_fused;
+        E.single_resident = q ? q(H.ga.act) : 0;
+        const int planned = pair ? pair->WG_PER_CU : H.spec->WG_PER_CU;
+        if (E.single_resident < planned) { E.single_off = true; return -1; }
+        E.d_sl_bar = (unsigned*)plat_malloc(sizeof(unsigned) * 4);
+        E.h_sl_flag = (unsigned*)plat_host_alloc(sizeof(unsigned) * 4);
+        if (!E.d_sl_bar || !E.h_sl_flag) { E.single_off = true; return -1; }
+        E.h_sl_flag[0] = 0;
+        E.sl_arrivals = 0;
+        plat_memset(E.d_sl_bar, 0, sizeof(unsigned) * 4, E.stream);
+        if (plat_sync(E.stream)) { E.single_off = true; return -1; }
+    }
+    return head;
 }
 
 int pe::run_loss_grad(pinn_engine& E, const float* d_theta, float* d_out, const float* term_w, int only_term , bool timing,
@@ -265,6 +310,8 @@
     const bool no_merge = std::getenv("PINN_NO_MERGE") != nullptr;
     const bool may_merge = !no_merge && !no_chain && !concurrent && only_term < 0;
     int nforked = 0;
+    const int single_group = single_tail_group(E, loss_only, only_term, concurrent, may_merge);
+    bool single_done = false;
     int nslabsets = 0, slabset_group = -1;
     if (concurrent) plat_event_record(E.ev_fork, E.stream);
     for (size_t g = 0; g < E.groups.size(); ++g) {
@@ -349,6 +396,20 @@
         if (forked) {
             st = E.aux_stream[nforked % 2];
             plat_stream_wait_event(st, E.ev_fork);
+        }
+        {
+            const char* lim = std::getenv("PINN_REDUCE_DIRECT_MAX");
+            const int direct_max = lim ? std::atoi(lim) : aux::REDUCE_DIRECT_MAX;
+            if ((int)g == single_group && !chained && blocks > direct_max && blocks <= E.ncu * E.single_resident) {
+                if (ga_launch != &ga_one) { ga_one = G.ga; ga_launch = &ga_one; }
+                pk::TailArgs& t = ga_one.tail;
+                E.sl_arrivals += (unsigned)blocks;
+                t.bar = E.d_sl_bar; t.target = E.sl_arrivals; t.hflag = E.h_sl_flag;
+                t.ent_theta = G.d_ent_theta; t.nent = G.nent; t.slab = G.slab_floats;
+                t.out = d_out; t.sums = d_sums; t.lossraw = lossraw ? lossraw : E.d_lossraw; t.P = (int)E.ntheta; t.K = K;
+                single_done = true;
+                E.single_last = 1;
+            }
         }
         if (group_ev(g)) plat_event_record(G.ev_a, st);
         if (merged_head) mu->pair->launch(*ga_launch, loss_only ? pk::MODE_LOSS : pk::MODE_FUSED, blocks, st);
@@ -423,7 +484,8 @@
     const bool no_reduce_one = std::getenv("PINN_NO_REDUCE_ONE") != nullptr;
     const Group* RG = (nslabsets == 1 && !coupled_active && !loss_only && !no_reduce_one) ? &E.groups[slabset_group] : nullptr;
     const bool one_kernel = ((RG && RG->d_ent_theta && RG->ent_covers_theta) || (loss_only && !no_reduce_one)) && !aux::reduce_is_small(a1, a2);
-    if (one_kernel) {
+    if (single_done) {
+    } else if (one_kernel) {
         aux::ReduceOneArgs ro;
         std::memset(&ro, 0, sizeof ro);
         if (RG) { ro.slabs = RG->d_slabs; ro.slab = RG->slab_floats; ro.nblocks = a1.nblocks[slabset_group]; ro.nent = RG->nent; ro.ent_theta = RG->d_ent_theta; }
@@ -523,7 +585,7 @@
     f64_destroy(E);
     free_plan(E);
     for (auto& T : E.terms) { plat_free(T.d_pts); plat_free(T.d_upts); plat_free(T.d_resid); plat_free(T.d_lb); plat_free(T.d_ub); plat_free(T.d_data); plat_free(T.d_pw); }
-    plat_free(E.d_opt_theta); plat_free(E.d_opt_m); plat_free(E.d_opt_v); plat_free(E.d_opt_out); plat_free(E.d_w_over_n); plat_free(E.d_hist); plat_free(E.d_step); plat_free(E.d_draws); plat_free(E.d_sampled); plat_free(E.d_c12); plat_free(E.d_bar); plat_free(E.d_sums2); plat_free(E.d_own_r); plat_free(E.d_train_samp); plat_free(E.d_opt_bak); plat_host_free(E.h_flag);
+    plat_free(E.d_opt_theta); plat_free(E.d_opt_m); plat_free(E.d_opt_v); plat_free(E.d_opt_out); plat_free(E.d_w_over_n); plat_free(E.d_hist); plat_free(E.d_step); plat_free(E.d_draws); plat_free(E.d_sampled); plat_free(E.d_c12); plat_free(E.d_bar); plat_free(E.d_sl_bar); plat_host_free(E.h_sl_flag); plat_free(E.d_sums2); plat_free(E.d_own_r); plat_free(E.d_train_samp); plat_free(E.d_opt_bak); plat_host_free(E.h_flag);
     plat_free(E.d_theta); plat_free(E.d_params); plat_free(E.d_defaults); plat_free(E.d_lossraw);
     plat_free(E.d_int_xi); plat_free(E.d_int_w);
     plat_free(E.d_out); plat_free(E.d_phi_pts); plat_free(E.d_phi_out); plat_free(E.d_phi_scr);
@@ -662,8 +724,15 @@
         if (plat_sync(E.stream)) return fail(std::string("device error: ") + plat_last_error());
         if (!train_timed_out(E)) { E.eval_path = 2; return 0; }
     }
-    if (run_loss_grad(E, E.d_theta, d_out, term_w, -1, timing, lossraw, false, false)) return 1;
+    {
+        SingleScope single(E);
+        if (run_loss_grad(E, E.d_theta, d_out, term_w, -1, timing, lossraw, false, false)) return 1;
+    }
     if (plat_sync(E.stream)) return fail(std::string("device error: ") + plat_last_error());
+    if (single_check_timeout(E)) {
+        if (run_loss_grad(E, E.d_theta, d_out, term_w, -1, timing, lossraw, false, false)) return 1;
+        if (plat_sync(E.stream)) return fail(std::string("device error: ") + plat_last_error());
+    }
     return 0;
 }
 
@@ -757,7 +826,11 @@
     plat_stream user = (plat_stream)stream;
     plat_stream saved = E.stream;
     E.stream = user;
-    int rc = E.f64 ? f64_eval_from_device_f32(E, d_theta, term_w, d_out, true) : run_loss_grad(E, d_theta, d_out, term_w, -1, true);
+    int rc;
+    {
+        SingleScope single(E);
+        rc = E.f64 ? f64_eval_from_device_f32(E, d_theta, term_w, d_out, true) : run_loss_grad(E, d_theta, d_out, term_w, -1, true);
+    }
     E.stream = saved;
     if (rc && g_err.empty()) return fail("pinn_loss_grad_device failed");
     E.timing_valid = (rc == 0) && E.timing_level >= 2;
@@ -1921,6 +1994,7 @@
             os << ",";
         }
         if (G.chain_to >= 0) os << " slabs=" << (G.blocks <= h->groups[G.chain_to].blocks ? "chained onto group " : "own (more workgroups than group ") << G.chain_to << (G.blocks <= h->groups[G.chain_to].blocks ? "" : ")");
+        if (h->single_last && G.launched_by == (int)g && G.active) os << " launch=single";
         if (G.merged >= 0 && h->merged[G.merged].tail == (int)g) os << " launch=merged into group " << h->merged[G.merged].head << "'s (one persistent kernel walks both tile lists)";
         os << "\n";
     }
diff --git a/neuralpde.jl_amd/csrc/engine_types.hpp b/neuralpde.jl_amd/csrc/engine_types.hpp
--- a/neuralpde.jl_amd/csrc/engine_types.hpp
+++ b/neuralpde.jl_amd/csrc/engine_types.hpp
@@ -261,6 +261,13 @@
     unsigned* d_bar = nullptr;
     unsigned* h_flag = nullptr;
     unsigned bar_arrivals = 0;
+    unsigned* d_sl_bar = nullptr;
+    unsigned* h_sl_flag = nullptr;
+    unsigned sl_arrivals = 0;
+    bool single_off = false;
+    int single_resident = -1;
+    bool single_allow = false;
+    int single_last = 0;
     float* d_sums2 = nullptr;
     int* d_own_r = nullptr;
     int own_blocks = 0, hist_gid = 0;
@@ -298,6 +305,12 @@
                      int np, Term& T);
 void analyse_static(Term& T, int np);
 bool fuse_laplacian(Term& T, int np);
+struct SingleScope {
+    pinn_engine& E;
+    explicit SingleScope(pinn_engine& e) : E(e) { E.single_allow = true; }
+    ~SingleScope() { E.single_allow = false; }
+};
+bool single_check_timeout(pinn_engine& E);
 int run_loss_grad(pinn_engine& E, const float* d_theta, float* d_out, const float* term_w, int only_term, bool timing, double* lossraw = nullptr,
                   bool packed_fresh = false, bool loss_only = false, float* d_sums = nullptr);
 int upload_theta(pinn_engine& E, const float* theta, int64_t p);
diff --git a/neuralpde.jl_amd/csrc/kernel_entry.hpp b/neuralpde.jl_amd/csrc/kernel_entry.hpp
--- a/neuralpde.jl_amd/csrc/kernel_entry.hpp
+++ b/neuralpde.jl_amd/csrc/kernel_entry.hpp
@@ -40,6 +40,7 @@
     int O_WBAR, O_BFRH, O_BFR0, O_W1, O_WL, O_BL, O_P;
     void (*launch)(const GroupArgs&, int mode, int blocks, plat_stream);
     void (*train)(const GroupArgs&, const TrainArgs&, int blocks, plat_stream);
+    int (*resident_fused)(int act);
 };
 
 template <class S>
@@ -65,8 +66,9 @@
 }
 
 template <class S>
-HD SpecInfo make_info2(void (*launch)(const GroupArgs&, int, int, plat_stream), int has_sin = 0) {
+HD SpecInfo make_info2(void (*launch)(const GroupArgs&, int, int, plat_stream), int has_sin = 0, int (*resident_fused)(int) = nullptr) {
     SpecInfo s = {};
+    s.resident_fused = resident_fused;
     s.has_sin = has_sin;
     s.jit = 0;
     s.act1 = s.act2 = s.dgm_rows = 0;
@@ -103,6 +105,7 @@
     s.launch = launch;
     return s;
 }
+constexpr bool TAIL_NW(int nw) { return nw == 4; }
 #ifndef PINN_EMU
 template <class S, int MODE, int ACTK>
 __global__ void __launch_bounds__(256, 1) k_wave(const GroupArgs ga) {
@@ -116,11 +119,28 @@
     const int w = __builtin_amdgcn_readfirstlane((int)(threadIdx.x >> 6));
     wave_train<S, ACTK>(ga, ta, (int)blockIdx.x, (int)gridDim.x, w, lds_all);
 }
+DEV void late_kernarg(void* dst, unsigned offset, unsigned bytes) {
+    const __attribute__((address_space(4))) char* k = (const __attribute__((address_space(4))) char*)__builtin_amdgcn_kernarg_segment_ptr();
+    asm volatile("" : "+s"(k) : : "memory");
+    __builtin_memcpy(dst, k + offset, bytes);
+}
+template <int NW, int LDS_FLOATS>
+DEV void single_tail_late(int w, float* lds) {
+    TailArgs t;
+    late_kernarg(&t, (unsigned)__builtin_offsetof(GroupArgs, tail), (unsigned)sizeof(TailArgs));
+    if (!t.bar) return;
+    float* slabs;
+    double* losspart;
+    late_kernarg(&slabs, (unsigned)__builtin_offsetof(GroupArgs, slabs), (unsigned)sizeof(float*));
+    late_kernarg(&losspart, (unsigned)__builtin_offsetof(GroupArgs, losspart), (unsigned)sizeof(double*));
+    single_tail2<NW, LDS_FLOATS>(t, slabs, losspart, (int)blockIdx.x, (int)gridDim.x, w, lds);
+}
 template <class S, int MODE, int ACTK>
 __global__ void __launch_bounds__(64 * S::NW, (mode_is_forward_only(MODE) ? S::OCC_FWD : S::OCC)) k_wave2(const GroupArgs ga) {
     __shared__ __attribute__((aligned(16))) float lds_all[mode_is_forward_only(MODE) ? S::LDS_FWD : S::LDS_WG];
     const int w = __builtin_amdgcn_readfirstlane((int)(threadIdx.x >> 6));
     wave_main2<S, MODE, ACTK>(ga, (int)blockIdx.x, (int)gridDim.x, w, lds_all);
+    if (MODE == MODE_FUSED && TAIL_NW(S::NW)) single_tail_late<S::NW, S::LDS_WG>(w, lds_all);
 }
 template <class S0, class S1> struct Pair2 {
     static constexpr int WG_PER_CU = S0::WG_PER_CU < S1::WG_PER_CU ? S0::WG_PER_CU : S1::WG_PER_CU;
@@ -136,6 +156,7 @@
     __shared__ __attribute__((aligned(16))) float lds_all[mode_is_forward_only(MODE) ? Pair2<S0, S1>::LDS_FWD : Pair2<S0, S1>::LDS_WG];
     const int w = __builtin_amdgcn_readfirstlane((int)(threadIdx.x >> 6));
     wave_main2m<S0, S1, ACTK, MODE>(ga, (int)blockIdx.x, (int)gridDim.x, w, lds_all);
+    if (MODE == MODE_FUSED && TAIL_NW(S0::NW)) single_tail_late<S0::NW, Pair2<S0, S1>::LDS_WG>(w, lds_all);
 }
 template <class S, int MODE>
 __global__ void __launch_bounds__(64) k_dgm(const GroupArgs ga) { wave_dgm<S, MODE>(ga, (int)blockIdx.x, (int)gridDim.x); }
diff --git a/neuralpde.jl_amd/csrc/pinn_kernels.hpp b/neuralpde.jl_amd/csrc/pinn_kernels.hpp
--- a/neuralpde.jl_amd/csrc/pinn_kernels.hpp
+++ b/neuralpde.jl_amd/csrc/pinn_kernels.hpp
@@ -168,6 +168,18 @@
     float lin_b[LIN_MAX_SRC];
 };
 
+struct TailArgs {
+    unsigned* bar;
+    unsigned target;
+    unsigned* hflag;
+    const int* ent_theta;
+    int nent, slab;
+    float* out;
+    float* sums;
+    double* lossraw;
+    int P, K;
+};
+
 struct GroupArgs {
     const float* packed;
     const float* params;
@@ -190,6 +202,7 @@
     int chain;
     int sub_terms0, sub_tiles0;
     int scr_stride;
+    TailArgs tail;
     TermDev terms[MAX_GROUP_TERMS];
 };
 
diff --git a/neuralpde.jl_amd/csrc/pinn_kernels2.hpp b/neuralpde.jl_amd/csrc/pinn_kernels2.hpp
--- a/neuralpde.jl_amd/csrc/pinn_kernels2.hpp
+++ b/neuralpde.jl_amd/csrc/pinn_kernels2.hpp
@@ -1,5 +1,6 @@
 #pragma once
 #include "pinn_kernels.hpp"
+#include "reduce_one.hpp"
 
 #if defined(PINN_STAMP) && !defined(PINN_EMU)
 #define STAMP_MEMBERS unsigned st_acc[24]; unsigned long long st_last;
@@ -1211,4 +1212,39 @@
     acc2_store<S0, (S0::PG > S1::PG ? S0::PG : S1::PG)>(ac, ga, blk, w, lds);
 }
 
+template <int NW, int LDS_FLOATS>
+DEV void single_tail2(const TailArgs& t, const float* slabs, const double* losspart, int blk, int nblocks, int w, float* lds) {
+    static_assert(LDS_FLOATS * 4 >= aux::RONE_SH * 8, "the tail's chunk sums live in the workgroup's LDS");
+    aux::ReduceOneArgs a;
+    a.slabs = slabs; a.slab = t.slab; a.nblocks = nblocks; a.nent = t.nent; a.ent_theta = t.ent_theta;
+    a.out = t.out; a.sums = t.sums; a.lossraw = t.lossraw; a.P = t.P; a.K = t.K;
+    a.nloss = 1; a.losspart[0] = losspart; a.nrows[0] = nblocks * NW;
+    double* sh = reinterpret_cast<double*>(lds);
+    const int nunits = aux::reduce_one_units(a), neb = aux::reduce_one_nentblocks(a);
+#ifdef PINN_EMU
+    for (int u = blk; u < nunits; u += nblocks) aux::reduce_one_unit_host(u, a, sh, false);
+#else
+    const int tid = w * 64 + (int)__builtin_amdgcn_mbcnt_hi(~0u, __builtin_amdgcn_mbcnt_lo(~0u, 0u));
+    grid_barrier(t.bar, t.target, tid);
+    const bool bad = __hip_atomic_load(t.bar + 1, __ATOMIC_RELAXED, __HIP_MEMORY_SCOPE_AGENT) != 0u;
+    if (bad && blk == 0 && tid == 0) *t.hflag = 1u;
+    for (int u = blk; u < nunits; u += nblocks) {
+        if (u < neb) {
+            if (tid < 256) aux::reduce_one_ent_chunks(u, tid, a, sh);
+            __syncthreads();
+            if (tid < 256) aux::reduce_one_ent_total(u, tid, a, sh, bad);
+        } else {
+            if (tid < 256) aux::reduce_one_loss_parts(u - neb, tid, a, sh);
+            __syncthreads();
+            for (int st = 128; st >= 1; st >>= 1) {
+                if (tid < 256) aux::reduce_one_loss_tree(st, tid, sh);
+                __syncthreads();
+            }
+            if (tid < 256) aux::reduce_one_loss_out(u - neb, tid, a, sh, bad);
+        }
+        __syncthreads();
+    }
+#endif
 }
+
+}
diff --git a/neuralpde.jl_amd/csrc/reduce_one.hpp b/neuralpde.jl_amd/csrc/reduce_one.hpp
--- /dev/null
+++ b/neuralpde.jl_amd/csrc/reduce_one.hpp
@@ -0,0 +1,93 @@
+#pragma once
+#include "aux_limits.hpp"
+
+namespace aux {
+
+#ifdef PINN_EMU
+#define AUX_DEV inline
+#else
+#define AUX_DEV __device__ __forceinline__
+#endif
+#ifdef PINN_EMU
+#define AUX_UNROLL8
+#else
+#define AUX_UNROLL8 _Pragma("unroll 8")
+#endif
+
+struct alignas(16) F4 { float x, y, z, w; };
+
+struct ReduceOneArgs {
+    const float* slabs;
+    int slab, nblocks, nent;
+    const int* ent_theta;
+    float* out;
+    float* sums;
+    double* lossraw;
+    int P, K;
+    int nloss;
+    const double* losspart[MAX_GROUPS];
+    int nrows[MAX_GROUPS];
+};
+constexpr int RONE_CHUNKS = 32, RONE_ENT = 32;
+constexpr int RONE_SH = RONE_CHUNKS * (RONE_ENT + 1);
+
+AUX_DEV void reduce_one_chunk(int e4, int ch, const ReduceOneArgs& a, double (&s)[4]) {
+    const int per = (a.nblocks + RONE_CHUNKS - 1) / RONE_CHUNKS;
+    const int b0 = ch * per, b1 = (b0 + per < a.nblocks) ? b0 + per : a.nblocks;
+    s[0] = s[1] = s[2] = s[3] = 0.0;
+    const float* p = a.slabs + 4 * e4;
+    AUX_UNROLL8
+    for (int b = b0; b < b1; ++b) {
+        const F4 q = *reinterpret_cast<const F4*>(p + (size_t)b * a.slab);
+        s[0] += (double)q.x; s[1] += (double)q.y; s[2] += (double)q.z; s[3] += (double)q.w;
+    }
+}
+AUX_DEV double reduce_one_loss_part(int k, int t, int nthreads, const ReduceOneArgs& a) {
+    double s = 0.0;
+    for (int i = 0; i < a.nloss; ++i)
+        for (int r = t; r < a.nrows[i]; r += nthreads) s += a.losspart[i][(size_t)r * a.K + k];
+    return s;
+}
+
+AUX_DEV int reduce_one_nentblocks(const ReduceOneArgs& a) { return (a.nent + RONE_ENT - 1) / RONE_ENT; }
+AUX_DEV int reduce_one_units(const ReduceOneArgs& a) { return reduce_one_nentblocks(a) + a.K; }
+AUX_DEV void reduce_one_ent_chunks(int u, int tid, const ReduceOneArgs& a, double* sh) {
+    const int j = tid & 7, ch = tid >> 3;
+    const int e4 = u * (RONE_ENT / 4) + j;
+    double s[4] = {0.0, 0.0, 0.0, 0.0};
+    if (4 * e4 < a.nent) reduce_one_chunk(e4, ch, a, s);
+    for (int e = 0; e < 4; ++e) sh[ch * (RONE_ENT + 1) + 4 * j + e] = s[e];
+}
+AUX_DEV void reduce_one_ent_total(int u, int tid, const ReduceOneArgs& a, const double* sh, bool poison) {
+    if (tid >= RONE_ENT) return;
+    const int ent = u * RONE_ENT + tid;
+    if (ent >= a.nent) return;
+    double tot = 0.0;
+    for (int c2 = 0; c2 < RONE_CHUNKS; ++c2) tot += sh[c2 * (RONE_ENT + 1) + tid];
+    const int th = a.ent_theta[ent];
+    if (th >= 0) a.out[th] = poison ? __builtin_nanf("") : (float)tot;
+}
+AUX_DEV void reduce_one_loss_parts(int k, int tid, const ReduceOneArgs& a, double* sh) { sh[tid] = reduce_one_loss_part(k, tid, 256, a); }
+AUX_DEV void reduce_one_loss_tree(int st, int tid, double* sh) { if (tid < st) sh[tid] += sh[tid + st]; }
+AUX_DEV void reduce_one_loss_out(int k, int tid, const ReduceOneArgs& a, const double* sh, bool poison) {
+    if (tid != 0) return;
+    const double s = poison ? (double)__builtin_nanf("") : sh[0];
+    a.sums[k] = (float)s;
+    if (a.lossraw) a.lossraw[k] = s;
+}
+#ifdef PINN_EMU
+inline void reduce_one_unit_host(int u, const ReduceOneArgs& a, double* sh, bool poison) {
+    const int neb = reduce_one_nentblocks(a);
+    if (u < neb) {
+        for (int tid = 0; tid < 256; ++tid) reduce_one_ent_chunks(u, tid, a, sh);
+        for (int tid = 0; tid < 256; ++tid) reduce_one_ent_total(u, tid, a, sh, poison);
+    } else {
+        for (int tid = 0; tid < 256; ++tid) reduce_one_loss_parts(u - neb, tid, a, sh);
+        for (int st = 128; st >= 1; st >>= 1)
+            for (int tid = 0; tid < st; ++tid) reduce_one_loss_tree(st, tid, sh);
+        reduce_one_loss_out(u - neb, 0, a, sh, poison);
+    }
+}
+#endif
+
+}
diff --git a/neuralpde.jl_amd/csrc/spec_registry.hpp b/neuralpde.jl_amd/csrc/spec_registry.hpp
--- a/neuralpde.jl_amd/csrc/spec_registry.hpp
+++ b/neuralpde.jl_amd/csrc/spec_registry.hpp
@@ -18,6 +18,7 @@
     int WG_PER_CU, NW, LDS_WG, SCR;
     int WG_FWD;
     void (*launch)(const GroupArgs&, int mode , int blocks, plat_stream);
+    int (*resident_fused)(int act);
 };
 std::deque<PairInfo>& pair_registry();
 
@@ -84,6 +85,8 @@
             });
         for (int w = 0; w < S::NW; ++w) th[w].join();
     }
+    if (MODE == MODE_FUSED && TAIL_NW(S::NW) && ga.tail.bar)
+        for (int b = 0; b < blocks; ++b) single_tail2<S::NW, S::LDS_WG>(ga.tail, ga.slabs, ga.losspart, b, blocks, 0, lds.data());
 }
 template <class S0, class S1, int ACTK, int MODE>
 void run_emu2m(const GroupArgs& ga, int blocks) {
@@ -101,6 +104,8 @@
             });
         for (int w = 0; w < S0::NW; ++w) th[w].join();
     }
+    if (MODE == MODE_FUSED && TAIL_NW(S0::NW) && ga.tail.bar)
+        for (int b = 0; b < blocks; ++b) single_tail2<S0::NW, (S0::LDS_WG > S1::LDS_WG ? S0::LDS_WG : S1::LDS_WG)>(ga.tail, ga.slabs, ga.losspart, b, blocks, 0, lds.data());
 }
 #define PINN_LAUNCH2(S, MODE, ACTK, ga, blocks, st) run_emu2<S, MODE, ACTK>(ga, blocks)
 #define PINN_LAUNCH2M(S0, S1, ACTK, MODE, ga, blocks, st) run_emu2m<S0, S1, ACTK, MODE>(ga, blocks)
@@ -112,6 +117,29 @@
 #define PINN_LAUNCH1(S, MODE, ACTK, ga, blocks, st) hipLaunchKernelGGL((k_wave<S, MODE, ACTK>), dim3(blocks), dim3(256), 0, st, ga)
 #define PINN_LAUNCH_TRAIN(S, ACTK, ga, ta, blocks, st) hipLaunchKernelGGL((k_train<S, ACTK>), dim3(blocks), dim3(256), 0, st, ga, ta)
 #endif
+
+template <class S> int resident_fused2(int act) {
+    if (!TAIL_NW(S::NW)) return 0;
+#ifdef PINN_EMU
+    return (act == ACT_TANH || act == ACT_SIGMOID) ? S::WG_PER_CU : 0;
+#else
+    int n = 0;
+    if (act == ACT_TANH) { if (hipOccupancyMaxActiveBlocksPerMultiprocessor(&n, k_wave2<S, MODE_FUSED, ACT_TANH>, 64 * S::NW, 0) != hipSuccess) n = 0; }
+    else if (act == ACT_SIGMOID) { if (hipOccupancyMaxActiveBlocksPerMultiprocessor(&n, k_wave2<S, MODE_FUSED, ACT_SIGMOID>, 64 * S::NW, 0) != hipSuccess) n = 0; }
+    return n;
+#endif
+}
+template <class S0, class S1> int resident_fused2m(int act) {
+    if (!TAIL_NW(S0::NW)) return 0;
+#ifdef PINN_EMU
+    return (act == ACT_TANH || act == ACT_SIGMOID) ? (S0::WG_PER_CU < S1::WG_PER_CU ? S0::WG_PER_CU : S1::WG_PER_CU) : 0;
+#else
+    int n = 0;
+    if (act == ACT_TANH) { if (hipOccupancyMaxActiveBlocksPerMultiprocessor(&n, k_wave2m<S0, S1, ACT_TANH, MODE_FUSED>, 64 * S0::NW, 0) != hipSuccess) n = 0; }
+    else if (act == ACT_SIGMOID) { if (hipOccupancyMaxActiveBlocksPerMultiprocessor(&n, k_wave2m<S0, S1, ACT_SIGMOID, MODE_FUSED>, 64 * S0::NW, 0) != hipSuccess) n = 0; }
+    return n;
+#endif
+}
 
 template <class S, int ACTK>
 void launch_modes2(const GroupArgs& ga, int mode, int blocks, plat_stream st) {
@@ -221,6 +249,7 @@
     p.SCR = S0::SCR > S1::SCR ? S0::SCR : S1::SCR;
     p.WG_FWD = S0::WG_FWD < S1::WG_FWD ? S0::WG_FWD : S1::WG_FWD;
     p.launch = &launch_pair2<S0, S1>;
+    p.resident_fused = &resident_fused2m<S0, S1>;
     return p;
 }
 
@@ -251,7 +280,7 @@
 template <class S> struct Launch2Swish { static void fn(const GroupArgs& ga, int mode, int blocks, plat_stream st) { launch_spec2_var<S, VARIANT_SWISH>(ga, mode, blocks, st); } };
 template <class S> struct Launch2SinSwish { static void fn(const GroupArgs& ga, int mode, int blocks, plat_stream st) { launch_spec2_var<S, VARIANT_SIN | VARIANT_SWISH>(ga, mode, blocks, st); } };
 template <class S, template <class> class L, bool ENABLE> struct Registrar2 {
-    explicit Registrar2(int has_sin) { registry().push_back(make_info2<S>(&L<S>::fn, has_sin)); }
+    explicit Registrar2(int has_sin) { registry().push_back(make_info2<S>(&L<S>::fn, has_sin, &resident_fused2<S>)); }
 };
 template <class S, template <class> class L> struct Registrar2<S, L, false> { explicit Registrar2(int) {} };
 template <class S0, class S1, bool ENABLE> struct PairRegistrar2 { PairRegistrar2() { pair_registry().push_back(make_pair_info<S0, S1>()); } };
diff --git a/neuralpde.jl_amd/csrc/vec.hpp b/neuralpde.jl_amd/csrc/vec.hpp
--- a/neuralpde.jl_amd/csrc/vec.hpp
+++ b/neuralpde.jl_amd/csrc/vec.hpp
@@ -464,10 +464,10 @@
 #define PINN_PROBE 0
 #endif
 DEV void wg_barrier() { if (!(PINN_PROBE & 4)) __syncthreads(); }
-DEV void grid_barrier(unsigned* bar, unsigned target) {
+DEV void grid_barrier(unsigned* bar, unsigned target, int tid) {
     asm volatile("s_waitcnt vmcnt(0)" ::: "memory");
     __syncthreads();
-    if (threadIdx.x == 0) {
+    if (tid == 0) {
         if (__hip_atomic_load(bar + 1, __ATOMIC_RELAXED, __HIP_MEMORY_SCOPE_AGENT) == 0u) {
             __builtin_amdgcn_fence(__ATOMIC_RELEASE, "agent");
             asm volatile("s_waitcnt vmcnt(0)" ::: "memory");
@@ -482,6 +482,7 @@
     }
     __syncthreads();
 }
+DEV void grid_barrier(unsigned* bar, unsigned target) { grid_barrier(bar, target, (int)threadIdx.x); }
 DEV void grid_barrier_wt(unsigned* bar, unsigned target) {
     asm volatile("s_waitcnt vmcnt(0)" ::: "memory");
     __syncthreads();
```

After: 207.6 million. 0.866x the previous value.
